# arangesh/TrackMPNN

Hardware: AMD Instinct MI355X
Metric: graph_edges_per_sec_fwd_bwd (higher is better)
Workload: dtype f32; 1 GPU; C2 KITTI Car/RRC-shaped rolling windows: 7 frames, D_t~clip(Poisson(6),1,20), F=8 (2d), H=64, K=0, diff; 1 fwd per frame + 1 bwd per window; 16384 windows/GPU batched block-diagonally (64 distinct seeds tiled); windows_per_gpu=16384, rows_final=6762496, parallelism=sequence-dp1

## Files before the change

### include/tmpnn.h

```cpp
#ifndef TMPNN_H
#define TMPNN_H

#include <stddef.h>
#include <stdint.h>

#ifdef __cplusplus
extern "C" {
#endif

#define TMPNN_ABI_VERSION 4

#define TMPNN_OK 0
#define TMPNN_EINVAL (-1)
#define TMPNN_ELAUNCH (-2)
#define TMPNN_EWORKSPACE (-3)

typedef void* tmpnn_stream;
typedef void* tmpnn_event;

typedef struct tmpnn_seg_plan {
    int32_t T;
    int32_t I;
    int32_t nsplit;
    const int32_t* t_row;
    const int32_t* items;
    const int32_t* rowptr2;
    const int32_t* inc2;
    float* ws;
    size_t ws_floats;
} tmpnn_seg_plan;

typedef struct tmpnn_win_plan {
    int32_t W;
    int32_t nbig;
    const int32_t* wrec;
    const int32_t* erow;
    const uint16_t* recs;
    const int32_t* det;
    const int32_t* drow;
    const int32_t* big_order;
} tmpnn_win_plan;

typedef struct tmpnn_graph {
    int32_t N;
    int32_t E;
    int32_t Dn;
    const int32_t* src;
    const int32_t* dst;
    const int32_t* edge_row;
    const int32_t* det_row;
    const int32_t* rowptr;
    const int32_t* inc;
    const int32_t* det_order;
    const tmpnn_seg_plan* seg_plan;
    const tmpnn_win_plan* win_plan;
} tmpnn_graph;

typedef struct tmpnn_edge_tiles {
    int32_t T;
    int32_t rows_per_tile;
    const int32_t* t_row;
    const int32_t* t_loc;
    const int32_t* t_dptr;
    const int32_t* t_dets;
} tmpnn_edge_tiles;

int tmpnn_abi_version(void);
const char* tmpnn_last_error(void);

int tmpnn_gather_diff_fwd(const tmpnn_graph* g, const float* in, int ld_in, float* out, int ld_out,
                          int H, int accumulate, tmpnn_stream stream);
int tmpnn_gather_concat_fwd(const tmpnn_graph* g, const float* in, int ld_in, float* out, int ld_out,
                            int H, int accumulate, tmpnn_stream stream);
int tmpnn_gather_diff_bwd(const tmpnn_graph* g, const float* d_out, int ld_dout, float* d_in, int ld_din,
                          int H, int accumulate, tmpnn_stream stream);
int tmpnn_gather_concat_bwd(const tmpnn_graph* g, const float* d_out, int ld_dout, float* d_in, int ld_din,
                            int H, int accumulate, tmpnn_stream stream);

int tmpnn_segsum_fwd(const tmpnn_graph* g, const float* in, int ld_in, float* out, int ld_out,
                     int H, int accumulate, int compact_out ,
                     tmpnn_stream stream);
int tmpnn_segsum_fwd_live(const tmpnn_graph* g, const float* in, int ld_in, float* out, int ld_out,
                          int H, int compact_out, int row_limit, tmpnn_stream stream);
int tmpnn_segsum_bwd(const tmpnn_graph* g, const float* d_out, int ld_dout, float* d_in, int ld_din,
                     int H, int accumulate, tmpnn_stream stream);

int tmpnn_att_fwd(const tmpnn_graph* g, const int32_t* erec, const float* h, int ld_h, int H, int K,
                  const float* W_cat, const float* a, const uint8_t* keep, float p_drop,
                  float* ha, float* score, float* stats, float* esk, float* alpha, float* out, int ld_out,
                  tmpnn_stream stream);
size_t tmpnn_att_bwd_ws(int E, int Dn, int H, int K);
int tmpnn_att_index(const tmpnn_graph* g, const int32_t* pos, const int32_t* src_pos, const int32_t* dst_pos,
                    int32_t* erec, int32_t* inc_other, tmpnn_stream stream);
int tmpnn_att_bwd(const tmpnn_graph* g, const int32_t* erec, const int32_t* inc_other,
                  const float* h, int ld_h, int H, int K,
                  const float* W_cat, const float* a, const uint8_t* keep, float p_drop,
                  const float* ha, const float* score, const float* stats, const float* esk,
                  const float* d_out, int ld_dout, float* ws, size_t ws_floats,
                  float* d_h, int ld_dh, float* dW_att, float* da, tmpnn_stream stream);
int tmpnn_att_bwd_heads(const tmpnn_graph* g, const int32_t* erec, const int32_t* inc_other,
                        const float* h, int ld_h, int H, int K,
                        const float* W_cat, const float* a, const uint8_t* keep, float p_drop,
                        const float* ha, const float* score, const float* stats, const float* esk,
                        const float* d_out, int ld_dout, float* ws, size_t ws_floats,
                        float* d_h, int ld_dh, float* const* dW_heads, float* const* da_heads, tmpnn_stream stream);

int tmpnn_gru_fwd_head_parts(int H, int IN, int xmode);
int tmpnn_gru_fwd(const int32_t* rows, int R, int xmode, const int32_t* src, const int32_t* dst,
                  const float* msg, int ld_msg, int msg_compact, int IN, const float* h, int ld_h, int H,
                  const float* wih_t, const float* whh_t, const float* b_ih, const float* b_hh,
                  float* h_out, int ld_out, float* gates, size_t gate_plane,
                  const float* w_head, float* logit_part, size_t part_stride, tmpnn_stream stream);
int tmpnn_gru_bwd_data(const int32_t* rows, int R, int IN, const float* h, int ld_h, int H,
                       const float* w_ih, const float* w_hh,
                       const float* gates, size_t gate_plane, const float* d_hout, int ld_dhout,
                       const float* dy, const float* w_head,
                       float* d_msg, int ld_dmsg, float* d_h, int ld_dh,
                       const int32_t* add_src, const int32_t* add_dst, const float* add_msg, int ld_add,
                       tmpnn_stream stream);
size_t tmpnn_gru_bwd_weights_ws(int R, int IN, int H);
int tmpnn_gru_bwd_weights(const int32_t* rows, int R, int xmode, const int32_t* src, const int32_t* dst,
                          const float* msg, int ld_msg, int msg_compact, int IN,
                          const float* h, int ld_h, int H,
                          const float* gates, size_t gate_plane, const float* d_hout, int ld_dhout,
                          const float* dy, const float* w_head,
                          float* dW_ih, float* dW_hh, float* db_ih, float* db_hh,
                          void* ws, size_t ws_bytes, tmpnn_stream stream);

int tmpnn_gru_bwd_fused_available(int H, int IN, int xmode);
size_t tmpnn_gru_bwd_fused_ws(int R, int IN, int H);
int tmpnn_gru_bwd_fused(const int32_t* rows, int R, int xmode, const int32_t* src, const int32_t* dst,
                        const float* msg, int ld_msg, int msg_compact, int IN,
                        const float* h, int ld_h, int H, const float* w_ih, const float* w_hh,
                        const float* gates, size_t gate_plane, const float* d_hout, int ld_dhout,
                        const float* dy, const float* w_head,
                        float* d_msg, int ld_dmsg, float* d_h, int ld_dh,
                        const int32_t* add_src, const int32_t* add_dst, const float* add_msg, int ld_add,
                        float* dW_ih, float* dW_hh, float* db_ih, float* db_hh,
                        void* ws, size_t ws_bytes, tmpnn_stream stream);
int tmpnn_gru_bwd_fused_zero_state_available(int H, int IN, int xmode);
int tmpnn_gru_bwd_fused_zero_state(const int32_t* rows, int R, const int32_t* src, const int32_t* dst, int IN,
                                   const float* h, int ld_h, int H, const float* w_ih, const float* b_hn,
                                   const float* gates, size_t gate_plane, const float* d_hout, int ld_dhout,
                                   const float* dy, const float* w_head, float* d_msg, int ld_dmsg,
                                   float* dW_ih, float* db_ih, float* db_hh,
                                   void* ws, size_t ws_bytes, tmpnn_stream stream);

int tmpnn_gru_fwd_tiles(const tmpnn_edge_tiles* tiles, int R, const float* proj, int ld_proj, const float* h, int ld_h, int H,
                        const float* whh_t, const float* b_ih, const float* b_hh, float* h_out, int ld_out, float* gates,
                        size_t gate_plane, const float* w_head, float* logit_part, size_t part_stride, tmpnn_stream stream);
int tmpnn_gru_fwd_tiles_zero_state_available(int H, int xmode);
int tmpnn_gru_fwd_tiles_zero_state(const tmpnn_edge_tiles* tiles, int R, const float* proj, int ld_proj, int H,
                                   const float* b_ih, const float* b_hh, float* h_out, int ld_out, float* gates,
                                   size_t gate_plane, int write_hn, const float* w_head, float* logit_part, size_t part_stride,
                                   tmpnn_stream stream);

int tmpnn_rows_linear(const int32_t* rows, int R, const float* in, int ld_in, int H, const float* wt, int NOUT,
                      float* out, int ld_out, tmpnn_stream stream);

int tmpnn_transpose(const float* in, int rows, int cols, float* out, tmpnn_stream stream);

int tmpnn_input_bn_fwd(const float* xdet, int ld_x, int F, int nd, const int32_t* seg_ptr,
                       const int32_t* seg_cnt, const int32_t* seg_of_det ,
                       int S, int H, int training,
                       const float* w1, const float* b1, const float* gamma, const float* beta,
                       float* running_mean, float* running_var,
                       const float* w2, const float* b2,
                       float* y_save, float* mean, float* rstd, float* ws_a ,
                       const int32_t* out_row, float* h_new, int ld_h, tmpnn_stream stream);
size_t tmpnn_input_bn_bwd_ws(int nd, int S, int H, int F);
int tmpnn_input_bn_bwd(const float* xdet, int ld_x, int F, int nd, const int32_t* seg_ptr,
                       const int32_t* seg_cnt, const int32_t* seg_of_det, int S, int H, int training,
                       const float* w1, const float* b1, const float* gamma, const float* beta,
                       const float* w2,
                       const float* y_save, const float* mean, const float* rstd,
                       const int32_t* out_row, const float* d_h, int ld_dh,
                       float* d_xdet, int ld_dx, float* d_xzero,
                       float* dw1, float* db1, float* dgamma, float* dbeta, float* dw2, float* db2,
                       float* ws, size_t ws_floats, tmpnn_stream stream);

int tmpnn_input_tf_supported(int H, int F, int max_seg_rows);
int tmpnn_input_tf_fwd(const float* xdet, const int64_t* x_rows, int ld_x, int F, int nd, const int32_t* seg_ptr, const int32_t* seg_cnt,
                       const int32_t* seg_of_det, int S, int max_seg_rows, int H, int training, const float* w1, const float* b1,
                       const float* gamma, const float* beta, float* running_mean, float* running_var, const float* w2,
                       const float* b2, float* y_save, float* mean, float* rstd, const int32_t* out_row, float* h_new,
                       int ld_h, tmpnn_stream stream);
size_t tmpnn_input_tf_bwd_ws(int nd, int S, int H, int F, int training);
int tmpnn_input_tf_bwd(const float* xdet, const int64_t* x_rows, int ld_x, int F, int nd, const int32_t* seg_ptr, const int32_t* seg_cnt,
                       const int32_t* seg_of_det, int S, int max_seg_rows, int H, int training, const float* w1, const float* b1,
                       const float* gamma, const float* beta, const float* w2, const float* y_save, const float* mean,
                       const float* rstd, const int32_t* out_row, const float* d_h, int ld_dh, float* d_xdet, int ld_dx,
                       float* d_xzero, float* dw1, float* db1, float* dgamma, float* dbeta, float* dw2, float* db2, void* ws,
                       size_t ws_bytes, tmpnn_stream stream);

int tmpnn_heads_fwd(const float* h, int ld_h, int C, int N, const uint8_t* is_edge,
                    const float* w_node, const float* b_node, const float* w_edge, const float* b_edge,
                    float* logits, float* scores, tmpnn_stream stream);
int tmpnn_heads_finish(const float* parts, size_t part_stride, int nparts, int N, const uint8_t* is_edge,
                       const float* b_node, const float* b_edge, float* logits, float* scores, tmpnn_stream stream);
size_t tmpnn_heads_bwd_ws(int N, int C);
int tmpnn_heads_bwd(const float* h, int ld_h, int C, int N, const uint8_t* is_edge,
                    const float* w_node, const float* w_edge, const float* scores,
                    const float* d_logits, const float* d_scores, float* dy_out,
                    float* d_h, int ld_dh, int accumulate,
                    float* dw_node, float* db_node, float* dw_edge, float* db_edge,
                    void* ws, size_t ws_bytes, tmpnn_stream stream);

int tmpnn_targets(const tmpnn_graph* g, const uint8_t* labels, uint8_t* targets, tmpnn_stream stream);
size_t tmpnn_ce_loss_ws(int Dn);
int tmpnn_ce_loss_fwd(const tmpnn_graph* g, const float* logits, const uint8_t* targets, float* stats, float* loss,
                      float* ws, size_t ws_floats, tmpnn_stream stream);
int tmpnn_ce_loss_bwd(const tmpnn_graph* g, const int32_t* src_pos, const int32_t* dst_pos, const float* logits,
                      const float* stats, const float* d_loss, float* d_logits, tmpnn_stream stream);
size_t tmpnn_focal_loss_ws(int R);
int tmpnn_focal_loss_fwd(const int32_t* rows, int R, const float* scores, const uint8_t* targets, float gamma,
                         int use_alpha, float alpha0, float alpha1, float* loss_sum, float* ws, size_t ws_floats,
                         tmpnn_stream stream);
int tmpnn_focal_loss_bwd(const int32_t* rows, int R, const float* scores, const uint8_t* targets, float gamma,
                         int use_alpha, float alpha0, float alpha1, const float* d_loss, float scale, float* d_scores,
                         tmpnn_stream stream);
size_t tmpnn_bce_logits_ws(long n);
int tmpnn_bce_logits_sum_fwd(const float* logits, const float* targets, long n, float* loss_sum, float* ws, size_t ws_floats,
                             tmpnn_stream stream);
int tmpnn_bce_logits_sum_bwd(const float* logits, const float* targets, long n, const float* d_loss, float* d_logits,
                             tmpnn_stream stream);
int tmpnn_train_losses_supported(int E, int Dn);
size_t tmpnn_train_losses_ws(int E, int Dn);
int tmpnn_train_losses_fwd(const tmpnn_graph* g, const float* logits, const float* scores, const uint8_t* labels,
                           int tp_classifier, uint8_t* targets, float* stats, float* out, float* ws, size_t ws_floats,
                           tmpnn_stream stream);
int tmpnn_train_losses_bwd(const tmpnn_graph* g, const int32_t* src_pos, const int32_t* dst_pos, const float* logits,
                           const float* scores, const uint8_t* targets, const float* stats, const float* d_c, const float* d_f,
                           int tp_classifier, float* d_logits, float* d_scores, tmpnn_stream stream);

#define TMPNN_DG_MAX_ROWS 4096
#define TMPNN_DG_BIG_ROWS 65535
#define TMPNN_TRACK_MAX_ROWS 32768
#define TMPNN_DG_META 8
#define TMPNN_DG_BAD_VALUE 1
#define TMPNN_DG_BAD_ROW 2
#define TMPNN_DG_BAD_ENDPOINT 4
#define TMPNN_DG_BAD_ORDER 8
#define TMPNN_DG_BAD_EDGE_DIAG 16
#define TMPNN_DG_BAD_EDGE_ADJ 32

typedef struct tmpnn_dgraph {
    int32_t N;
    int32_t cap;
    int32_t* meta;
    uint8_t* is_edge;
    int32_t* pos;
    int32_t* src;
    int32_t* dst;
    int32_t* src_pos;
    int32_t* dst_pos;
    int32_t* edge_row;
    int32_t* det_row;
    int32_t* rowptr;
    int32_t* inc;
} tmpnn_dgraph;

size_t tmpnn_dgraph_ints(int cap);
int tmpnn_dgraph_bind(void* arena, int cap, int N, tmpnn_dgraph* out);

int tmpnn_graph_from_coo(int N, const int64_t* node_idx, const float* node_val, int64_t nnz_node,
                         const int64_t* edge_idx, const float* edge_val, int64_t nnz_edge,
                         const tmpnn_dgraph* g, tmpnn_stream stream);

int tmpnn_graph_from_coo_arena(int N, const int64_t* node_idx, const float* node_val, int64_t nnz_node,
                               const int64_t* edge_idx, const float* edge_val, int64_t nnz_edge, void* arena, int cap,
                               tmpnn_stream stream);
int tmpnn_graph_from_coo_arena_ws(int N, const int64_t* node_idx, const float* node_val, int64_t nnz_node,
                                  const int64_t* edge_idx, const float* edge_val, int64_t nnz_edge, void* arena, int cap,
                                  void* ws, size_t ws_ints, tmpnn_stream stream);

int tmpnn_graph_from_rows_ws(int N, const uint8_t* is_edge, const int32_t* row_src, const int32_t* row_dst,
                             const tmpnn_dgraph* g, void* ws, size_t ws_ints, tmpnn_stream stream);

typedef struct tmpnn_mp_params {
    int32_t G, H, IN_e , F_total;
    int32_t F[3];
    float* w1[3]; float* b1[3]; float* gamma[3]; float* beta[3]; float* w2[3]; float* b2[3];
    float* run_mean[3]; float* run_var[3];
    int64_t* num_batches_tracked[3];
    float* e_wih[3]; float* e_whh[3]; float* e_bih[3]; float* e_bhh[3];
    float* n_wih[3]; float* n_whh[3]; float* n_bih[3]; float* n_bhh[3];
    float* w_node; float* b_node; float* w_edge; float* b_edge;
} tmpnn_mp_params;

size_t tmpnn_mp_iter_prep_floats(int G, int H, int IN_e);
int tmpnn_mp_iter_prepare(const tmpnn_mp_params* P, float* prep, tmpnn_stream stream);

size_t tmpnn_mp_iter_save_floats(int N, int n_new, int G, int H);
int tmpnn_mp_iter_fwd(const tmpnn_mp_params* P, const float* prep, const tmpnn_dgraph* g, int n_new,
                      const float* x, int ld_x, float* h, int training,
                      float* h_out, float* logits, float* scores, float* save, size_t save_floats,
                      tmpnn_stream stream);
size_t tmpnn_mp_iter_save_es_offset(int N, int n_new, int G, int H);
int tmpnn_mp_iter_fwd_parts(const tmpnn_mp_params* P, const float* prep, const tmpnn_dgraph* g, int n_new,
                            const float* x, int ld_x, float* h, int training,
                            float* h_out, float* logits, float* scores, float* save, size_t save_floats, int parts,
                            tmpnn_stream stream);
size_t tmpnn_mp_iter_bwd_ws(int N, int n_new, int G, int H, int IN_e);
int tmpnn_mp_iter_bwd(const tmpnn_mp_params* P, const float* prep, const tmpnn_dgraph* g, int n_new,
                      const float* x, int ld_x, const float* h, const float* h_out, const float* scores,
                      const float* save, int training,
                      const float* d_scores, int st_dscores, const float* d_logits, int st_dlogits,
                      const float* d_hout, float* d_h, float* d_x, const tmpnn_mp_params* grads,
                      void* ws, size_t ws_bytes, tmpnn_stream stream);
int tmpnn_mp_iter_bwd_parts(const tmpnn_mp_params* P, const float* prep, const tmpnn_dgraph* g, int n_new,
                            const float* x, int ld_x, const float* h, const float* h_out, const float* scores,
                            const float* save, int training,
                            const float* d_scores, int st_dscores, const float* d_logits, int st_dlogits,
                            const float* d_hout, float* d_h, float* d_x, const tmpnn_mp_params* grads,
                            void* ws, size_t ws_bytes, int parts, tmpnn_stream stream);

size_t tmpnn_track_finalize_ws(int max_dets);

typedef struct tmpnn_track_rows {
    int32_t *ts, *det_id, *assoc;
    uint8_t* is_edge;
    int32_t *src, *dst;
    uint8_t* labels;
} tmpnn_track_rows;
int tmpnn_track_load(int N, int ND, const int32_t* packed, const tmpnn_track_rows* rows, const float* X, int ld_x, int F,
                     float* feats, int ld_f, int32_t* y_track, const tmpnn_dgraph* g, void* ws, size_t ws_ints,
                     tmpnn_stream stream);
int tmpnn_track_select(const tmpnn_dgraph* g, const tmpnn_track_rows* rows, const float* score, int mode, int t,
                       int associate, int32_t* active, int32_t* small, tmpnn_stream stream);
int tmpnn_track_select_ws(const tmpnn_dgraph* g, const tmpnn_track_rows* rows, const float* score, int mode, int t,
                          int associate, int32_t* active, int32_t* small, void* ws, size_t ws_bytes, tmpnn_stream stream);
int tmpnn_track_hungarian_max_dets(void);
int tmpnn_track_extend(int N, int A, int D, const int32_t* active, const int32_t* new_ids, int t, const int32_t* track,
                       const tmpnn_track_rows* rows, const float* X, int ld_x, int F, float* feats, int ld_f,
                       const tmpnn_dgraph* g_new, void* ws, size_t ws_ints, tmpnn_stream stream);
int tmpnn_track_extend_tf(int N, int A, int D, const int32_t* active, const int32_t* new_ids, int t, const int32_t* track,
                          const tmpnn_track_rows* rows, const float* X, int ld_x, const tmpnn_mp_params* P, float* h,
                          float* save, size_t save_floats, const tmpnn_dgraph* g_new, const int32_t* counts,
                          const float* gather_src, int ld_gather, const int32_t* gather_keep, tmpnn_stream stream);
int tmpnn_track_retire(const tmpnn_dgraph* g, const tmpnn_track_rows* rows, const float* score, int associate, int t_upto,
                       int ret_win, int32_t* y_track, int ND, int32_t* pos_of_det, void* fin_ws, size_t fin_ws_bytes,
                       int32_t* keep, int32_t* small, const tmpnn_track_rows* rows_out, const float* h, int ld_h, int W,
                       float* h_new, int ld_hn, float* s_new, int next_t, int32_t* active, int32_t* notify,
                       tmpnn_stream stream);


int tmpnn_wide_supported(int H, int IN);
size_t tmpnn_wide_prep_bytes(int H, int IN);
int tmpnn_wide_prepare(const float* w_ih , const float* w_hh , int IN, int H, void* prep,
                       tmpnn_stream stream);
int tmpnn_wide_gru_fwd(const void* prep, const int32_t* det_rows, int Dn, const int32_t* rows, int R,
                       const int32_t* src_pos, const int32_t* dst_pos, const float* h, int ld_h, int H,
                       const float* b_ih, const float* b_hh, float* P, float* h_out, int ld_out, float* gates,
                       size_t gate_plane, tmpnn_stream stream);
int tmpnn_wide_gru_fwd_tiled(const void* prep, const int32_t* det_rows, int Dn, const tmpnn_edge_tiles* tiles, int R,
                             const float* h, int ld_h, int H, const float* b_ih, const float* b_hh, float* P,
                             float* h_out, int ld_out, float* gates, size_t gate_plane, tmpnn_stream stream);


// ... 44 lines not shown
```

### trackmpnn_amd/_lib.py

```python
from __future__ import annotations

import ctypes as C

import torch
import os
import re
from typing import Dict, List, Optional

_HERE = os.path.dirname(os.path.abspath(__file__))
LIB_PATH = os.environ.get('TMPNN_LIB_PATH') or os.path.join(_HERE, 'lib', 'libtmpnn.so')
HEADER_PATH = os.path.join(os.path.dirname(_HERE), 'include', 'tmpnn.h')

ABI_VERSION = 4

c_int = C.c_int
c_void_p = C.c_void_p
c_size_t = C.c_size_t
c_float = C.c_float


class CSegPlan(C.Structure):
    _fields_ = [('T', C.c_int32), ('I', C.c_int32), ('nsplit', C.c_int32), ('t_row', c_void_p), ('items', c_void_p),
                ('rowptr2', c_void_p), ('inc2', c_void_p), ('ws', c_void_p), ('ws_floats', c_size_t)]


class CWinPlan(C.Structure):
    _fields_ = [('W', C.c_int32), ('nbig', C.c_int32), ('wrec', c_void_p), ('erow', c_void_p), ('recs', c_void_p),
                ('det', c_void_p), ('drow', c_void_p), ('big_order', c_void_p)]


class CGraph(C.Structure):
    _fields_ = [('N', C.c_int32), ('E', C.c_int32), ('Dn', C.c_int32),
                ('src', c_void_p), ('dst', c_void_p), ('edge_row', c_void_p), ('det_row', c_void_p),
                ('rowptr', c_void_p), ('inc', c_void_p), ('det_order', c_void_p), ('seg_plan', c_void_p),
                ('win_plan', c_void_p)]


_GP = C.POINTER(CGraph)


class CEdgeTiles(C.Structure):
    _fields_ = [('T', C.c_int32), ('rows_per_tile', C.c_int32), ('t_row', c_void_p), ('t_loc', c_void_p),
                ('t_dptr', c_void_p), ('t_dets', c_void_p)]


_TP = C.POINTER(CEdgeTiles)


class CDGraph(C.Structure):
    _fields_ = [('N', C.c_int32), ('cap', C.c_int32), ('meta', c_void_p), ('is_edge', c_void_p), ('pos', c_void_p),
                ('src', c_void_p), ('dst', c_void_p), ('src_pos', c_void_p), ('dst_pos', c_void_p),
                ('edge_row', c_void_p), ('det_row', c_void_p), ('rowptr', c_void_p), ('inc', c_void_p)]


_P3 = c_void_p * 3


class CMpParams(C.Structure):
    _fields_ = [('G', C.c_int32), ('H', C.c_int32), ('IN_e', C.c_int32), ('F_total', C.c_int32), ('F', C.c_int32 * 3),
                ('w1', _P3), ('b1', _P3), ('gamma', _P3), ('beta', _P3), ('w2', _P3), ('b2', _P3),
                ('run_mean', _P3), ('run_var', _P3), ('num_batches_tracked', _P3),
                ('e_wih', _P3), ('e_whh', _P3), ('e_bih', _P3), ('e_bhh', _P3),
                ('n_wih', _P3), ('n_whh', _P3), ('n_bih', _P3), ('n_bhh', _P3),
                ('w_node', c_void_p), ('b_node', c_void_p), ('w_edge', c_void_p), ('b_edge', c_void_p)]


class CTrackRows(C.Structure):
    _fields_ = [('ts', c_void_p), ('det_id', c_void_p), ('assoc', c_void_p), ('is_edge', c_void_p), ('src', c_void_p),
                ('dst', c_void_p), ('labels', c_void_p)]


_DGP = C.POINTER(CDGraph)
_MPP = C.POINTER(CMpParams)
_TRP = C.POINTER(CTrackRows)

_SIGNATURES = {
    'tmpnn_abi_version': (c_int, []),
    'tmpnn_last_error': (C.c_char_p, []),
    'tmpnn_gather_diff_fwd': (c_int, [_GP, c_void_p, c_int, c_void_p, c_int, c_int, c_int, c_void_p]),
    'tmpnn_gather_concat_fwd': (c_int, [_GP, c_void_p, c_int, c_void_p, c_int, c_int, c_int, c_void_p]),
    'tmpnn_gather_diff_bwd': (c_int, [_GP, c_void_p, c_int, c_void_p, c_int, c_int, c_int, c_void_p]),
    'tmpnn_gather_concat_bwd': (c_int, [_GP, c_void_p, c_int, c_void_p, c_int, c_int, c_int, c_void_p]),
    'tmpnn_segsum_fwd': (c_int, [_GP, c_void_p, c_int, c_void_p, c_int, c_int, c_int, c_int, c_void_p]),
    'tmpnn_segsum_fwd_live': (c_int, [_GP, c_void_p, c_int, c_void_p, c_int, c_int, c_int, c_int, c_void_p]),
    'tmpnn_segsum_bwd': (c_int, [_GP, c_void_p, c_int, c_void_p, c_int, c_int, c_int, c_void_p]),
    'tmpnn_att_fwd': (c_int, [_GP, c_void_p, c_void_p, c_int, c_int, c_int, c_void_p, c_void_p, c_void_p, c_float,
                              c_void_p, c_void_p, c_void_p, c_void_p, c_void_p, c_void_p, c_int, c_void_p]),
    'tmpnn_att_bwd_ws': (c_size_t, [c_int, c_int, c_int, c_int]),
    'tmpnn_att_index': (c_int, [_GP, c_void_p, c_void_p, c_void_p, c_void_p, c_void_p, c_void_p]),
    'tmpnn_att_bwd': (c_int, [_GP, c_void_p, c_void_p, c_void_p, c_int, c_int, c_int, c_void_p, c_void_p, c_void_p,
                              c_float, c_void_p, c_void_p, c_void_p, c_void_p, c_void_p, c_int, c_void_p, c_size_t,
                              c_void_p, c_int, c_void_p, c_void_p, c_void_p]),
    'tmpnn_att_bwd_heads': (c_int, [_GP, c_void_p, c_void_p, c_void_p, c_int, c_int, c_int, c_void_p, c_void_p,
                                    c_void_p, c_float, c_void_p, c_void_p, c_void_p, c_void_p, c_void_p, c_int, c_void_p,
                                    c_size_t, c_void_p, c_int, c_void_p, c_void_p, c_void_p]),
    'tmpnn_gru_fwd': (c_int, [c_void_p, c_int, c_int, c_void_p, c_void_p, c_void_p, c_int, c_int, c_int,
                              c_void_p, c_int, c_int, c_void_p, c_void_p, c_void_p, c_void_p,
                              c_void_p, c_int, c_void_p, c_size_t, c_void_p, c_void_p, c_size_t, c_void_p]),
    'tmpnn_gru_fwd_head_parts': (c_int, [c_int, c_int, c_int]),
    'tmpnn_gru_fwd_tiles': (c_int, [_TP, c_int, c_void_p, c_int, c_void_p, c_int, c_int, c_void_p, c_void_p, c_void_p,
                                    c_void_p, c_int, c_void_p, c_size_t, c_void_p, c_void_p, c_size_t, c_void_p]),
    'tmpnn_gru_fwd_tiles_zero_state_available': (c_int, [c_int, c_int]),
    'tmpnn_gru_fwd_tiles_zero_state': (c_int, [_TP, c_int, c_void_p, c_int, c_int, c_void_p, c_void_p, c_void_p, c_int,
                                               c_void_p, c_size_t, c_int, c_void_p, c_void_p, c_size_t, c_void_p]),
    'tmpnn_heads_finish': (c_int, [c_void_p, c_size_t, c_int, c_int, c_void_p, c_void_p, c_void_p, c_void_p, c_void_p, c_void_p]),
    'tmpnn_gru_bwd_data': (c_int, [c_void_p, c_int, c_int, c_void_p, c_int, c_int, c_void_p, c_void_p,
                                   c_void_p, c_size_t, c_void_p, c_int, c_void_p, c_void_p,
                                   c_void_p, c_int, c_void_p, c_int,
                                   c_void_p, c_void_p, c_void_p, c_int, c_void_p]),
    'tmpnn_gru_bwd_weights_ws': (c_size_t, [c_int, c_int, c_int]),
    'tmpnn_gru_bwd_weights': (c_int, [c_void_p, c_int, c_int, c_void_p, c_void_p, c_void_p, c_int, c_int, c_int,
                                      c_void_p, c_int, c_int, c_void_p, c_size_t, c_void_p, c_int, c_void_p, c_void_p,
                                      c_void_p, c_void_p, c_void_p, c_void_p, c_void_p, c_size_t, c_void_p]),
    'tmpnn_gru_bwd_fused_available': (c_int, [c_int, c_int, c_int]),
    'tmpnn_gru_bwd_fused_ws': (c_size_t, [c_int, c_int, c_int]),
    'tmpnn_gru_bwd_fused': (c_int, [c_void_p, c_int, c_int, c_void_p, c_void_p, c_void_p, c_int, c_int, c_int,
                                    c_void_p, c_int, c_int, c_void_p, c_void_p, c_void_p, c_size_t, c_void_p, c_int,
                                    c_void_p, c_void_p, c_void_p, c_int, c_void_p, c_int,
                                    c_void_p, c_void_p, c_void_p, c_int, c_void_p, c_void_p, c_void_p, c_void_p,
                                    c_void_p, c_size_t, c_void_p]),
    'tmpnn_gru_bwd_fused_zero_state_available': (c_int, [c_int, c_int, c_int]),
    'tmpnn_gru_bwd_fused_zero_state': (c_int, [c_void_p, c_int, c_void_p, c_void_p, c_int, c_void_p, c_int, c_int,
                                               c_void_p, c_void_p, c_void_p, c_size_t, c_void_p, c_int, c_void_p,
                                               c_void_p, c_void_p, c_int, c_void_p, c_void_p, c_void_p, c_void_p,
                                               c_size_t, c_void_p]),
    'tmpnn_rows_linear': (c_int, [c_void_p, c_int, c_void_p, c_int, c_int, c_void_p, c_int, c_void_p, c_int, c_void_p]),
    'tmpnn_transpose': (c_int, [c_void_p, c_int, c_int, c_void_p, c_void_p]),
    'tmpnn_input_bn_fwd': (c_int, [c_void_p, c_int, c_int, c_int, c_void_p, c_void_p, c_void_p, c_int, c_int, c_int,
                                   c_void_p, c_void_p, c_void_p, c_void_p, c_void_p, c_void_p, c_void_p, c_void_p,
                                   c_void_p, c_void_p, c_void_p, c_void_p, c_void_p, c_void_p, c_int, c_void_p]),
    'tmpnn_input_bn_bwd_ws': (c_size_t, [c_int, c_int, c_int, c_int]),
    'tmpnn_input_bn_bwd': (c_int, [c_void_p, c_int, c_int, c_int, c_void_p, c_void_p, c_void_p, c_int, c_int, c_int,
                                   c_void_p, c_void_p, c_void_p, c_void_p, c_void_p,
                                   c_void_p, c_void_p, c_void_p, c_void_p, c_void_p, c_int,
                                   c_void_p, c_int, c_void_p,
                                   c_void_p, c_void_p, c_void_p, c_void_p, c_void_p, c_void_p,
                                   c_void_p, c_size_t, c_void_p]),
    'tmpnn_input_tf_supported': (c_int, [c_int, c_int, c_int]),
    'tmpnn_input_tf_fwd': (c_int, [c_void_p, c_void_p, c_int, c_int, c_int, c_void_p, c_void_p, c_void_p, c_int, c_int, c_int, c_int,
                                   c_void_p, c_void_p, c_void_p, c_void_p, c_void_p, c_void_p, c_void_p, c_void_p,
                                   c_void_p, c_void_p, c_void_p, c_void_p, c_void_p, c_int, c_void_p]),
    'tmpnn_input_tf_bwd_ws': (c_size_t, [c_int, c_int, c_int, c_int, c_int]),
    'tmpnn_input_tf_bwd': (c_int, [c_void_p, c_void_p, c_int, c_int, c_int, c_void_p, c_void_p, c_void_p, c_int, c_int, c_int, c_int,
                                   c_void_p, c_void_p, c_void_p, c_void_p, c_void_p,
                                   c_void_p, c_void_p, c_void_p, c_void_p, c_void_p, c_int,
                                   c_void_p, c_int, c_void_p,
                                   c_void_p, c_void_p, c_void_p, c_void_p, c_void_p, c_void_p,
                                   c_void_p, c_size_t, c_void_p]),
    'tmpnn_heads_fwd': (c_int, [c_void_p, c_int, c_int, c_int, c_void_p, c_void_p, c_void_p, c_void_p, c_void_p,
                                c_void_p, c_void_p, c_void_p]),
    'tmpnn_heads_bwd_ws': (c_size_t, [c_int, c_int]),
    'tmpnn_heads_bwd': (c_int, [c_void_p, c_int, c_int, c_int, c_void_p, c_void_p, c_void_p, c_void_p, c_void_p,
                                c_void_p, c_void_p, c_void_p, c_int, c_int, c_void_p, c_void_p, c_void_p, c_void_p,
                                c_void_p, c_size_t, c_void_p]),
    'tmpnn_targets': (c_int, [_GP, c_void_p, c_void_p, c_void_p]),
    'tmpnn_ce_loss_ws': (c_size_t, [c_int]),
    'tmpnn_ce_loss_fwd': (c_int, [_GP, c_void_p, c_void_p, c_void_p, c_void_p, c_void_p, c_size_t, c_void_p]),
    'tmpnn_ce_loss_bwd': (c_int, [_GP, c_void_p, c_void_p, c_void_p, c_void_p, c_void_p, c_void_p, c_void_p]),
    'tmpnn_focal_loss_ws': (c_size_t, [c_int]),
    'tmpnn_focal_loss_fwd': (c_int, [c_void_p, c_int, c_void_p, c_void_p, c_float, c_int, c_float, c_float, c_void_p,
                                     c_void_p, c_size_t, c_void_p]),
    'tmpnn_focal_loss_bwd': (c_int, [c_void_p, c_int, c_void_p, c_void_p, c_float, c_int, c_float, c_float, c_void_p,
                                     c_float, c_void_p, c_void_p]),
    'tmpnn_bce_logits_ws': (c_size_t, [C.c_long]),
    'tmpnn_bce_logits_sum_fwd': (c_int, [c_void_p, c_void_p, C.c_long, c_void_p, c_void_p, c_size_t, c_void_p]),
    'tmpnn_bce_logits_sum_bwd': (c_int, [c_void_p, c_void_p, C.c_long, c_void_p, c_void_p, c_void_p]),
    'tmpnn_train_losses_supported': (c_int, [c_int, c_int]),
    'tmpnn_train_losses_ws': (c_size_t, [c_int, c_int]),
    'tmpnn_train_losses_fwd': (c_int, [_GP, c_void_p, c_void_p, c_void_p, c_int, c_void_p, c_void_p, c_void_p, c_void_p,
                                       c_size_t, c_void_p]),
    'tmpnn_train_losses_bwd': (c_int, [_GP, c_void_p, c_void_p, c_void_p, c_void_p, c_void_p, c_void_p, c_void_p, c_void_p,
                                       c_int, c_void_p, c_void_p, c_void_p]),
    'tmpnn_dgraph_ints': (c_size_t, [c_int]),
    'tmpnn_dgraph_bind': (c_int, [c_void_p, c_int, c_int, _DGP]),
    'tmpnn_graph_from_coo': (c_int, [c_int, c_void_p, c_void_p, C.c_int64, c_void_p, c_void_p, C.c_int64, _DGP, c_void_p]),
    'tmpnn_graph_from_coo_arena': (c_int, [c_int, c_void_p, c_void_p, C.c_int64, c_void_p, c_void_p, C.c_int64, c_void_p, c_int, c_void_p]),
    'tmpnn_graph_from_coo_arena_ws': (c_int, [c_int, c_void_p, c_void_p, C.c_int64, c_void_p, c_void_p, C.c_int64, c_void_p, c_int,
                                              c_void_p, c_size_t, c_void_p]),
    'tmpnn_graph_from_rows_ws': (c_int, [c_int, c_void_p, c_void_p, c_void_p, _DGP, c_void_p, c_size_t, c_void_p]),
    'tmpnn_track_finalize_ws': (c_size_t, [c_int]),
    'tmpnn_track_load': (c_int, [c_int, c_int, c_void_p, _TRP, c_void_p, c_int, c_int, c_void_p, c_int, c_void_p, _DGP, c_void_p,
                                 c_size_t, c_void_p]),
    'tmpnn_track_select': (c_int, [_DGP, _TRP, c_void_p, c_int, c_int, c_int, c_void_p, c_void_p, c_void_p]),
    'tmpnn_track_select_ws': (c_int, [_DGP, _TRP, c_void_p, c_int, c_int, c_int, c_void_p, c_void_p, c_void_p, c_size_t, c_void_p]),
    'tmpnn_track_hungarian_max_dets': (c_int, []),
    'tmpnn_track_extend': (c_int, [c_int, c_int, c_int, c_void_p, c_void_p, c_int, c_void_p, _TRP, c_void_p, c_int, c_int,
                                   c_void_p, c_int, _DGP, c_void_p, c_size_t, c_void_p]),
    'tmpnn_track_extend_tf': (c_int, [c_int, c_int, c_int, c_void_p, c_void_p, c_int, c_void_p, _TRP, c_void_p, c_int, c_void_p,
                                      c_void_p, c_void_p, c_size_t, _DGP, c_void_p, c_void_p, c_int, c_void_p, c_void_p]),
    'tmpnn_track_retire': (c_int, [_DGP, _TRP, c_void_p, c_int, c_int, c_int, c_void_p, c_int, c_void_p, c_void_p, c_size_t,
                                   c_void_p, c_void_p, _TRP, c_void_p, c_int, c_int, c_void_p, c_int, c_void_p, c_int,
                                   c_void_p, c_void_p, c_void_p]),
    'tmpnn_wide_supported': (c_int, [c_int, c_int]),
    'tmpnn_wide_prep_bytes': (c_size_t, [c_int, c_int]),
    'tmpnn_wide_prepare': (c_int, [c_void_p, c_void_p, c_int, c_int, c_void_p, c_void_p]),
    'tmpnn_wide_gru_fwd': (c_int, [c_void_p, c_void_p, c_int, c_void_p, c_int, c_void_p, c_void_p, c_void_p, c_int, c_int,
                                   c_void_p, c_void_p, c_void_p, c_void_p, c_int, c_void_p, c_size_t, c_void_p]),
    'tmpnn_wide_gru_fwd_tiled': (c_int, [c_void_p, c_void_p, c_int, _TP, c_int, c_void_p, c_int, c_int, c_void_p, c_void_p,
                                         c_void_p, c_void_p, c_int, c_void_p, c_size_t, c_void_p]),
    'tmpnn_wide_gru_bwd_diff_ws': (c_size_t, [c_int, c_int, c_int, c_int]),
    'tmpnn_wide_gru_bwd_diff': (c_int, [c_void_p, _GP, c_void_p, c_int, c_int, c_void_p, c_size_t, c_void_p, c_int,
                                        c_void_p, c_void_p, c_void_p, c_int, c_void_p, c_void_p, c_void_p, c_void_p,
                                        c_void_p, c_size_t, c_void_p]),
    'tmpnn_wide_gru_bwd_diff_fused': (c_int, [c_void_p, _GP, c_void_p, c_int, c_int, c_void_p, c_size_t, c_void_p, c_int,
                                              c_void_p, c_void_p, c_void_p, c_int, c_void_p, c_void_p, c_void_p, c_void_p,
                                              c_void_p, c_size_t, c_void_p, c_int, c_void_p, c_void_p, c_void_p, c_void_p]),
    'tmpnn_mp_iter_prep_floats': (c_size_t, [c_int, c_int, c_int]),
    'tmpnn_mp_iter_prepare': (c_int, [_MPP, c_void_p, c_void_p]),
    'tmpnn_mp_iter_save_floats': (c_size_t, [c_int, c_int, c_int, c_int]),
    'tmpnn_mp_iter_fwd': (c_int, [_MPP, c_void_p, _DGP, c_int, c_void_p, c_int, c_void_p, c_int,
                                  c_void_p, c_void_p, c_void_p, c_void_p, c_size_t, c_void_p]),
    'tmpnn_mp_iter_save_es_offset': (c_size_t, [c_int, c_int, c_int, c_int]),
    'tmpnn_mp_iter_fwd_parts': (c_int, [_MPP, c_void_p, _DGP, c_int, c_void_p, c_int, c_void_p, c_int,
                                        c_void_p, c_void_p, c_void_p, c_void_p, c_size_t, c_int, c_void_p]),
    'tmpnn_mp_iter_bwd_parts': (c_int, [_MPP, c_void_p, _DGP, c_int, c_void_p, c_int, c_void_p, c_void_p, c_void_p, c_void_p,
                                        c_int, c_void_p, c_int, c_void_p, c_int, c_void_p, c_void_p, c_void_p, _MPP, c_void_p,
                                        c_size_t, c_int, c_void_p]),
    'tmpnn_mp_iter_bwd_ws': (c_size_t, [c_int, c_int, c_int, c_int, c_int]),
    'tmpnn_mp_iter_bwd': (c_int, [_MPP, c_void_p, _DGP, c_int, c_void_p, c_int, c_void_p, c_void_p, c_void_p, c_void_p,
                                  c_int, c_void_p, c_int, c_void_p, c_int, c_void_p, c_void_p, c_void_p, _MPP, c_void_p,
                                  c_size_t, c_void_p]),
}

_lib: Optional[C.CDLL] = None


_VARIANT_SIGNATURES = {
    'tmpnn_track_append': (c_int, [c_int, c_int, c_int, c_void_p, c_void_p, c_int, c_void_p, c_void_p, c_void_p, c_void_p,
                                   c_void_p, c_void_p, c_void_p, c_void_p, c_void_p]),
    'tmpnn_gru_bwd_weights_variant': (c_int, [c_void_p, c_int, c_int, c_void_p, c_void_p, c_void_p, c_int, c_int, c_int,
                                              c_void_p, c_int, c_int, c_void_p, c_size_t, c_void_p, c_int, c_void_p, c_void_p,
                                              c_void_p, c_void_p, c_void_p, c_void_p, c_void_p, c_size_t, c_int, c_void_p]),
    'tmpnn_gru_bwd_weights_choice': (c_int, []),
    'tmpnn_wide_gru_bwd_diff_aux': (c_int, [c_void_p, _GP, c_void_p, c_int, c_int, c_void_p, c_size_t, c_void_p, c_int,
                                            c_void_p, c_void_p, c_void_p, c_int, c_void_p, c_void_p, c_void_p, c_void_p,
                                            c_void_p, c_size_t, c_void_p, c_void_p, c_void_p, c_void_p]),
    'tmpnn_wide_gru_bwd_data_ws': (c_size_t, [c_int, c_int]),
    'tmpnn_wide_gru_bwd_data': (c_int, [c_void_p, c_void_p, c_int, c_void_p, c_int, c_int, c_void_p, c_size_t, c_void_p, c_int,
                                        c_void_p, c_void_p, c_void_p, c_int, c_void_p, c_int, c_void_p, c_size_t, c_void_p]),
    'tmpnn_wide_gru_bwd_weights_ws': (c_size_t, [c_int, c_int]),
    'tmpnn_wide_gru_bwd_weights': (c_int, [c_void_p, c_void_p, c_int, c_void_p, c_void_p, c_void_p, c_int, c_int, c_void_p,
                                           c_void_p, c_void_p, c_void_p, c_void_p, c_size_t, c_void_p]),
}


def header_symbols(variants: bool = False) -> List[str]:
    with open(HEADER_PATH) as f:
        txt = f.read()
    if not variants:
        txt = re.sub(r'#ifdef TMPNN_KEEP_VARIANTS.*?#endif', '', txt, flags=re.S)
    txt = re.sub(r'/\*.*?\*/', '', txt, flags=re.S)
    return sorted(set(re.findall(r'\b(tmpnn_[a-z0-9_]+)\s*\(', txt)))


def load() -> C.CDLL:
    global _lib
    if _lib is not None:
        return _lib
    if not os.path.exists(LIB_PATH):
        raise RuntimeError(
            f'{LIB_PATH} is missing: build it with `python -c "import __graft_entry__ as g; g.build()"` '
            '(hipcc --offload-arch=gfx950).  trackmpnn_amd has no CPU or torch fallback.')
    lib = C.CDLL(LIB_PATH)
    for name, (res, args) in _SIGNATURES.items():
        try:
            fn = getattr(lib, name)
        except AttributeError as e:
            raise RuntimeError(f'libtmpnn.so does not export {name}; rebuild it') from e
        fn.restype = res
        fn.argtypes = args
    for name, (res, args) in _VARIANT_SIGNATURES.items():
        fn = getattr(lib, name, None)
        if fn is not None:
            fn.restype = res
            fn.argtypes = args
    v = lib.tmpnn_abi_version()
    if v != ABI_VERSION:
        raise RuntimeError(f'libtmpnn.so ABI version {v} != expected {ABI_VERSION}; rebuild it')
    _lib = lib
    return lib


def last_error() -> str:
    return load().tmpnn_last_error().decode('utf-8', 'replace')


def call(name: str, *args) -> None:
    lib = load()
    rc = getattr(lib, name)(*args)
    if rc != 0:
        raise RuntimeError(f'{name} failed (code {rc}): {last_error()}')


def fn(name: str):
    return getattr(load(), name)


def ptr(t) -> Optional[int]:
    if t is None:
        return None
    return t.data_ptr()


def raw_stream(device=None) -> int:
    idx = torch.cuda.current_device() if device is None or device.index is None else device.index
    return torch._C._cuda_getCurrentRawStream(idx)
```

### trackmpnn_amd/csrc/dense.hip

```cpp
#include "common.h"

namespace tmpnn {

static constexpr float BN_EPS = 1e-5f;
static constexpr float BN_MOMENTUM = 0.1f;

__global__ __launch_bounds__(256) void k_gemm(GemmArgs g, int kper, float* slab) {
    __shared__ float As[16][68];
    __shared__ float Bs[16][68];
    const int tid = threadIdx.x;
    const int tx = tid & 15, ty = tid >> 4;
    const int m0 = blockIdx.y * 64, n0 = blockIdx.x * 64;
    const int kbeg = blockIdx.z * kper;
    const int kend = min(g.K, kbeg + kper);
    float acc[4][4] = {};
    const bool va = (reinterpret_cast<uintptr_t>(g.A) & 15) == 0 && ((g.sak == 1 ? g.sam : g.sak) & 3) == 0;
    const bool vb = (reinterpret_cast<uintptr_t>(g.B) & 15) == 0 && ((g.sbn == 1 ? g.sbk : g.sbn) & 3) == 0;
    for (int k0 = kbeg; k0 < kend; k0 += 16) {
        const bool fullk = k0 + 16 <= kend;
        if (fullk && m0 + 64 <= g.M && !g.a_krows && g.sak == 1 && va) {
            const int m = tid >> 2, kq = (tid & 3) * 4;
            const long ar = g.a_rows ? g.a_rows[m0 + m] : (m0 + m);
            const float4 v = *reinterpret_cast<const float4*>(g.A + ar * g.sam + k0 + kq);
            As[kq][m] = v.x; As[kq + 1][m] = v.y; As[kq + 2][m] = v.z; As[kq + 3][m] = v.w;
// ... 498 lines not shown
    d.w = r.w / cnt * (cnt * d.w - a1.w - yh.w * a2.w);
    *reinterpret_cast<float4*>(dyhat + idx) = d;
}

__global__ void k_bn_bwd_dy0(float* __restrict__ s1, float* __restrict__ s2, const int32_t* __restrict__ seg_ptr,
                             const int32_t* __restrict__ seg_cnt, int S, int H, const float* __restrict__ b1,
                             const float* __restrict__ mean, const float* __restrict__ rstd) {
    const size_t idx = (size_t)blockIdx.x * blockDim.x + threadIdx.x;
    if (idx >= (size_t)S * H) return;
    const int s = (int)(idx / H), j = (int)(idx % H);
    const float cnt = (float)seg_cnt[s];
    const float nz = cnt - (float)(seg_ptr[s + 1] - seg_ptr[s]);
    const float yh0 = (b1[j] - mean[idx]) * rstd[idx];
    const float dy0 = rstd[idx] / cnt * (-s1[idx] - yh0 * s2[idx]);
    s1[idx] = dy0;
    s2[idx] = nz * dy0;
}

__global__ void k_gather_rows(const float* __restrict__ src, long ld, const int32_t* __restrict__ rows, int n, int H,
                              float* __restrict__ dst) {
    const size_t idx = ((size_t)blockIdx.x * blockDim.x + threadIdx.x) * 4;
    if (idx >= (size_t)n * H) return;
    const int i = (int)(idx / H), j = (int)(idx % H);
    *reinterpret_cast<float4*>(dst + idx) = *reinterpret_cast<const float4*>(src + (size_t)rows[i] * ld + j);
}

__global__ __launch_bounds__(256) void k_heads_fwd(const float* __restrict__ h, int ld_h, int C, int N,
                                                   const uint8_t* __restrict__ is_edge,
                                                   const float* __restrict__ w_node, const float* __restrict__ b_node,
                                                   const float* __restrict__ w_edge, const float* __restrict__ b_edge,
                                                   float* __restrict__ logits, float* __restrict__ scores) {
    const int sub = threadIdx.x & 15;
    const long rows_per_pass = (long)gridDim.x * 16;
    for (long i = (long)blockIdx.x * 16 + (threadIdx.x >> 4); i < N; i += rows_per_pass) {
        const bool e = is_edge[i] != 0;
        const float* w = e ? w_edge : w_node;
        const float* hr = h + (size_t)i * ld_h;
        float s = 0.f;
        for (int c4 = sub * 4; c4 < C; c4 += 64) {
            const float4 x = *reinterpret_cast<const float4*>(hr + c4);
            const float4 ww = *reinterpret_cast<const float4*>(w + c4);
            s += x.x * ww.x + x.y * ww.y + x.z * ww.z + x.w * ww.w;
        }
        s += __shfl_xor(s, 8);
        s += __shfl_xor(s, 4);
        s += __shfl_xor(s, 2);
        s += __shfl_xor(s, 1);
        if (sub == 0) {
            const float y = s + (e ? b_edge[0] : b_node[0]);
            logits[i] = y;
            scores[i] = 1.0f / (1.0f + expf(-y));
        }
    }
}

__global__ void k_heads_finish(const float* __restrict__ parts, size_t stride, int nparts, int N,
                               const uint8_t* __restrict__ is_edge, const float* __restrict__ b_node,
                               const float* __restrict__ b_edge, float* __restrict__ logits,
                               float* __restrict__ scores) {
    const int i = blockIdx.x * blockDim.x + threadIdx.x;
    if (i >= N) return;
    float y = is_edge[i] ? b_edge[0] : b_node[0];
    for (int p = 0; p < nparts; ++p) y += parts[(size_t)p * stride + i];
    logits[i] = y;
    scores[i] = 1.0f / (1.0f + expf(-y));
}

__global__ __launch_bounds__(256) void k_heads_bwd(const float* __restrict__ h, int ld_h, int C, int N,
                                                   const uint8_t* __restrict__ is_edge,
                                                   const float* __restrict__ w_node, const float* __restrict__ w_edge,
                                                   const float* __restrict__ scores, const float* __restrict__ d_logits,
                                                   const float* __restrict__ d_scores, float* __restrict__ dy_out,
                                                   float* __restrict__ d_h,
                                                   int ld_dh, int accumulate, int rows_per_block,
                                                   float* __restrict__ part) {
    extern __shared__ float sm[];
    const int cpt = C >> 2;
    const int slots = 256 / cpt;
    const int slot = threadIdx.x / cpt;
    const int c4 = (threadIdx.x % cpt) * 4;
    const bool active = slot < slots;
    float4 an = make_float4(0.f, 0.f, 0.f, 0.f), ae = an;
    float bn = 0.f, be = 0.f;
    const long r0 = (long)blockIdx.x * rows_per_block;
    const long r1 = min((long)N, r0 + rows_per_block);
    if (active) {
        constexpr int UR = 4;
        for (long i0 = r0 + slot; i0 < r1; i0 += (long)slots * UR) {
            float dyv[UR];
            bool ev[UR], live[UR];
            float4 xv[UR];
#pragma unroll
            for (int u = 0; u < UR; ++u) {
                const long i = i0 + (long)u * slots;
                live[u] = i < r1;
                const long ic = live[u] ? i : r1 - 1;
                float dy = d_logits ? d_logits[ic] : 0.f;
                if (d_scores) {
                    const float sc = scores[ic];
                    dy += d_scores[ic] * sc * (1.0f - sc);
                }
                dyv[u] = live[u] ? dy : 0.f;
                ev[u] = is_edge[ic] != 0;
                xv[u] = *reinterpret_cast<const float4*>(h + (size_t)ic * ld_h + c4);
            }
#pragma unroll
            for (int u = 0; u < UR; ++u) {
                if (!live[u]) continue;
                const long i = i0 + (long)u * slots;
                const float dy = dyv[u];
                const bool e = ev[u];
                const float4 x = xv[u];
                if (dy_out && c4 == 0) dy_out[i] = dy;
                if (d_h) {
                    const float4 w = *reinterpret_cast<const float4*>((e ? w_edge : w_node) + c4);
                    float* dp = d_h + (size_t)i * ld_dh + c4;
                    float4 o = make_float4(dy * w.x, dy * w.y, dy * w.z, dy * w.w);
                    if (accumulate) {
                        const float4 p = *reinterpret_cast<const float4*>(dp);
                        o.x += p.x; o.y += p.y; o.z += p.z; o.w += p.w;
                    }
                    *reinterpret_cast<float4*>(dp) = o;
                }
                if (e) { ae.x += dy * x.x; ae.y += dy * x.y; ae.z += dy * x.z; ae.w += dy * x.w; if (c4 == 0) be += dy; }
                else   { an.x += dy * x.x; an.y += dy * x.y; an.z += dy * x.z; an.w += dy * x.w; if (c4 == 0) bn += dy; }
            }
        }
        float* my = sm + (size_t)slot * 2 * C;
        *reinterpret_cast<float4*>(my + c4) = an;
        *reinterpret_cast<float4*>(my + C + c4) = ae;
        if (c4 == 0) {
            sm[(size_t)slots * 2 * C + slot * 2 + 0] = bn;
            sm[(size_t)slots * 2 * C + slot * 2 + 1] = be;
        }
    }
    __syncthreads();
    float* out = part + (size_t)blockIdx.x * (2 * C + 2);
    for (int j = threadIdx.x; j < 2 * C + 2; j += 256) {
        float s = 0.f;
        if (j < 2 * C) for (int k = 0; k < slots; ++k) s += sm[(size_t)k * 2 * C + j];
        else for (int k = 0; k < slots; ++k) s += sm[(size_t)slots * 2 * C + k * 2 + (j - 2 * C)];
        out[j] = s;
    }
}

__global__ void k_heads_bwd_final(const float* __restrict__ red, int C, float* __restrict__ dw_node,
                                  float* __restrict__ db_node, float* __restrict__ dw_edge,
                                  float* __restrict__ db_edge) {
    const int j = blockIdx.x * blockDim.x + threadIdx.x;
    if (j >= 2 * C + 2) return;
    const float s = red[j];
    if (j < C) dw_node[j] += s;
    else if (j < 2 * C) dw_edge[j - C] += s;
    else if (j == 2 * C) db_node[0] += s;
    else db_edge[0] += s;
}

static int heads_rows_per_block(int N) {
    long rpb = ((long)N + 2047) / 2048;
    if (rpb < 64) rpb = 64;
    return (int)rpb;
}

}

using namespace tmpnn;

extern "C" {

int tmpnn_input_bn_fwd(const float* xdet, int ld_x, int F, int nd, const int32_t* seg_ptr, const int32_t* seg_cnt,
                       const int32_t* seg_of_det, int S, int H, int training, const float* w1, const float* b1, const float* gamma,
                       const float* beta, float* running_mean, float* running_var, const float* w2, const float* b2,
                       float* y_save, float* mean, float* rstd, float* ws_a, const int32_t* out_row, float* h_new,
                       int ld_h, tmpnn_stream stream) {
    TM_REQUIRE(supported_H_cell(H), "input_bn_fwd: unsupported H=%d", H);
    TM_REQUIRE(F > 0 && nd >= 0 && S >= 0, "input_bn_fwd: F=%d nd=%d S=%d", F, nd, S);
    TM_REQUIRE(w1 && b1 && gamma && beta && running_mean && running_var && w2 && b2 && mean && rstd,
               "input_bn_fwd: null parameter pointer");
    TM_REQUIRE(!training || (seg_ptr && seg_cnt && S > 0), "input_bn_fwd: training needs segments");
    hipStream_t st = as_stream(stream);
    int rc;
    if (nd > 0) {
        TM_REQUIRE(xdet && y_save && ws_a && out_row && h_new && ld_x >= F && ld_h >= H, "input_bn_fwd: null/short buffers");
        TM_REQUIRE(aligned16(y_save) && aligned16(ws_a) && aligned16(mean) && aligned16(rstd) && aligned16(gamma) && aligned16(beta),
                   "input_bn_fwd: y_save / ws_a / mean / rstd / gamma / beta must be 16-byte aligned");
        GemmArgs g{xdet, ld_x, 1, nullptr, nullptr, w1, 1, F, b1, y_save, H, nullptr, nd, H, F, 0};
        if ((rc = launch_gemm(g, st))) return rc;
    }
    if (training) {
        hipLaunchKernelGGL(k_bn_stats, dim3(S), dim3(H, bn_row_groups(nd, S, H)), 0, st, y_save, seg_ptr, seg_cnt, H, b1, mean, rstd);
        if ((rc = check_launch("bn_stats"))) return rc;
        hipLaunchKernelGGL(k_bn_running, dim3(H), dim3(64), 0, st, mean, rstd, seg_cnt, S, H, running_mean,
                           running_var);
        if ((rc = check_launch("bn_running"))) return rc;
    } else {
        hipLaunchKernelGGL(k_running_to_stats, dim3(ceil_div(H, 64)), dim3(64), 0, st, running_mean, running_var, H,
                           mean, rstd);
        if ((rc = check_launch("running_to_stats"))) return rc;
    }
    if (nd == 0) return TMPNN_OK;
    hipLaunchKernelGGL(k_bn_apply, dim3(ceil_div((long)nd * H / 4, 256)), dim3(256), 0, st, y_save, nd, H,
                       training ? seg_ptr : nullptr, S, seg_of_det, mean, rstd, gamma, beta, (float*)nullptr, ws_a);
    if ((rc = check_launch("bn_apply"))) return rc;
    GemmArgs g2{ws_a, H, 1, nullptr, nullptr, w2, 1, H, b2, h_new, ld_h, out_row, nd, H, H, 0};
    return launch_gemm(g2, st);
}

int tmpnn_input_bn_bwd(const float* xdet, int ld_x, int F, int nd, const int32_t* seg_ptr, const int32_t* seg_cnt,
                       const int32_t* seg_of_det, int S, int H, int training, const float* w1, const float* b1, const float* gamma,
                       const float* beta, const float* w2, const float* y_save, const float* mean, const float* rstd,
                       const int32_t* out_row, const float* d_h, int ld_dh, float* d_xdet, int ld_dx, float* d_xzero,
                       float* dw1, float* db1, float* dgamma, float* dbeta, float* dw2, float* db2, float* ws,
                       size_t ws_floats, tmpnn_stream stream) {
    TM_REQUIRE(supported_H_cell(H), "input_bn_bwd: unsupported H=%d", H);
    TM_REQUIRE(F > 0 && nd >= 0 && S >= 0, "input_bn_bwd: F=%d nd=%d S=%d", F, nd, S);
    TM_REQUIRE(w1 && b1 && gamma && beta && w2 && mean && rstd && dw1 && db1 && dgamma && dbeta && dw2 && db2,
               "input_bn_bwd: null parameter pointer");
    hipStream_t st = as_stream(stream);
    if (nd == 0) {
        if (d_xzero && S > 0) (void)hipMemsetAsync(d_xzero, 0, sizeof(float) * (size_t)S * F, st);
        return TMPNN_OK;
    }
    TM_REQUIRE(xdet && y_save && out_row && d_h && ws, "input_bn_bwd: null buffers");
    const size_t ndH = (size_t)nd * H, SH = (size_t)(S > 0 ? S : 1) * H;
    const size_t need = tmpnn_input_bn_bwd_ws(nd, S, H, F);
    if (ws_floats < need) return set_error(TMPNN_EWORKSPACE, "input_bn_bwd: workspace %zu < %zu floats", ws_floats, need);
    TM_REQUIRE(aligned16(y_save) && aligned16(mean) && aligned16(rstd) && aligned16(gamma) && aligned16(beta) && aligned16(ws) &&
                   aligned16(d_h) && (ld_dh & 3) == 0,
               "input_bn_bwd: y_save / mean / rstd / gamma / beta / ws / d_h must be 16-byte aligned (ld_dh a multiple of 4)");
    float* B0 = ws;
    float* B1 = B0 + ndH;
    float* B2 = B1 + ndH;
    float* s1 = B2 + ndH;
    float* s2 = s1 + SH;
    float* scratch = s2 + SH;
    const size_t scratch_n = ws_floats - (3 * ndH + 2 * SH);
    const int gridE = ceil_div((long)ndH / 4, 256);
    int rc;
    hipLaunchKernelGGL(k_gather_rows, dim3(gridE), dim3(256), 0, st, d_h, (long)ld_dh, out_row, nd, H, B0);
    if ((rc = check_launch("gather_rows"))) return rc;
    hipLaunchKernelGGL(k_bn_apply, dim3(gridE), dim3(256), 0, st, y_save, nd, H, training ? seg_ptr : nullptr, S,
                       seg_of_det, mean, rstd, gamma, beta, B1, B2);
    if ((rc = check_launch("bn_apply"))) return rc;
    {
        GemmArgs g{B0, 1, H, nullptr, nullptr, B2, H, 1, nullptr, dw2, H, nullptr, H, H, nd, 1};
        if ((rc = launch_gemm_splitk(g, scratch, scratch_n, st))) return rc;
        if ((rc = launch_colsum(B0, H, nullptr, 0, nd, H, db2, 1, scratch, scratch_n, st))) return rc;
    }
    {
        GemmArgs g{B0, H, 1, nullptr, nullptr, w2, H, 1, nullptr, B2, H, nullptr, nd, H, H, 0};
        if ((rc = launch_gemm(g, st))) return rc;
    }
    hipLaunchKernelGGL(k_bn_bwd_act, dim3(gridE), dim3(256), 0, st, B2, B1, nd, H, gamma, beta, B0);
    if ((rc = check_launch("bn_bwd_act"))) return rc;
    if ((rc = launch_colsum(B0, H, B1, H, nd, H, dgamma, 1, scratch, scratch_n, st))) return rc;
    if ((rc = launch_colsum(B0, H, nullptr, 0, nd, H, dbeta, 1, scratch, scratch_n, st))) return rc;
    if (training) {
        hipLaunchKernelGGL(k_bn_bwd_seg, dim3(S), dim3(H, bn_row_groups(nd, S, H)), 0, st, B2, B1, seg_ptr, seg_cnt, H, b1, mean, rstd, s1, s2);
        if ((rc = check_launch("bn_bwd_seg"))) return rc;
    }
    hipLaunchKernelGGL(k_bn_bwd_dy, dim3(gridE), dim3(256), 0, st, B2, B1, nd, H, seg_ptr, seg_cnt, S, seg_of_det, rstd,
                       s1, s2, training);
    if ((rc = check_launch("bn_bwd_dy"))) return rc;
    {
        GemmArgs g{B2, 1, H, nullptr, nullptr, xdet, ld_x, 1, nullptr, dw1, F, nullptr, H, F, nd, 1};
        if ((rc = launch_gemm_splitk(g, scratch, scratch_n, st))) return rc;
        if ((rc = launch_colsum(B2, H, nullptr, 0, nd, H, db1, 1, scratch, scratch_n, st))) return rc;
        if (d_xdet) {
            GemmArgs gx{B2, H, 1, nullptr, nullptr, w1, F, 1, nullptr, d_xdet, ld_dx, nullptr, nd, F, H, 0};
            if ((rc = launch_gemm(gx, st))) return rc;
        }
    }
    if (training) {
        hipLaunchKernelGGL(k_bn_bwd_dy0, dim3(ceil_div((long)S * H, 256)), dim3(256), 0, st, s1, s2, seg_ptr, seg_cnt,
                           S, H, b1, mean, rstd);
        if ((rc = check_launch("bn_bwd_dy0"))) return rc;
        const size_t cs2 = colsum_ws_floats(S, H);
        if (scratch_n < cs2) return set_error(TMPNN_EWORKSPACE, "input_bn_bwd: workspace too small for segments");
        if ((rc = launch_colsum(s2, H, nullptr, 0, S, H, db1, 1, scratch, scratch_n, st))) return rc;
        if (d_xzero) {
            GemmArgs gz{s1, H, 1, nullptr, nullptr, w1, F, 1, nullptr, d_xzero, F, nullptr, S, F, H, 0};
            if ((rc = launch_gemm(gz, st))) return rc;
        }
    } else if (d_xzero && S > 0) {
        (void)hipMemsetAsync(d_xzero, 0, sizeof(float) * (size_t)S * F, st);
    }
    return TMPNN_OK;
}

size_t tmpnn_input_bn_bwd_ws(int nd, int S, int H, int F) {
    if (nd <= 0) return 0;
    const size_t ndH = (size_t)nd * H, SH = (size_t)(S > 0 ? S : 1) * H;
    size_t x = colsum_ws_floats(nd, H);
    const size_t a = gemm_splitk_ws_floats(H, H, nd), b = gemm_splitk_ws_floats(H, F, nd),
                 c = colsum_ws_floats(S > 0 ? S : 1, H);
    if (a > x) x = a;
    if (b > x) x = b;
    if (c > x) x = c;
    return 3 * ndH + 2 * SH + x;
}

int tmpnn_heads_fwd(const float* h, int ld_h, int C, int N, const uint8_t* is_edge, const float* w_node,
                    const float* b_node, const float* w_edge, const float* b_edge, float* logits, float* scores,
                    tmpnn_stream stream) {
    TM_REQUIRE(C > 0 && (C & 3) == 0 && N >= 0, "heads_fwd: C=%d N=%d", C, N);
    if (N == 0) return TMPNN_OK;
    TM_REQUIRE(h && is_edge && w_node && b_node && w_edge && b_edge && logits && scores, "heads_fwd: null pointer");
    TM_REQUIRE(ld_h >= C && (ld_h & 3) == 0 && aligned16(h) && aligned16(w_node) && aligned16(w_edge),
               "heads_fwd: rows must be 16-byte aligned");
    long b = ((long)N + 15) / 16;
    if (b > 4096) b = 4096;
    hipLaunchKernelGGL(k_heads_fwd, dim3((int)b), dim3(256), 0, as_stream(stream), h, ld_h, C, N, is_edge, w_node,
                       b_node, w_edge, b_edge, logits, scores);
    return check_launch("heads_fwd");
}

int tmpnn_heads_finish(const float* parts, size_t part_stride, int nparts, int N, const uint8_t* is_edge,
                       const float* b_node, const float* b_edge, float* logits, float* scores, tmpnn_stream stream) {
    TM_REQUIRE(nparts > 0 && N >= 0, "heads_finish: nparts=%d N=%d", nparts, N);
    if (N == 0) return TMPNN_OK;
    TM_REQUIRE(parts && is_edge && b_node && b_edge && logits && scores && part_stride >= (size_t)N, "heads_finish: null pointer");
    hipLaunchKernelGGL(k_heads_finish, dim3(ceil_div(N, 256)), dim3(256), 0, as_stream(stream), parts, part_stride, nparts, N,
                       is_edge, b_node, b_edge, logits, scores);
    return check_launch("heads_finish");
}

size_t tmpnn_heads_bwd_ws(int N, int C) {
    if (N <= 0) return 0;
    const int rpb = heads_rows_per_block(N);
    const int nblk = ceil_div(N, rpb);
    const size_t n = 2 * (size_t)C + 2;
    return ((size_t)nblk * n + n + reduce_slabs_ws_floats(nblk, n)) * sizeof(float);
}

int tmpnn_heads_bwd(const float* h, int ld_h, int C, int N, const uint8_t* is_edge, const float* w_node,
                    const float* w_edge, const float* scores, const float* d_logits, const float* d_scores,
                    float* dy_out, float* d_h, int ld_dh, int accumulate, float* dw_node, float* db_node,
                    float* dw_edge, float* db_edge, void* ws, size_t ws_bytes, tmpnn_stream stream) {
    TM_REQUIRE(C > 0 && (C & 3) == 0 && C <= 1024 && N >= 0, "heads_bwd: C=%d N=%d", C, N);
    if (N == 0) return TMPNN_OK;
    TM_REQUIRE(h && is_edge && w_node && w_edge && dw_node && db_node && dw_edge && db_edge, "heads_bwd: null pointer");
    TM_REQUIRE(d_scores == nullptr || scores != nullptr, "heads_bwd: d_scores needs scores");
    TM_REQUIRE((ld_h & 3) == 0 && aligned16(h) && aligned16(w_node) && aligned16(w_edge) &&
                   (d_h == nullptr || ((ld_dh & 3) == 0 && aligned16(d_h))),
               "heads_bwd: rows must be 16-byte aligned");
    const size_t need = tmpnn_heads_bwd_ws(N, C);
    if (!ws || ws_bytes < need) return set_error(TMPNN_EWORKSPACE, "heads_bwd: workspace %zu < %zu", ws_bytes, need);
    const int rpb = heads_rows_per_block(N);
    const int nblk = ceil_div(N, rpb);
    const int cpt = C >> 2;
    TM_REQUIRE(cpt <= 256, "heads_bwd: C too wide");
    const int slots = 256 / cpt;
    const size_t shm = ((size_t)slots * 2 * C + (size_t)slots * 2) * sizeof(float);
    hipStream_t st = as_stream(stream);
    hipLaunchKernelGGL(k_heads_bwd, dim3(nblk), dim3(256), shm, st, h, ld_h, C, N, is_edge, w_node, w_edge, scores,
                       d_logits, d_scores, dy_out, d_h, ld_dh, accumulate, rpb, reinterpret_cast<float*>(ws));
    int rc = check_launch("heads_bwd");
    if (rc) return rc;
    const size_t nred = 2 * (size_t)C + 2;
    float* part = reinterpret_cast<float*>(ws);
    float* red = part + (size_t)nblk * nred;
    if ((rc = launch_reduce_slabs(part, nred, nblk, red, nred, 0, st, red + nred))) return rc;
    hipLaunchKernelGGL(k_heads_bwd_final, dim3(ceil_div(2 * C + 2, 256)), dim3(256), 0, st, red, C, dw_node, db_node,
                       dw_edge, db_edge);
    return check_launch("heads_bwd_final");
}

}
```

### trackmpnn_amd/csrc/gru_bwd.hip

```cpp
#include "gru_common.h"

namespace tmpnn {



template <int NT>
__global__ __launch_bounds__(256) void k_gru_bwd_data(GruBwdDataArgs a) {
    const int wave = threadIdx.x >> 6, lane = threadIdx.x & 63;
    const int c = lane & 31, half = lane >> 5;
    const int r0 = (blockIdx.x * 4 + wave) * 32;
    if (r0 >= a.R) return;
    const int H = a.H;
    const int vcol0 = blockIdx.y * (32 * NT);
    const bool is_dx = vcol0 < a.IN;
    const int n0 = is_dx ? vcol0 : vcol0 - a.IN;
    const float* __restrict__ W = is_dx ? a.w_ih : a.w_hh;
    const int ldw = is_dx ? a.IN : H;
    const int li = min(r0 + c, a.R - 1);
    const int row = a.rows[li];
    const size_t gp = a.gate_plane;

    f32x16 acc[NT];
#pragma unroll
    for (int t = 0; t < NT; ++t)
// ... 1290 lines not shown
        const uint16_t* p0_ = (base0);                                                                       \
        const uint16_t* p1_ = (base1);                                                                       \
        const uint2 u0_ = lds_read_tr(p0_), u1_ = lds_read_tr(p1_);                                          \
        const uint2 v0_ = lds_read_tr(p0_ + (pstride)), v1_ = lds_read_tr(p1_ + (pstride));                 \
        const uint2 w0_ = lds_read_tr(p0_ + 2 * (pstride)), w1_ = lds_read_tr(p1_ + 2 * (pstride));         \
        (q1) = make_uint4(u0_.x, u0_.y, u1_.x, u1_.y);                                                       \
        (q2) = make_uint4(v0_.x, v0_.y, v1_.x, v1_.y);                                                       \
        (q3) = make_uint4(w0_.x, w0_.y, w1_.x, w1_.y);                                                       \
    } while (0)
#define ONE_LD_BT(kb)                                                                                        \
    do {                                                                                                     \
        ONE_LD_TR(cur + (kb) * 2048 + offB[0][0], cur + (kb) * 2048 + offB[0][1], PB, bt[0].p1, bt[0].p2, bt[0].p3); \
        ONE_LD_TR(cur + (kb) * 2048 + offB[1][0], cur + (kb) * 2048 + offB[1][1], PB, bt[1].p1, bt[1].p2, bt[1].p3); \
    } while (0)
#define ONE_LD_A(g)                                                                                          \
    ONE_LD_TR(cur + ((g) / 3) * 2048 + offA[(g) % 3][0], cur + ((g) / 3) * 2048 + offA[(g) % 3][1], PA,      \
              aW[0][0], aW[0][1], aW[0][2])
        ONE_LD_D(0);
        ONE_LD_BT(0);
        ONE_LD_A(0);
        const int erow_n = a.rows[min((tile + G) * 32 + c, a.R - 1)];
        const bool elive_n = (it + 1 < nmine) && ((tile + G) * 32 + c < a.R);

        f32x16 accd;
#pragma unroll
        for (int i = 0; i < 16; ++i) accd[i] = 0.f;
        float d0[4], tt[4];
#pragma unroll
        for (int hs = 0; hs < 12; ++hs) {
            const int g = hs >> 1, kk = hs & 1, j = g % 3;
            if (hs + 1 < 12) ONE_LD_D(hs + 1);
            if (kk == 0) {
                acc[j][0] = mfma_c<0>(aW[0], bt[0], acc[j][0]);  accd = mfma_c<0>(wq[hs], bD[hs & 1], accd);
                acc[j][1] = mfma_c<0>(aW[0], bt[1], acc[j][1]);  accd = mfma_c<1>(wq[hs], bD[hs & 1], accd);
                acc[j][0] = mfma_c<1>(aW[0], bt[0], acc[j][0]);  accd = mfma_c<2>(wq[hs], bD[hs & 1], accd);
                acc[j][1] = mfma_c<1>(aW[0], bt[1], acc[j][1]);  accd = mfma_c<3>(wq[hs], bD[hs & 1], accd);
                acc[j][0] = mfma_c<2>(aW[0], bt[0], acc[j][0]);  accd = mfma_c<4>(wq[hs], bD[hs & 1], accd);
                acc[j][1] = mfma_c<2>(aW[0], bt[1], acc[j][1]);  accd = mfma_c<5>(wq[hs], bD[hs & 1], accd);
#pragma unroll
                for (int pc = 0; pc < 3; ++pc) {
                    const uint4 q = aW[0][pc];
                    bsum[j] = dot2_ones(q.x, bsum[j]); bsum[j] = dot2_ones(q.y, bsum[j]);
                    bsum[j] = dot2_ones(q.z, bsum[j]); bsum[j] = dot2_ones(q.w, bsum[j]);
                }
            } else {
                accd = mfma_c<0>(wq[hs], bD[hs & 1], accd);  acc[j][0] = mfma_c<3>(aW[0], bt[0], acc[j][0]);
                accd = mfma_c<1>(wq[hs], bD[hs & 1], accd);  acc[j][1] = mfma_c<3>(aW[0], bt[1], acc[j][1]);
                accd = mfma_c<2>(wq[hs], bD[hs & 1], accd);  acc[j][0] = mfma_c<4>(aW[0], bt[0], acc[j][0]);
                accd = mfma_c<3>(wq[hs], bD[hs & 1], accd);  acc[j][1] = mfma_c<4>(aW[0], bt[1], acc[j][1]);
                accd = mfma_c<4>(wq[hs], bD[hs & 1], accd);  acc[j][0] = mfma_c<5>(aW[0], bt[0], acc[j][0]);
                accd = mfma_c<5>(wq[hs], bD[hs & 1], accd);  acc[j][1] = mfma_c<5>(aW[0], bt[1], acc[j][1]);
            }
            if (kk == 1 && g + 1 < 6) ONE_LD_A(g + 1);
            if (hs == 5) ONE_LD_BT(1);
            if (hs < 6)
                half_slice<XMODE, UP, FUSE>(hs % 6, rawA, validA, head4, d0, tt, nxt, stA0, stA1, seA, SUB, PA, PB, OFF_B, OFF_E);
            else
                half_slice<XMODE, UP, FUSE>(hs % 6, rawB, validB, head4, d0, tt, nxt, stA0 + stB, stA1 + stB, seA + seB, SUB,
                                                    PA, PB, OFF_B, OFF_E);
            __builtin_amdgcn_sched_barrier(0);
            if (hs == 5) {
                half_issue_main<UP>(a, idA, f4, rawA);
                half_issue_gather<XMODE, FUSE>(a, idB, f4, rawB);
                __builtin_amdgcn_sched_barrier(0);
                validB = idB.valid;
                idB = half_ids<XMODE, FUSE>(a, tile + 2 * G, it + 2 < nmine, 16 + hr);
            }
            if (hs == 11) {
                half_issue_main<UP>(a, idB, f4, rawB);
                half_issue_gather<XMODE, FUSE>(a, idA, f4, rawA);
                __builtin_amdgcn_sched_barrier(0);
                validA = idA.valid;
                idA = half_ids<XMODE, FUSE>(a, tile + 3 * G, it + 3 < nmine, hr);
            }
        }
#undef ONE_LD_A
#undef ONE_LD_BT
#undef ONE_LD_TR
#undef ONE_LD_D
        if (is_dx) {
            if (elive) {
#pragma unroll
                for (int q = 0; q < 4; ++q)
                    *reinterpret_cast<float4*>(a.d_msg + (size_t)erow * a.ld_dmsg + n0 + 8 * q + 4 * half) =
                        make_float4(accd[4 * q], accd[4 * q + 1], accd[4 * q + 2], accd[4 * q + 3]);
            }
        } else {
            const float* e = reinterpret_cast<const float*>(cur + OFF_E) + eoff;
            float4 ex4[4];
#pragma unroll
            for (int q = 0; q < 4; ++q) ex4[q] = *reinterpret_cast<const float4*>(e + ((((n0 + 8 * q + 4 * half) >> 2) ^ (c & 15)) << 2));
            if (elive) {
#pragma unroll
                for (int q = 0; q < 4; ++q)
                    *reinterpret_cast<float4*>(a.d_h + (size_t)erow * a.ld_dh + n0 + 8 * q + 4 * half) =
                        make_float4(accd[4 * q] + ex4[q].x, accd[4 * q + 1] + ex4[q].y, accd[4 * q + 2] + ex4[q].z,
                                    accd[4 * q + 3] + ex4[q].w);
            }
        }
        erow = erow_n; elive = elive_n;
        __syncthreads();
    }
#undef ONE_STAGE
    float* sw = a.slab_w + (size_t)blockIdx.x * (3 * H) * (2 * H);
#pragma unroll
    for (int j = 0; j < 3; ++j)
#pragma unroll
        for (int t = 0; t < 2; ++t)
#pragma unroll
            for (int reg = 0; reg < 16; ++reg) {
                const int jj = (jt0 + j) * 32 + acc_row(reg, half);
                sw[(size_t)jj * (2 * H) + which * H + t * 32 + c] = acc[j][t][reg];
            }
    float* sb = a.slab_b + (size_t)blockIdx.x * 6 * H;
#pragma unroll
    for (int j = 0; j < 3; ++j) {
        const float tot = bsum[j] + __shfl_xor(bsum[j], 32);
        const int col = (jt0 + j) * 32 + c;
        if (half == 0) {
            if (which == 0) {
                sb[col] = tot;
                if (col < 2 * H) sb[3 * H + col] = tot;
            } else if (col >= 2 * H) {
                sb[3 * H + col] = tot;
            }
        }
    }
}
#endif

__device__ __forceinline__ f32x4 mfma16_bf16(const uint4& a, const uint4& b, f32x4 c) {
    return __builtin_amdgcn_mfma_f32_16x16x32_bf16(__builtin_bit_cast(bf16x8, a), __builtin_bit_cast(bf16x8, b), c, 0, 0, 0);
}
template <int C>
__device__ __forceinline__ f32x4 mfma16_c(const uint4 (&a)[3], const uint4 (&b)[3], f32x4 acc) {
    if (C == 0) return mfma16_bf16(a[2], b[0], acc);
    if (C == 1) return mfma16_bf16(a[0], b[2], acc);
    if (C == 2) return mfma16_bf16(a[1], b[1], acc);
    if (C == 3) return mfma16_bf16(a[1], b[0], acc);
    if (C == 4) return mfma16_bf16(a[0], b[1], acc);
    return mfma16_bf16(a[0], b[0], acc);
}
template <int C>
__device__ __forceinline__ f32x16 mfma32_c(const uint4 (&a)[3], const uint4 (&b)[3], f32x16 acc) {
    if (C == 0) return mfma_bf16(a[2], b[0], acc);
    if (C == 1) return mfma_bf16(a[0], b[2], acc);
    if (C == 2) return mfma_bf16(a[1], b[1], acc);
    if (C == 3) return mfma_bf16(a[1], b[0], acc);
    if (C == 4) return mfma_bf16(a[0], b[1], acc);
    return mfma_bf16(a[0], b[0], acc);
}

#define TWO_MARK(i) do { } while (0)
struct TwoRaw { float4 dh, r, z, n, hn, hp, xa, xb, ea, eb; float dy; };
#define TWO_LD4(p) (*reinterpret_cast<const float4*>(p))

#ifndef TWO_SCHED
#define TWO_SCHED 1
#endif
#ifndef TWO_EXP
#define TWO_EXP 0
#endif
template <int XMODE, int UP, bool FUSE, bool HHS = true>
__global__ __launch_bounds__(512) void k_gru_bwd_two(GruBwdFusedArgs a, int ntiles) {
    constexpr int exp_ = TWO_EXP;
    constexpr int H = 64;
    constexpr int SUB = 32 * 128;
    constexpr int PA = 2 * SUB, PB = SUB;
    constexpr int OFF_B = 3 * PA, OFF_E = OFF_B + 3 * PB;
    constexpr int BUF = OFF_E + 32 * 64 * 2;
    extern __shared__ float lds[];
    uint16_t* const lds16 = reinterpret_cast<uint16_t*>(lds);
    const int tid = threadIdx.x;
    const int wave = __builtin_amdgcn_readfirstlane(tid >> 6), lane = tid & 63;
    const int role = wave >> 2, q = wave & 3;
    const int lrole = role;
    const int j16 = lane & 15, kq = lane >> 4;
    const int srow = 4 * wave + kq, f4 = 4 * j16;
    const int n0 = 16 * q;
    uint4 wq[6][3];
    {
        const float* W = role == 0 ? a.w_ih : a.w_hh;
        const int ldw = role == 0 ? a.ld_wih : H;
#pragma unroll
        for (int s6 = 0; s6 < 6; ++s6) {
            const int ch = s6 < 4 ? 4 * kq + s6 : 16 + 4 * (s6 - 4) + kq;
            float v[8];
#pragma unroll
            for (int i = 0; i < 8; ++i) v[i] = W[(size_t)(8 * ch + i) * ldw + n0 + j16];
            const Split8 sp = split8_arr(v);
            wq[s6][0] = sp.p1; wq[s6][1] = sp.p2; wq[s6][2] = sp.p3;
        }
    }
    const float headl = (UP & 2) ? a.up.w_head[lane] : 0.f;
    const int st0 = dui_off(srow, f4);
    const int se0 = srow * 64 + (((f4 >> 2) ^ (srow & 15)) << 2);
    const int swzj = dui_swz(j16), rowj = j16 * 128;
    const int hix = lrole == 0 ? 0 : 64;
    const int half = lane >> 5, c32 = lane & 31;
    const int jt0 = (q >> 1) * 3, tt = q & 1;
    const int i16 = lane & 15, tq = i16 >> 2, tp = i16 & 3, tg = (lane >> 4) & 1;
    const int trow = (8 * half + tq) * 128, tsw0 = (tq << 2) | (2 * half);
    int offA[3], offB;
#pragma unroll
    for (int j = 0; j < 3; ++j) {
        const int jj0 = (jt0 + j) * 32;
        const int col = (lrole == 1 && jj0 >= 2 * H) ? jj0 + H : jj0;
        const int ch = ((col & 127) >> 3) + 2 * tg + (tp >> 1);
        offA[j] = (col >> 7) * SUB + trow + ((ch ^ tsw0) << 3) + 4 * (tp & 1);
    }
    {
        const int ch = ((lrole * H + tt * 32) >> 3) + 2 * tg + (tp >> 1);
        offB = OFF_B + trow + ((ch ^ tsw0) << 3) + 4 * (tp & 1);
    }
    f32x16 acc[3];
#pragma unroll
    for (int j = 0; j < 3; ++j)
#pragma unroll
        for (int i = 0; i < 16; ++i) acc[j][i] = 0.f;
    float bsum[3] = {0.f, 0.f, 0.f};

    const int G = gridDim.x;
    const int nmine = (ntiles - (int)blockIdx.x + G - 1) / G;
    TwoRaw raw;
    float d0[4], tv[4];
    auto row_of = [&](int tile, bool tvld, bool& vld) -> int {
        const int lr = tile * 32 + srow;
        vld = tvld && lr < a.R;
        return vld ? lr : a.R - 1;
    };
#define TWO_SLICE(SL, img, vld)                                                                              \
    do {                                                                                                     \
        float o_[4];                                                                                         \
        if ((SL) == 0) {                                                                                     \
            const float dh_[4] = {raw.dh.x, raw.dh.y, raw.dh.z, raw.dh.w}, r_[4] = {raw.r.x, raw.r.y, raw.r.z, raw.r.w}; \
            const float z_[4] = {raw.z.x, raw.z.y, raw.z.z, raw.z.w}, n_[4] = {raw.n.x, raw.n.y, raw.n.z, raw.n.w}; \
            const float hn_[4] = {raw.hn.x, raw.hn.y, raw.hn.z, raw.hn.w};                                   \
            float q_[4];                                                                                     \
            _Pragma("unroll") for (int i = 0; i < 4; ++i) {                                                  \
                float d_ = (UP & 1) ? dh_[i] : 0.f;                                                          \
                if (UP & 2) d_ += raw.dy * __shfl(headl, f4 + i);                                                        \
                d0[i] = (vld) ? d_ : 0.f;                                                                    \
                tv[i] = d0[i] * (1.0f - z_[i]) * (1.0f - n_[i] * n_[i]);                                     \
                q_[i] = tv[i] * r_[i];                                                                       \
                o_[i] = q_[i] * hn_[i] * (1.0f - r_[i]);                                                     \
            }                                                                                                \
            half_put((img), st0, PA, o_);                                                                    \
            half_put((img), SUB + (st0 ^ 64), PA, q_);                                                       \
        } else if ((SL) == 1) {                                                                              \
            const float z_[4] = {raw.z.x, raw.z.y, raw.z.z, raw.z.w}, n_[4] = {raw.n.x, raw.n.y, raw.n.z, raw.n.w}; \
            const float hp_[4] = {raw.hp.x, raw.hp.y, raw.hp.z, raw.hp.w};                                   \
            float e_[4];                                                                                     \
            _Pragma("unroll") for (int i = 0; i < 4; ++i) {                                                  \
                o_[i] = d0[i] * (hp_[i] - n_[i]) * z_[i] * (1.0f - z_[i]);                                   \
                e_[i] = d0[i] * z_[i];                                                                       \
            }                                                                                                \
            half_put((img), st0 ^ 64, PA, o_);                                                               \
            *reinterpret_cast<float4*>(reinterpret_cast<float*>((img) + OFF_E) + se0) = make_float4(e_[0], e_[1], e_[2], e_[3]); \
        } else if ((SL) == 2) {                                                                              \
            const float hp_[4] = {raw.hp.x, raw.hp.y, raw.hp.z, raw.hp.w};                                   \
            half_put((img) + OFF_B, st0 ^ 64, PB, hp_);                                                      \
        } else if ((SL) == 3) {                                                                              \
            half_put((img), SUB + st0, PA, tv);                                                              \
        } else if ((SL) == 5) {                                                                              \
            const float xa_[4] = {raw.xa.x, raw.xa.y, raw.xa.z, raw.xa.w}, xb_[4] = {raw.xb.x, raw.xb.y, raw.xb.z, raw.xb.w}; \
            _Pragma("unroll") for (int i = 0; i < 4; ++i) o_[i] = XMODE == 1 ? xa_[i] - xb_[i] : xa_[i];     \
            half_put((img) + OFF_B, st0, PB, o_);                                                            \
            if (FUSE) {                                                                                      \
                float4* ep_ = reinterpret_cast<float4*>(reinterpret_cast<float*>((img) + OFF_E) + se0);      \
                float4 e4_ = *ep_;                                                                           \
                e4_.x += raw.ea.x - raw.eb.x; e4_.y += raw.ea.y - raw.eb.y;                                  \
                e4_.z += raw.ea.z - raw.eb.z; e4_.w += raw.ea.w - raw.eb.w;                                  \
                *ep_ = e4_;                                                                                  \
            }                                                                                                \
        }                                                                                                    \
    } while (0)
#define TWO_ISSUE_MAIN(SL, orow_)                                                                            \
    do {                                                                                                     \
        const size_t gp_ = a.gate_plane;                                                                     \
        const float* g0_ = a.gates + (size_t)(orow_) * H + f4;                                               \
        if ((SL) == 0) {                                                                                     \
            if (UP & 1) raw.dh = *reinterpret_cast<const float4*>(a.up.d_hout + (size_t)(orow_) * a.up.ld_dhout + f4); \
            if (UP & 2) raw.dy = a.up.dy[(orow_)];                                                           \
            raw.hn = TWO_LD4(g0_ + 3 * gp_);                                                                 \
            raw.r = TWO_LD4(g0_);                                                                            \
        } else if ((SL) == 1) {                                                                              \
            raw.n = TWO_LD4(g0_ + 2 * gp_);                                                                  \
            raw.z = TWO_LD4(g0_ + gp_);                                                                      \
        } else if ((SL) == 2) {                                                                              \
            raw.hp = *reinterpret_cast<const float4*>(a.h + (size_t)(orow_) * a.ld_h + f4);                  \
        }                                                                                                    \
    } while (0)
#define TWO_ISSUE_GATHER(gs_, gd_)                                                                           \
    do {                                                                                                     \
        if (XMODE == 0) raw.xa = *reinterpret_cast<const float4*>(a.msg + (size_t)(gs_) * a.ld_msg + f4);    \
        if (XMODE != 0) {                                                                                    \
            raw.xa = *reinterpret_cast<const float4*>(a.h + (size_t)(gs_) * a.ld_h + f4);                    \
            if (XMODE == 1) raw.xb = *reinterpret_cast<const float4*>(a.h + (size_t)(gd_) * a.ld_h + f4);    \
            if (FUSE) {                                                                                      \
                raw.ea = *reinterpret_cast<const float4*>(a.add_msg + (size_t)(gs_) * a.ld_add + f4);        \
                raw.eb = *reinterpret_cast<const float4*>(a.add_msg + (size_t)(gd_) * a.ld_add + f4);        \
            }                                                                                                \
        }                                                                                                    \
    } while (0)
#define TWO_GATHER_IDS(lp_, gs_, gd_)                                                                        \
    do {                                                                                                     \
        if (XMODE == 0) { (gs_) = a.msg_compact ? (lp_) : a.rows[(lp_)]; (gd_) = 0; }                        \
        else { (gs_) = a.src[(lp_)]; (gd_) = a.dst[(lp_)]; }                                                 \
    } while (0)

    bool valid_cur, valid_n;
    int gs_cur, gd_cur;
    int orow_n;
    {
        bool v0, v1;
        const int lp0 = row_of(blockIdx.x, true, v0);
        const int o0 = a.rows[lp0];
        TWO_GATHER_IDS(lp0, gs_cur, gd_cur);
        TWO_ISSUE_MAIN(0, o0); TWO_ISSUE_MAIN(1, o0); TWO_ISSUE_MAIN(2, o0); TWO_ISSUE_GATHER(gs_cur, gd_cur);
        const int lp1 = row_of(blockIdx.x + G, 1 < nmine, v1);
        const int o1 = a.rows[lp1];
        TWO_SLICE(0, lds16, v0); TWO_ISSUE_MAIN(0, o1);
        TWO_SLICE(1, lds16, v0); TWO_ISSUE_MAIN(1, o1);
        TWO_SLICE(2, lds16, v0); TWO_ISSUE_MAIN(2, o1);
        TWO_SLICE(3, lds16, v0);
        TWO_SLICE(5, lds16, v0);
        valid_cur = v1;
        TWO_GATHER_IDS(lp1, gs_cur, gd_cur);
        const int lp2 = row_of(blockIdx.x + 2 * G, 2 < nmine, valid_n);
        orow_n = a.rows[lp2];
    }
    __syncthreads();

#define TWO_STAGE(ROLE_)                                                                                     \
    do {                                                                                                     \
        if (!(exp_ & 2)) TWO_SLICE(s6, nxt, valid_cur);                                                      \
        if (!(exp_ & 1)) {                                                                                   \
            TWO_ISSUE_MAIN(s6, orow_n);                                                                      \
             \
             \
            if (s6 == 3) TWO_ISSUE_GATHER(gs_cur, gd_cur);                                                   \
        }                                                                                                    \
        if (TWO_SCHED == 0) __builtin_amdgcn_sched_barrier(0);                                               \
    } while (0)
    for (int it = 0; it < nmine; ++it) {
        const int tile = blockIdx.x + it * G;
        uint16_t* const cur = lds16 + (it & 1) * BUF;
        uint16_t* const nxt = lds16 + ((it & 1) ^ 1) * BUF;
        const int er0 = a.rows[min(tile * 32 + j16, a.R - 1)], er1 = a.rows[min(tile * 32 + 16 + j16, a.R - 1)];
        const bool el0 = tile * 32 + j16 < a.R, el1 = tile * 32 + 16 + j16 < a.R;
        f32x4 accd[2];
#pragma unroll
        for (int i = 0; i < 4; ++i) { accd[0][i] = 0.f; accd[1][i] = 0.f; }
#pragma unroll
        for (int s6 = 0; s6 < 6; ++s6) {
            const int kb = s6 / 3, j = s6 % 3;
            uint4 bd[3], aw[3], bt[3];
            const uint16_t* pd;
            {
                const int chunk = s6 < 4 ? 4 * kq + s6 : 4 * (s6 - 4) + kq;
                int inrow = (chunk ^ swzj) << 3;
                if (s6 >= 4) inrow ^= hix;
                pd = cur + (s6 >= 4 ? SUB : 0) + rowj + inrow;
            }
            {
                const uint16_t* p0 = cur + kb * 2048 + offB;
                const uint16_t* p1 = cur + kb * 2048 + (offB ^ 8) + 4 * 128;
#pragma unroll
                for (int pc = 0; pc < 3; ++pc) {
                    const uint2 u0 = lds_read_tr(p0 + pc * PB), u1 = lds_read_tr(p1 + pc * PB);
                    bt[pc] = make_uint4(u0.x, u0.y, u1.x, u1.y);
                }
            }
            {
                const uint16_t* p0 = cur + kb * 2048 + offA[j];
                const uint16_t* p1 = cur + kb * 2048 + (offA[j] ^ 8) + 4 * 128;
#pragma unroll
                for (int pc = 0; pc < 3; ++pc) {
                    const uint2 u0 = lds_read_tr(p0 + pc * PA), u1 = lds_read_tr(p1 + pc * PA);
                    aw[pc] = make_uint4(u0.x, u0.y, u1.x, u1.y);
                }
            }
            TWO_MARK(0);
            if (TWO_SCHED >= 1) TWO_STAGE(0);
            TWO_MARK(1);
            if (!(exp_ & 4)) {
            acc[j] = mfma32_c<0>(aw, bt, acc[j]); acc[j] = mfma32_c<1>(aw, bt, acc[j]);
            acc[j] = mfma32_c<2>(aw, bt, acc[j]); acc[j] = mfma32_c<3>(aw, bt, acc[j]);
            acc[j] = mfma32_c<4>(aw, bt, acc[j]); acc[j] = mfma32_c<5>(aw, bt, acc[j]);
            } else { acc[j][0] += __uint_as_float(aw[0].x ^ bt[0].x ^ aw[1].y ^ bt[1].y ^ aw[2].z ^ bt[2].z); }
            if (HHS && kb == tt && !(exp_ & 8)) {
#pragma unroll
                for (int pc = 0; pc < 3; ++pc) {
                    const uint4 v = aw[pc];
                    bsum[j] = dot2_ones(v.x, bsum[j]); bsum[j] = dot2_ones(v.y, bsum[j]);
                    bsum[j] = dot2_ones(v.z, bsum[j]); bsum[j] = dot2_ones(v.w, bsum[j]);
                }
            }
            if (TWO_SCHED == 0) __builtin_amdgcn_sched_barrier(0);
            TWO_MARK(2);
#pragma unroll
            for (int pc = 0; pc < 3; ++pc) bd[pc] = *reinterpret_cast<const uint4*>(pd + pc * PA);
            if (!(exp_ & 4)) {
            accd[0] = mfma16_c<0>(wq[s6], bd, accd[0]); accd[0] = mfma16_c<1>(wq[s6], bd, accd[0]);
            accd[0] = mfma16_c<2>(wq[s6], bd, accd[0]); accd[0] = mfma16_c<3>(wq[s6], bd, accd[0]);
            accd[0] = mfma16_c<4>(wq[s6], bd, accd[0]); accd[0] = mfma16_c<5>(wq[s6], bd, accd[0]);
            } else { accd[0][0] += __uint_as_float(bd[0].x ^ bd[1].y ^ bd[2].z); }
            if (TWO_SCHED == 0) __builtin_amdgcn_sched_barrier(0);
#pragma unroll
            for (int pc = 0; pc < 3; ++pc) bd[pc] = *reinterpret_cast<const uint4*>(pd + pc * PA + 16 * 128);
            if (!(exp_ & 4)) {
            accd[1] = mfma16_c<0>(wq[s6], bd, accd[1]); accd[1] = mfma16_c<1>(wq[s6], bd, accd[1]);
            accd[1] = mfma16_c<2>(wq[s6], bd, accd[1]); accd[1] = mfma16_c<3>(wq[s6], bd, accd[1]);
            accd[1] = mfma16_c<4>(wq[s6], bd, accd[1]); accd[1] = mfma16_c<5>(wq[s6], bd, accd[1]);
            } else { accd[1][0] += __uint_as_float(bd[0].x ^ bd[1].y ^ bd[2].z); }
            if (TWO_SCHED == 0) __builtin_amdgcn_sched_barrier(0);
            if (TWO_SCHED == 0) TWO_STAGE(0);
            __builtin_amdgcn_sched_barrier(0);
            TWO_MARK(3);
        }
        {
            bool vnn;
            const int lp2 = row_of(tile + 2 * G, it + 2 < nmine, vnn);
            TWO_GATHER_IDS(lp2, gs_cur, gd_cur);
            valid_cur = valid_n;
            const int lp3 = row_of(tile + 3 * G, it + 3 < nmine, valid_n);
            orow_n = a.rows[lp3];
            (void)vnn;
        }
        int cofs = n0 + 4 * kq;
        asm volatile("" : "+v"(cofs));
        if (exp_ & 16) {
            if (accd[0][0] + accd[1][1] + (float)er0 + (float)er1 == 123.456f) a.d_msg[cofs] = 1.f;
        } else if (role == 0) {
            if (el0) *reinterpret_cast<float4*>(a.d_msg + ((size_t)er0 * a.ld_dmsg + cofs)) =
                         make_float4(accd[0][0], accd[0][1], accd[0][2], accd[0][3]);
            if (el1) *reinterpret_cast<float4*>(a.d_msg + ((size_t)er1 * a.ld_dmsg + cofs)) =
                         make_float4(accd[1][0], accd[1][1], accd[1][2], accd[1][3]);
        } else if (HHS) {
            const float* e = reinterpret_cast<const float*>(cur + OFF_E);
            const int cq = cofs >> 2;
            const float4 x0 = *reinterpret_cast<const float4*>(e + j16 * 64 + ((cq ^ j16) << 2));
            const float4 x1 = *reinterpret_cast<const float4*>(e + (16 + j16) * 64 + ((cq ^ j16) << 2));
            if (el0) *reinterpret_cast<float4*>(a.d_h + ((size_t)er0 * a.ld_dh + cofs)) =
                         make_float4(accd[0][0] + x0.x, accd[0][1] + x0.y, accd[0][2] + x0.z, accd[0][3] + x0.w);
            if (el1) *reinterpret_cast<float4*>(a.d_h + ((size_t)er1 * a.ld_dh + cofs)) =
                         make_float4(accd[1][0] + x1.x, accd[1][1] + x1.y, accd[1][2] + x1.z, accd[1][3] + x1.w);
        }
        TWO_MARK(4);
        __syncthreads();
        TWO_MARK(5);
    }
#undef TWO_STAGE
#undef TWO_GATHER_IDS
#undef TWO_ISSUE_GATHER
#undef TWO_ISSUE_MAIN
#undef TWO_SLICE
    float* sw = a.slab_w + (size_t)blockIdx.x * (3 * H) * (2 * H);
    if (HHS || role == 0) {
#pragma unroll
        for (int j = 0; j < 3; ++j)
#pragma unroll
            for (int reg = 0; reg < 16; ++reg) {
                const int jj = (jt0 + j) * 32 + acc_row(reg, half);
                sw[(size_t)jj * (2 * H) + role * H + tt * 32 + c32] = acc[j][reg];
            }
    }
    {
        float* red = lds;
#pragma unroll
        for (int j = 0; j < 3; ++j) {
            const float tot = bsum[j] + __shfl_xor(bsum[j], 32);
            if (half == 0) red[wave * 96 + j * 32 + c32] = tot;
        }
        __syncthreads();
        if (HHS && tt == 0 && half == 0) {
            float* sb = a.slab_b + (size_t)blockIdx.x * 6 * H;
#pragma unroll
            for (int j = 0; j < 3; ++j)
                sb[role * 3 * H + (jt0 + j) * 32 + c32] = red[wave * 96 + j * 32 + c32] + red[(wave + 1) * 96 + j * 32 + c32];
        }
    }
}

template <int UP>
__global__ __launch_bounds__(512) void k_gru_bwd_zs(GruBwdFusedArgs a, const float* __restrict__ b_hn, int ntiles) {
    constexpr int H = 64;
    constexpr int SUB = 32 * 128;
    constexpr int PA = 2 * SUB, PB = SUB;
    constexpr int OFF_B = 3 * PA;
    constexpr int BUF = OFF_B + 3 * PB;
    extern __shared__ float lds[];
    uint16_t* const lds16 = reinterpret_cast<uint16_t*>(lds);
    const int tid = threadIdx.x;
    const int wave = __builtin_amdgcn_readfirstlane(tid >> 6), lane = tid & 63;
    const int role = wave >> 2, q = wave & 3;
    const int j16 = lane & 15, kq = lane >> 4;
    const int srow = 4 * wave + kq, f4 = 4 * j16;
    const int n0 = 16 * q;
    uint4 wq[6][3];
#pragma unroll
    for (int s6 = 0; s6 < 6; ++s6) {
        const int ch = s6 < 4 ? 4 * kq + s6 : 16 + 4 * (s6 - 4) + kq;
        float v[8];
#pragma unroll
        for (int i = 0; i < 8; ++i) v[i] = a.w_ih[(size_t)(8 * ch + i) * a.ld_wih + n0 + j16];
        const Split8 sp = split8_arr(v);
        wq[s6][0] = sp.p1; wq[s6][1] = sp.p2; wq[s6][2] = sp.p3;
    }
    const float headl = (UP & 2) ? a.up.w_head[lane] : 0.f;
    const float4 bhn = *reinterpret_cast<const float4*>(b_hn + f4);
    const int st0 = dui_off(srow, f4);
    const int swzj = dui_swz(j16), rowj = (16 * role + j16) * 128;
    const int half = lane >> 5, c32 = lane & 31;
    const int jt0 = (q >> 1) * 3, tt = q & 1;
    const int i16 = lane & 15, tq = i16 >> 2, tp = i16 & 3, tg = (lane >> 4) & 1;
    const int trow = (8 * half + tq) * 128, tsw0 = (tq << 2) | (2 * half);
    const int kofs = role * 2048;
    int offA[3], offB;
#pragma unroll
    for (int j = 0; j < 3; ++j) {
        const int col = (jt0 + j) * 32;
        const int ch = ((col & 127) >> 3) + 2 * tg + (tp >> 1);
        offA[j] = kofs + (col >> 7) * SUB + trow + ((ch ^ tsw0) << 3) + 4 * (tp & 1);
    }
    {
        const int ch = ((tt * 32) >> 3) + 2 * tg + (tp >> 1);
        offB = kofs + OFF_B + trow + ((ch ^ tsw0) << 3) + 4 * (tp & 1);
    }
    f32x16 acc[3];
#pragma unroll
    for (int j = 0; j < 3; ++j)
#pragma unroll
        for (int i = 0; i < 16; ++i) acc[j][i] = 0.f;
    float bs_r[4] = {0.f, 0.f, 0.f, 0.f}, bs_z[4] = {0.f, 0.f, 0.f, 0.f};
    float bs_n[4] = {0.f, 0.f, 0.f, 0.f}, bs_nr[4] = {0.f, 0.f, 0.f, 0.f};

    const int G = gridDim.x;
    const int nmine = (ntiles - (int)blockIdx.x + G - 1) / G;
    struct { float4 dh, r, z, n, xa, xb; float dy; } raw;
    float d0[4], tv[4];
    auto row_of = [&](int tile, bool tvld, bool& vld) -> int {
        const int lr = tile * 32 + srow;
        vld = tvld && lr < a.R;
        return vld ? lr : a.R - 1;
    };
#define ZS_SLICE(SL, img, vld)                                                                               \
    do {                                                                                                     \
        float o_[4];                                                                                         \
        if ((SL) == 0) {                                                                                     \
            const float dh_[4] = {raw.dh.x, raw.dh.y, raw.dh.z, raw.dh.w}, r_[4] = {raw.r.x, raw.r.y, raw.r.z, raw.r.w}; \
            const float z_[4] = {raw.z.x, raw.z.y, raw.z.z, raw.z.w}, n_[4] = {raw.n.x, raw.n.y, raw.n.z, raw.n.w}; \
            const float hn_[4] = {bhn.x, bhn.y, bhn.z, bhn.w};                                               \
            _Pragma("unroll") for (int i = 0; i < 4; ++i) {                                                  \
                float d_ = (UP & 1) ? dh_[i] : 0.f;                                                          \
                if (UP & 2) d_ += raw.dy * __shfl(headl, f4 + i);                                            \
                d0[i] = (vld) ? d_ : 0.f;                                                                    \
                tv[i] = d0[i] * (1.0f - z_[i]) * (1.0f - n_[i] * n_[i]);                                     \
                const float q_ = tv[i] * r_[i];                                                              \
                o_[i] = q_ * hn_[i] * (1.0f - r_[i]);                                                        \
                bs_r[i] += o_[i]; bs_n[i] += tv[i]; bs_nr[i] += q_;                                          \
            }                                                                                                \
            half_put((img), st0, PA, o_);                                                                    \
        } else if ((SL) == 1) {                                                                              \
            const float z_[4] = {raw.z.x, raw.z.y, raw.z.z, raw.z.w}, n_[4] = {raw.n.x, raw.n.y, raw.n.z, raw.n.w}; \
            _Pragma("unroll") for (int i = 0; i < 4; ++i) {                                                  \
                o_[i] = d0[i] * (0.0f - n_[i]) * z_[i] * (1.0f - z_[i]);                                     \
                bs_z[i] += o_[i];                                                                            \
            }                                                                                                \
            half_put((img), st0 ^ 64, PA, o_);                                                               \
        } else if ((SL) == 3) {                                                                              \
            half_put((img), SUB + st0, PA, tv);                                                              \
        } else if ((SL) == 5) {                                                                              \
            const float xa_[4] = {raw.xa.x, raw.xa.y, raw.xa.z, raw.xa.w}, xb_[4] = {raw.xb.x, raw.xb.y, raw.xb.z, raw.xb.w}; \
            _Pragma("unroll") for (int i = 0; i < 4; ++i) o_[i] = xa_[i] - xb_[i];                           \
            half_put((img) + OFF_B, st0, PB, o_);                                                            \
        }                                                                                                    \
    } while (0)
#define ZS_ISSUE_MAIN(SL, orow_)                                                                             \
    do {                                                                                                     \
        const size_t gp_ = a.gate_plane;                                                                     \
        const float* g0_ = a.gates + (size_t)(orow_) * H + f4;                                               \
        if ((SL) == 0) {                                                                                     \
            if (UP & 1) raw.dh = *reinterpret_cast<const float4*>(a.up.d_hout + (size_t)(orow_) * a.up.ld_dhout + f4); \
            if (UP & 2) raw.dy = a.up.dy[(orow_)];                                                           \
            raw.r = TWO_LD4(g0_);                                                                            \
        } else if ((SL) == 1) {                                                                              \
            raw.n = TWO_LD4(g0_ + 2 * gp_);                                                                  \
            raw.z = TWO_LD4(g0_ + gp_);                                                                      \
        }                                                                                                    \
    } while (0)
#define ZS_ISSUE_GATHER(gs_, gd_)                                                                            \
    do {                                                                                                     \
        raw.xa = *reinterpret_cast<const float4*>(a.h + (size_t)(gs_) * a.ld_h + f4);                        \
        raw.xb = *reinterpret_cast<const float4*>(a.h + (size_t)(gd_) * a.ld_h + f4);                        \
    } while (0)

    bool valid_cur, valid_n;
    int gs_cur, gd_cur;
    int orow_n;
    {
        bool v0, v1;
        const int lp0 = row_of(blockIdx.x, true, v0);
        const int o0 = a.rows[lp0];
        gs_cur = a.src[lp0]; gd_cur = a.dst[lp0];
        ZS_ISSUE_MAIN(0, o0); ZS_ISSUE_MAIN(1, o0); ZS_ISSUE_GATHER(gs_cur, gd_cur);
        const int lp1 = row_of(blockIdx.x + G, 1 < nmine, v1);
        const int o1 = a.rows[lp1];
        ZS_SLICE(0, lds16, v0); ZS_ISSUE_MAIN(0, o1);
        ZS_SLICE(1, lds16, v0); ZS_ISSUE_MAIN(1, o1);
        ZS_SLICE(3, lds16, v0);
        ZS_SLICE(5, lds16, v0);
        valid_cur = v1;
        gs_cur = a.src[lp1]; gd_cur = a.dst[lp1];
        const int lp2 = row_of(blockIdx.x + 2 * G, 2 < nmine, valid_n);
        orow_n = a.rows[lp2];
    }
    __syncthreads();

    for (int it = 0; it < nmine; ++it) {
        const int tile = blockIdx.x + it * G;
        uint16_t* const cur = lds16 + (it & 1) * BUF;
        uint16_t* const nxt = lds16 + ((it & 1) ^ 1) * BUF;
        const int er = a.rows[min(tile * 32 + 16 * role + j16, a.R - 1)];
        const bool el = tile * 32 + 16 * role + j16 < a.R;
        f32x4 accd;
#pragma unroll
        for (int i = 0; i < 4; ++i) accd[i] = 0.f;
// ... 6 lines not shown
                pd = cur + (s6 >= 4 ? SUB : 0) + rowj + ((chunk ^ swzj) << 3);
            }
            if (s6 < 3) {
                uint4 aw[3], bt[3];
                {
                    const uint16_t* p0 = cur + offB;
                    const uint16_t* p1 = cur + (offB ^ 8) + 4 * 128;
#pragma unroll
                    for (int pc = 0; pc < 3; ++pc) {
                        const uint2 u0 = lds_read_tr(p0 + pc * PB), u1 = lds_read_tr(p1 + pc * PB);
                        bt[pc] = make_uint4(u0.x, u0.y, u1.x, u1.y);
                    }
                }
                const uint16_t* p0 = cur + offA[s6];
                const uint16_t* p1 = cur + (offA[s6] ^ 8) + 4 * 128;
#pragma unroll
                for (int pc = 0; pc < 3; ++pc) {
                    const uint2 u0 = lds_read_tr(p0 + pc * PA), u1 = lds_read_tr(p1 + pc * PA);
                    aw[pc] = make_uint4(u0.x, u0.y, u1.x, u1.y);
                }
                ZS_SLICE(s6, nxt, valid_cur);
                ZS_ISSUE_MAIN(s6, orow_n);
                acc[s6] = mfma32_c<0>(aw, bt, acc[s6]); acc[s6] = mfma32_c<1>(aw, bt, acc[s6]);
                acc[s6] = mfma32_c<2>(aw, bt, acc[s6]); acc[s6] = mfma32_c<3>(aw, bt, acc[s6]);
                acc[s6] = mfma32_c<4>(aw, bt, acc[s6]); acc[s6] = mfma32_c<5>(aw, bt, acc[s6]);
            } else {
                ZS_SLICE(s6, nxt, valid_cur);
                if (s6 == 3) ZS_ISSUE_GATHER(gs_cur, gd_cur);
            }
#pragma unroll
            for (int pc = 0; pc < 3; ++pc) bd[pc] = *reinterpret_cast<const uint4*>(pd + pc * PA);
            accd = mfma16_c<0>(wq[s6], bd, accd); accd = mfma16_c<1>(wq[s6], bd, accd);
            accd = mfma16_c<2>(wq[s6], bd, accd); accd = mfma16_c<3>(wq[s6], bd, accd);
            accd = mfma16_c<4>(wq[s6], bd, accd); accd = mfma16_c<5>(wq[s6], bd, accd);
            __builtin_amdgcn_sched_barrier(0);
        }
        {
            bool vnn;
            const int lp2 = row_of(tile + 2 * G, it + 2 < nmine, vnn);
            gs_cur = a.src[lp2]; gd_cur = a.dst[lp2];
            valid_cur = valid_n;
            const int lp3 = row_of(tile + 3 * G, it + 3 < nmine, valid_n);
            orow_n = a.rows[lp3];
            (void)vnn;
        }
        int cofs = n0 + 4 * kq;
        asm volatile("" : "+v"(cofs));
        if (el) *reinterpret_cast<float4*>(a.d_msg + ((size_t)er * a.ld_dmsg + cofs)) =
                    make_float4(accd[0], accd[1], accd[2], accd[3]);
        __syncthreads();
    }
#undef ZS_ISSUE_GATHER
#undef ZS_ISSUE_MAIN
#undef ZS_SLICE
    float* sw = a.slab_w + (size_t)blockIdx.x * (3 * H) * (2 * H);
#pragma unroll
    for (int j = 0; j < 3; ++j)
#pragma unroll
        for (int reg = 0; reg < 16; ++reg) {
            const int jj = (jt0 + j) * 32 + acc_row(reg, half);
            sw[(size_t)jj * (2 * H) + role * H + tt * 32 + c32] = acc[j][reg];
        }
    {
        float* red = lds;
        *reinterpret_cast<float4*>(red + srow * 256 + 0 * 64 + f4) = make_float4(bs_r[0], bs_r[1], bs_r[2], bs_r[3]);
        *reinterpret_cast<float4*>(red + srow * 256 + 1 * 64 + f4) = make_float4(bs_z[0], bs_z[1], bs_z[2], bs_z[3]);
        *reinterpret_cast<float4*>(red + srow * 256 + 2 * 64 + f4) = make_float4(bs_n[0], bs_n[1], bs_n[2], bs_n[3]);
        *reinterpret_cast<float4*>(red + srow * 256 + 3 * 64 + f4) = make_float4(bs_nr[0], bs_nr[1], bs_nr[2], bs_nr[3]);
        __syncthreads();
        if (tid < 256) {
            float s = 0.f;
            for (int r = 0; r < 32; ++r) s += red[r * 256 + tid];
            float* sb = a.slab_b + (size_t)blockIdx.x * 6 * H;
            const int g = tid >> 6, c = tid & 63;
            if (g < 3) sb[g * H + c] = s;
            if (g != 2) sb[3 * H + (g == 3 ? 2 : g) * H + c] = s;
        }
    }
}


__global__ void k_gru_reduce_w(const float* __restrict__ slab_w, const float* __restrict__ slab_b, int n_rs,
                               int IN, int H, float* __restrict__ dW_ih, float* __restrict__ dW_hh,
                               float* __restrict__ db_ih, float* __restrict__ db_hh) {
    const int XH = IN + H;
    const size_t nW = (size_t)3 * H * XH;
    const size_t i = (size_t)blockIdx.x * blockDim.x + threadIdx.x;
    if (i < nW) {
        float s = 0.f;
        for (int k = 0; k < n_rs; ++k) s += slab_w[(size_t)k * nW + i];
        const int j = (int)(i / XH), col = (int)(i % XH);
        if (col < IN) dW_ih[(size_t)j * IN + col] += s;
        else dW_hh[(size_t)j * H + (col - IN)] += s;
    } else if (i < nW + (size_t)6 * H) {
        const int b = (int)(i - nW);
        float s = 0.f;
        for (int k = 0; k < n_rs; ++k) s += slab_b[(size_t)k * 6 * H + b];
        if (b < 3 * H) db_ih[b] += s;
        else db_hh[b - 3 * H] += s;
    }
}

__global__ void k_gru_reduce_w_half(const float* __restrict__ slab_w, const float* __restrict__ slab_b, int n_rs, int H,
                                    float* __restrict__ dW_ih, int ld_dwih, float* __restrict__ dW_hh,
                                    float* __restrict__ db_ih, float* __restrict__ db_hh, int full) {
    const int XH = 2 * H;
    const size_t nW = (size_t)3 * H * XH;
    const size_t i = (size_t)blockIdx.x * blockDim.x + threadIdx.x;
    if (i < nW) {
        const int j = (int)(i / XH), col = (int)(i % XH);
        if (col >= H && !full) return;
        float s = 0.f;
        for (int k = 0; k < n_rs; ++k) s += slab_w[(size_t)k * nW + i];
        if (col < H) dW_ih[(size_t)j * ld_dwih + col] += s;
        else dW_hh[(size_t)j * H + (col - H)] += s;
    } else if (full && i < nW + (size_t)6 * H) {
        const int b = (int)(i - nW);
        float s = 0.f;
        for (int k = 0; k < n_rs; ++k) s += slab_b[(size_t)k * 6 * H + b];
        if (b < 3 * H) db_ih[b] += s;
        else db_hh[b - 3 * H] += s;
    }
}

__global__ void k_fold_slabs_gru(const float* __restrict__ slabs, size_t stride, int nslab, float* __restrict__ out,
                                 size_t n) {
    const size_t i = (size_t)blockIdx.x * blockDim.x + threadIdx.x;
    if (i >= n) return;
    const int k0 = blockIdx.y * 32, k1 = min(nslab, k0 + 32);
    float s = 0.f;
#pragma unroll 8
    for (int k = k0; k < k1; ++k) s += slabs[(size_t)k * stride + i];
    out[(size_t)blockIdx.y * n + i] = s;
}

__global__ void k_gru_reduce_w_zs(const float* __restrict__ slab_w, const float* __restrict__ slab_b, int n_rs, int H,
                                  float* __restrict__ dW_ih, float* __restrict__ db_ih, float* __restrict__ db_hh) {
    const size_t nI = (size_t)3 * H * H, nW = 2 * nI;
    const size_t i = (size_t)blockIdx.x * blockDim.x + threadIdx.x;
    if (i < nI) {
        const size_t o = (i / H) * (2 * H) + (i % H);
        float s = 0.f;
        for (int k = 0; k < n_rs; ++k) s += slab_w[(size_t)k * nW + o] + slab_w[(size_t)k * nW + o + H];
        dW_ih[i] += s;
    } else if (i < nI + (size_t)6 * H) {
        const int b = (int)(i - nI);
        float s = 0.f;
        for (int k = 0; k < n_rs; ++k) s += slab_b[(size_t)k * 6 * H + b];
        if (b < 3 * H) db_ih[b] += s;
        else db_hh[b - 3 * H] += s;
    }
}


static int weights_variant_default() {
    static const int v = [] {
        if (!split_enabled()) return 0;
        const char* e = getenv("TMPNN_SPLIT_WEIGHTS");
        return (e && e[0] == '0') ? 0 : 1;
    }();
    return v;
}
static void plan_weights(int R, int IN, int H, int* n_rs, int* RS, int* NQ, int* NCH) {
    *NQ = 3 * H / 32;
    *NCH = (IN + H + 127) / 128;
    long per = (long)(*NQ) * (*NCH);
    long want = 4096 / per;
    if (want < 1) want = 1;
    long by_rows = (R + 63) / 64;
    long n = by_rows < want ? by_rows : want;
    if (n < 1) n = 1;
    long rs = (R + n - 1) / n;
    rs = (rs + 1) & ~1L;
    if (rs < 2) rs = 2;
    n = (R + rs - 1) / rs;
    if (n < 1) n = 1;
    *n_rs = (int)n;
    *RS = (int)rs;
}

}

using namespace tmpnn;

extern "C" {

int tmpnn_gru_bwd_data(const int32_t* rows, int R, int IN, const float* h, int ld_h, int H, const float* w_ih,
                       const float* w_hh, const float* gates, size_t gate_plane, const float* d_hout, int ld_dhout,
                       const float* dy, const float* w_head, float* d_msg, int ld_dmsg, float* d_h, int ld_dh,
                       const int32_t* add_src, const int32_t* add_dst, const float* add_msg, int ld_add,
                       tmpnn_stream stream) {
    TM_REQUIRE(supported_H_cell(H), "gru_bwd_data: unsupported H=%d", H);
    if (R == 0) return TMPNN_OK;
    TM_REQUIRE(R > 0 && IN > 0 && IN % 32 == 0 && (H % 64 != 0 || IN % 64 == 0), "gru_bwd_data: R=%d IN=%d", R, IN);
    TM_REQUIRE(rows && h && w_ih && w_hh && gates && d_msg && d_h, "gru_bwd_data: null pointer");
    TM_REQUIRE(d_hout != nullptr || dy != nullptr, "gru_bwd_data: no upstream gradient (d_hout and dy both null)");
    TM_REQUIRE(dy == nullptr || (w_head != nullptr && aligned16(w_head)), "gru_bwd_data: dy needs a 16-byte aligned w_head");
    TM_REQUIRE((ld_h & 3) == 0 && aligned16(h) && aligned16(gates) && (gate_plane & 3) == 0 &&
                   (d_hout == nullptr || ((ld_dhout & 3) == 0 && aligned16(d_hout) && ld_dhout >= H)),
               "gru_bwd_data: rows must be 16-byte aligned");
    TM_REQUIRE(ld_dmsg >= IN && ld_dh >= H && ld_h >= H, "gru_bwd_data: leading dimension too small");
    TM_REQUIRE(add_msg == nullptr || (add_src && add_dst && ld_add >= H), "gru_bwd_data: fused aggregation adjoint args");
    GruBwdDataArgs a{rows, R, IN, h, ld_h, H, w_ih, w_hh, gates, gate_plane, DhSrc{d_hout, ld_dhout, dy, w_head},
                     d_msg, ld_dmsg, d_h, ld_dh, add_src, add_dst, add_msg, ld_add};
    hipStream_t st = as_stream(stream);
    if (H <= 64 && (IN == H || IN == 2 * H) && aligned16(w_ih) && aligned16(w_hh) && aligned16(d_msg) &&
        (ld_dmsg & 3) == 0 && aligned16(d_h) && (ld_dh & 3) == 0 &&
        (add_msg == nullptr || (aligned16(add_msg) && (ld_add & 3) == 0))) {
        const int ntiles = ceil_div(R, 256);
        dim3 pgrid(ntiles < 256 ? ntiles : 256), pblock(512);
        const size_t shm = sizeof(float) * ((size_t)(IN + H) * 3 * H + 4);
        const int up = (d_hout ? 1 : 0) | (dy ? 2 : 0);
        const bool fuse = add_msg != nullptr;
        if (split_enabled() && IN == H) {
            const size_t shm2 = (size_t)3 * (IN + H) * (3 * H + 8) * 2 + 16 + sizeof(float) * H;
#define S3(HH, UU, FF)                                                                                       \
    do {                                                                                                     \
        TM_SHM_ONCE((k_gru_bwd_data_split<HH, UU, FF>), shm2);                    \
        hipLaunchKernelGGL((k_gru_bwd_data_split<HH, UU, FF>), pgrid, pblock, shm2, st, a, ntiles);          \
    } while (0)
#define SL(HH)                                                                                               \
    do {                                                                                                     \
        if (fuse) { if (up == 1) S3(HH, 1, true); else if (up == 2) S3(HH, 2, true); else S3(HH, 3, true); }      \
        else      { if (up == 1) S3(HH, 1, false); else if (up == 2) S3(HH, 2, false); else S3(HH, 3, false); }   \
    } while (0)
            if (H == 64) SL(64); else SL(32);
#undef SL
#undef S3
            return check_launch("gru_bwd_data_split");
        }
#define L3(HH, II, UU, FF)                                                                                   \
    do {                                                                                                     \
        TM_SHM_ONCE((k_gru_bwd_data_lds<HH, II, UU, FF>), shm);                     \
        hipLaunchKernelGGL((k_gru_bwd_data_lds<HH, II, UU, FF>), pgrid, pblock, shm, st, a, ntiles);         \
    } while (0)
#define LL(HH, II)                                                                                           \
    do {                                                                                                     \
        if (fuse) { if (up == 1) L3(HH, II, 1, true); else if (up == 2) L3(HH, II, 2, true); else L3(HH, II, 3, true); }      \
        else      { if (up == 1) L3(HH, II, 1, false); else if (up == 2) L3(HH, II, 2, false); else L3(HH, II, 3, false); }   \
    } while (0)
        if (H == 64) { if (IN == 64) LL(64, 64); else LL(64, 128); }
        else         { if (IN == 32) LL(32, 32); else LL(32, 64); }
#undef LL
#undef L3
        return check_launch("gru_bwd_data_lds");
    }
    int NT = (H % 128 == 0 && IN % 128 == 0) ? 4 : (H % 64 == 0) ? 2 : 1;
    if (NT > 1 && (long)ceil_div(R, 128) * ((IN + H) / (32 * NT)) < 128) NT = 1;
    dim3 grid(ceil_div(R, 128), (IN + H) / (32 * NT)), block(256);
    if (NT == 4) hipLaunchKernelGGL((k_gru_bwd_data<4>), grid, block, 0, st, a);
    else if (NT == 2) hipLaunchKernelGGL((k_gru_bwd_data<2>), grid, block, 0, st, a);
    else hipLaunchKernelGGL((k_gru_bwd_data<1>), grid, block, 0, st, a);
    return check_launch("gru_bwd_data");
}

static bool weights_use_lds(int IN, int H) { return H == 64 && IN == H; }
static int weights_lds_blocks(int R) {
    const int ntiles = ceil_div(R, 32);
    return ntiles < 512 ? ntiles : 512;
}

static bool weights_use_chunk(int IN, int H) { return H % 64 == 0 && IN % 64 == 0 && !weights_use_lds(IN, H); }
static int weights_chunk_slabs(int R, int IN, int H) {
    const int ntiles = ceil_div(R, 32);
    const int per = (H / 64) * ceil_div(IN + H, 128);
    int want = 1024 / per;
    if (want < 1) want = 1;
    return ntiles < want ? ntiles : want;
}


#ifdef TMPNN_KEEP_VARIANTS
static bool fused_two_waves() {
    static const bool v = [] { const char* e = getenv("TMPNN_BWD_TWO"); return e == nullptr || e[0] != '0'; }();
    return v;
}
#endif

static int fused_blocks(int R) {
    const int ntiles = ceil_div(R, 32);
    return ntiles < 256 ? ntiles : 256;
}

static bool device_gives_160k() {
    static std::atomic<int> cache[16];
    int dev = 0;
    (void)hipGetDevice(&dev);
    int v = cache[dev & 15].load(std::memory_order_relaxed);
    if (v == 0) {
        int bytes = 0;
        if (hipDeviceGetAttribute(&bytes, hipDeviceAttributeMaxSharedMemoryPerBlock, dev) != hipSuccess) bytes = 0;
        v = bytes >= 163840 ? 1 : 2;
        cache[dev & 15].store(v, std::memory_order_relaxed);
    }
    return v == 1;
}

int tmpnn_gru_bwd_fused_available(int H, int IN, int xmode) {
#ifdef TMPNN_KEEP_VARIANTS
    if (xmode == 2 && !fused_two_waves()) return 0;
#endif
    return (H == 64 && ((IN == 64 && (xmode == 0 || xmode == 1)) || (IN == 128 && xmode == 2)) && device_gives_160k()) ? 1 : 0;
}

size_t tmpnn_gru_bwd_fused_ws(int R, int IN, int H) {
    if (R <= 0) return 0;
    const int n = fused_blocks(R);
    const size_t per = (size_t)3 * H * (IN + H) + (size_t)6 * H;
    return ((size_t)n * per + reduce_slabs_ws_floats(n, per)) * sizeof(float);
}

static int gru_bwd_fused_concat(GruBwdFusedArgs a, int R, int H, const int32_t* src, const int32_t* dst, const float* w_ih,
                                float* d_msg, float* dW_ih, float* dW_hh, float* db_ih, float* db_hh, float* fold, int up,
                                bool fuse, hipStream_t st) {
    const int n_rs = fused_blocks(R);
    const int ntiles = ceil_div(R, 32);
    const size_t shm = 163840;
    const size_t nW = (size_t)3 * H * 2 * H, nB = (size_t)6 * H;
    int rc;
    for (int half = 0; half < 2; ++half) {
        a.src = half == 0 ? src : dst;
        a.dst = half == 0 ? dst : src;
        a.w_ih = w_ih + (size_t)half * H;
        a.ld_wih = 2 * H;
        a.d_msg = d_msg + (size_t)half * H;
#define LC(U, F, S)                                                                                          \
    do {                                                                                                     \
        TM_SHM_ONCE((k_gru_bwd_two<2, U, F, S>), shm);                                                       \
        hipLaunchKernelGGL((k_gru_bwd_two<2, U, F, S>), dim3(n_rs), dim3(512), shm, st, a, ntiles);          \
    } while (0)
#define LCU(F, S) do { if (up == 1) LC(1, F, S); else if (up == 2) LC(2, F, S); else LC(3, F, S); } while (0)
        if (half == 0) { if (fuse) LCU(true, true); else LCU(false, true); }
        else LCU(false, false);
#undef LCU
#undef LC
        if ((rc = check_launch("gru_bwd_fused_concat"))) return rc;
        const float* rw = a.slab_w;
        const float* rb = a.slab_b;
        int nred = n_rs;
        if (n_rs > 64) {
            const int ng = ceil_div(n_rs, 32);
            float* fw = fold;
            float* fb = fold + (size_t)ng * nW;
            hipLaunchKernelGGL(k_fold_slabs_gru, dim3(ceil_div((long)nW, 256), ng), dim3(256), 0, st, a.slab_w, nW, n_rs, fw, nW);
            if (half == 0)
                hipLaunchKernelGGL(k_fold_slabs_gru, dim3(ceil_div((long)nB, 256), ng), dim3(256), 0, st, a.slab_b, nB, n_rs, fb, nB);
            if ((rc = check_launch("gru_fold"))) return rc;
            rw = fw; rb = fb; nred = ng;
        }
        hipLaunchKernelGGL(k_gru_reduce_w_half, dim3(ceil_div((long)(nW + nB), 256)), dim3(256), 0, st, rw, rb, nred, H,
                           dW_ih + (size_t)half * H, 2 * H, dW_hh, db_ih, db_hh, half == 0 ? 1 : 0);
        if ((rc = check_launch("gru_reduce_w_half"))) return rc;
    }
    return TMPNN_OK;
}

int tmpnn_gru_bwd_fused(const int32_t* rows, int R, int xmode, const int32_t* src, const int32_t* dst, const float* msg,
                        int ld_msg, int msg_compact, int IN, const float* h, int ld_h, int H, const float* w_ih,
                        const float* w_hh, const float* gates, size_t gate_plane, const float* d_hout, int ld_dhout,
                        const float* dy, const float* w_head, float* d_msg, int ld_dmsg, float* d_h, int ld_dh,
                        const int32_t* add_src, const int32_t* add_dst, const float* add_msg, int ld_add, float* dW_ih,
                        float* dW_hh, float* db_ih, float* db_hh, void* ws, size_t ws_bytes, tmpnn_stream stream) {
    TM_REQUIRE(tmpnn_gru_bwd_fused_available(H, IN, xmode), "gru_bwd_fused: H=%d IN=%d xmode=%d not supported", H, IN, xmode);
    if (R == 0) return TMPNN_OK;
    TM_REQUIRE(R > 0 && rows && h && w_ih && w_hh && gates && d_msg && d_h && dW_ih && dW_hh && db_ih && db_hh,
               "gru_bwd_fused: null pointer");
    TM_REQUIRE(d_hout != nullptr || dy != nullptr, "gru_bwd_fused: no upstream gradient");
    TM_REQUIRE(dy == nullptr || (w_head != nullptr && aligned16(w_head)), "gru_bwd_fused: dy needs a 16-byte aligned w_head");
    TM_REQUIRE(xmode == 0 ? (msg != nullptr && (ld_msg & 3) == 0 && aligned16(msg) && ld_msg >= IN) : (src && dst),
               "gru_bwd_fused: message source");
    TM_REQUIRE((ld_h & 3) == 0 && aligned16(h) && aligned16(gates) && (gate_plane & 3) == 0 && aligned16(w_ih) &&
                   aligned16(w_hh) && (d_hout == nullptr || ((ld_dhout & 3) == 0 && aligned16(d_hout))) &&
                   (ld_dmsg & 3) == 0 && aligned16(d_msg) && (ld_dh & 3) == 0 && aligned16(d_h) &&
                   (add_msg == nullptr || ((ld_add & 3) == 0 && aligned16(add_msg) && add_src && add_dst)),
               "gru_bwd_fused: rows must be 16-byte aligned");
    TM_REQUIRE(xmode == 0 || add_msg == nullptr || (add_src == src && add_dst == dst),
               "gru_bwd_fused: with xmode != 0 the fused adjoint gathers through src / dst (pass the same arrays)");
    const size_t need = tmpnn_gru_bwd_fused_ws(R, IN, H);
    if (ws == nullptr || ws_bytes < need)
        return set_error(TMPNN_EWORKSPACE, "gru_bwd_fused: workspace %zu < %zu bytes", ws_bytes, need);
    const int n_rs = fused_blocks(R);
    const size_t nW = (size_t)3 * H * (IN + H), nB = (size_t)6 * H;
    float* slab_w = reinterpret_cast<float*>(ws);
    float* slab_b = slab_w + (size_t)n_rs * nW;
    float* fold = slab_b + (size_t)n_rs * nB;
    GruBwdFusedArgs a{rows, R, src, dst, msg, ld_msg, msg_compact, h, ld_h, w_ih, w_hh, gates, gate_plane,
                      DhSrc{d_hout, ld_dhout, dy, w_head}, d_msg, ld_dmsg, d_h, ld_dh, add_src, add_dst, add_msg, ld_add,
                      slab_w, slab_b, IN};
    const int ntiles = ceil_div(R, 32);
    const size_t shm = 163840;
    hipStream_t st = as_stream(stream);
    const int up = (d_hout ? 1 : 0) | (dy ? 2 : 0);
    const bool fuse = add_msg != nullptr;
    if (xmode == 2) {
        TM_REQUIRE(ld_dmsg >= 2 * H, "gru_bwd_fused: the concat cell writes d_msg [.., 2H]");
        float* sb = slab_w + (size_t)n_rs * 3 * H * 2 * H;
        a.slab_b = sb;
        return gru_bwd_fused_concat(a, R, H, src, dst, w_ih, d_msg, dW_ih, dW_hh, db_ih, db_hh, sb + (size_t)n_rs * nB, up,
                                    fuse, st);
    }
#ifdef TMPNN_KEEP_VARIANTS
#define LF(X, U, F)                                                                                          \
    do {                                                                                                     \
        if (fused_two_waves() && !((X) == 0 && (F))) {      \
            TM_SHM_ONCE((k_gru_bwd_two<X, U, F>), shm);                                                      \
            hipLaunchKernelGGL((k_gru_bwd_two<X, U, F>), dim3(n_rs), dim3(512), shm, st, a, ntiles);         \
        } else {                                                                                             \
            TM_SHM_ONCE((k_gru_bwd_one<X, U, F>), shm);                                                      \
            hipLaunchKernelGGL((k_gru_bwd_one<X, U, F>), dim3(n_rs), dim3(256), shm, st, a, ntiles);         \
        }                                                                                                    \
    } while (0)
#else
    TM_REQUIRE(!(xmode == 0 && fuse), "gru_bwd_fused: xmode 0 with a fused adjoint needs a TMPNN_KEEP_VARIANTS build");
#define LF(X, U, F)                                                                                          \
    do {                                                                                                     \
        if (!((X) == 0 && (F))) {                                                                            \
            TM_SHM_ONCE((k_gru_bwd_two<X, U, F>), shm);                                                      \
            hipLaunchKernelGGL((k_gru_bwd_two<X, U, F>), dim3(n_rs), dim3(512), shm, st, a, ntiles);         \
        }                                                                                                    \
    } while (0)
#endif
#define LU(X, F) do { if (up == 1) LF(X, 1, F); else if (up == 2) LF(X, 2, F); else LF(X, 3, F); } while (0)
    if (xmode == 0) { if (fuse) LU(0, true); else LU(0, false); }
    else            { if (fuse) LU(1, true); else LU(1, false); }
#undef LU
#undef LF
    int rc = check_launch("gru_bwd_fused");
    if (rc) return rc;
    const float* rw = slab_w;
    const float* rb = slab_b;
    int nred = n_rs;
    if (n_rs > 64) {
        const int ng = ceil_div(n_rs, 32);
        float* fw = fold;
        float* fb = fold + (size_t)ng * nW;
        hipLaunchKernelGGL(k_fold_slabs_gru, dim3(ceil_div((long)nW, 256), ng), dim3(256), 0, st, slab_w, nW, n_rs, fw, nW);
        hipLaunchKernelGGL(k_fold_slabs_gru, dim3(ceil_div((long)nB, 256), ng), dim3(256), 0, st, slab_b, nB, n_rs, fb, nB);
        if ((rc = check_launch("gru_fold"))) return rc;
        rw = fw; rb = fb; nred = ng;
    }
    hipLaunchKernelGGL(k_gru_reduce_w, dim3(ceil_div((long)(nW + nB), 256)), dim3(256), 0, st, rw, rb, nred, IN, H,
                       dW_ih, dW_hh, db_ih, db_hh);
    return check_launch("gru_reduce_w");
}

int tmpnn_gru_bwd_fused_zero_state_available(int H, int IN, int xmode) {
    return (H == 64 && IN == 64 && xmode == 1 && device_gives_160k()) ? 1 : 0;
}

int tmpnn_gru_bwd_fused_zero_state(const int32_t* rows, int R, const int32_t* src, const int32_t* dst, int IN,
                                   const float* h, int ld_h, int H, const float* w_ih, const float* b_hn,
                                   const float* gates, size_t gate_plane, const float* d_hout, int ld_dhout,
                                   const float* dy, const float* w_head, float* d_msg, int ld_dmsg, float* dW_ih,
                                   float* db_ih, float* db_hh, void* ws, size_t ws_bytes, tmpnn_stream stream) {
    TM_REQUIRE(tmpnn_gru_bwd_fused_zero_state_available(H, IN, 1), "gru_bwd_fused_zero_state: H=%d IN=%d not supported", H, IN);
    if (R == 0) return TMPNN_OK;
    TM_REQUIRE(R > 0 && rows && src && dst && h && w_ih && b_hn && gates && d_msg && dW_ih && db_ih && db_hh,
               "gru_bwd_fused_zero_state: null pointer");
    TM_REQUIRE(d_hout != nullptr || dy != nullptr, "gru_bwd_fused_zero_state: no upstream gradient");
    TM_REQUIRE(dy == nullptr || (w_head != nullptr && aligned16(w_head)),
               "gru_bwd_fused_zero_state: dy needs a 16-byte aligned w_head");
    TM_REQUIRE((ld_h & 3) == 0 && aligned16(h) && aligned16(gates) && (gate_plane & 3) == 0 && aligned16(w_ih) &&
                   aligned16(b_hn) && (d_hout == nullptr || ((ld_dhout & 3) == 0 && aligned16(d_hout))) &&
                   (ld_dmsg & 3) == 0 && aligned16(d_msg) && ld_dmsg >= IN && ld_h >= H,
               "gru_bwd_fused_zero_state: rows must be 16-byte aligned");
    const size_t need = tmpnn_gru_bwd_fused_ws(R, IN, H);
    if (ws == nullptr || ws_bytes < need)
        return set_error(TMPNN_EWORKSPACE, "gru_bwd_fused_zero_state: workspace %zu < %zu bytes", ws_bytes, need);
    const int n_rs = fused_blocks(R);
    const size_t nW = (size_t)3 * H * (IN + H), nB = (size_t)6 * H;
    float* slab_w = reinterpret_cast<float*>(ws);
    float* slab_b = slab_w + (size_t)n_rs * nW;
    float* fold = slab_b + (size_t)n_rs * nB;
    GruBwdFusedArgs a{rows, R, src, dst, nullptr, 0, 0, h, ld_h, w_ih, nullptr, gates, gate_plane,
                      DhSrc{d_hout, ld_dhout, dy, w_head}, d_msg, ld_dmsg, nullptr, 0, nullptr, nullptr, nullptr, 0,
                      slab_w, slab_b, IN};
    const int ntiles = ceil_div(R, 32);
    const size_t shm = 147456;
    hipStream_t st = as_stream(stream);
    const int up = (d_hout ? 1 : 0) | (dy ? 2 : 0);
#define LZ(U)                                                                                                \
    do {                                                                                                     \
        TM_SHM_ONCE((k_gru_bwd_zs<U>), shm);                                                                 \
        hipLaunchKernelGGL((k_gru_bwd_zs<U>), dim3(n_rs), dim3(512), shm, st, a, b_hn, ntiles);              \
    } while (0)
    if (up == 1) LZ(1); else if (up == 2) LZ(2); else LZ(3);
#undef LZ
    int rc = check_launch("gru_bwd_fused_zero_state");
    if (rc) return rc;
    const float* rw = slab_w;
    const float* rb = slab_b;
    int nred = n_rs;
    if (n_rs > 64) {
        const int ng = ceil_div(n_rs, 32);
        float* fw = fold;
        float* fb = fold + (size_t)ng * nW;
        hipLaunchKernelGGL(k_fold_slabs_gru, dim3(ceil_div((long)nW, 256), ng), dim3(256), 0, st, slab_w, nW, n_rs, fw, nW);
        hipLaunchKernelGGL(k_fold_slabs_gru, dim3(ceil_div((long)nB, 256), ng), dim3(256), 0, st, slab_b, nB, n_rs, fb, nB);
        if ((rc = check_launch("gru_fold"))) return rc;
        rw = fw; rb = fb; nred = ng;
    }
    hipLaunchKernelGGL(k_gru_reduce_w_zs, dim3(ceil_div((long)(3 * H * H + nB), 256)), dim3(256), 0, st, rw, rb, nred, H,
                       dW_ih, db_ih, db_hh);
    return check_launch("gru_reduce_w_zs");
}

#ifdef TMPNN_KEEP_VARIANTS
int tmpnn_gru_bwd_weights_choice(void) { return weights_variant_default(); }
#endif

size_t tmpnn_gru_bwd_weights_ws(int R, int IN, int H) {
    if (R <= 0) return 0;
    int n_rs, RS, NQ, NCH;
    plan_weights(R, IN, H, &n_rs, &RS, &NQ, &NCH);
    if (weights_use_lds(IN, H)) n_rs = std::max(n_rs, weights_lds_blocks(R));
    if (weights_use_chunk(IN, H)) n_rs = std::max(n_rs, weights_chunk_slabs(R, IN, H));
    const size_t per = (size_t)3 * H * (IN + H) + (size_t)6 * H;
    return ((size_t)n_rs * per + reduce_slabs_ws_floats(n_rs, per)) * sizeof(float);
}

int tmpnn_gru_bwd_weights(const int32_t* rows, int R, int xmode, const int32_t* src, const int32_t* dst,
                          const float* msg, int ld_msg, int msg_compact, int IN, const float* h, int ld_h, int H,
                          const float* gates,
                          size_t gate_plane, const float* d_hout, int ld_dhout, const float* dy, const float* w_head,
                          float* dW_ih, float* dW_hh,
                          float* db_ih, float* db_hh, void* ws, size_t ws_bytes, tmpnn_stream stream) {
    return tmpnn_gru_bwd_weights_variant(rows, R, xmode, src, dst, msg, ld_msg, msg_compact, IN, h, ld_h, H, gates,
                                         gate_plane, d_hout, ld_dhout, dy, w_head, dW_ih, dW_hh, db_ih, db_hh, ws,
                                         ws_bytes, -1, stream);
}

int tmpnn_gru_bwd_weights_variant(const int32_t* rows, int R, int xmode, const int32_t* src, const int32_t* dst,
                                  const float* msg, int ld_msg, int msg_compact, int IN, const float* h, int ld_h, int H,
                                  const float* gates,
                                  size_t gate_plane, const float* d_hout, int ld_dhout, const float* dy,
                                  const float* w_head, float* dW_ih, float* dW_hh,
                                  float* db_ih, float* db_hh, void* ws, size_t ws_bytes, int variant,
                                  tmpnn_stream stream) {
    TM_REQUIRE(variant >= -1 && variant <= 1, "gru_bwd_weights: variant %d (need -1, 0 or 1)", variant);
    TM_REQUIRE(supported_H_cell(H), "gru_bwd_weights: unsupported H=%d", H);
    if (R == 0) return TMPNN_OK;
    TM_REQUIRE(R > 0 && xmode >= 0 && xmode <= 2 && IN % 32 == 0 && IN > 0, "gru_bwd_weights: R=%d xmode=%d IN=%d", R,
               xmode, IN);
    TM_REQUIRE(IN == (xmode == 2 ? 2 * H : (xmode == 1 ? H : IN)), "gru_bwd_weights: IN=%d vs xmode=%d", IN, xmode);
    TM_REQUIRE(rows && h && gates && dW_ih && dW_hh && db_ih && db_hh, "gru_bwd_weights: null pointer");
    TM_REQUIRE(d_hout != nullptr || dy != nullptr, "gru_bwd_weights: no upstream gradient");
    TM_REQUIRE(dy == nullptr || (w_head != nullptr && aligned16(w_head)), "gru_bwd_weights: dy needs a 16-byte aligned w_head");
    TM_REQUIRE(xmode == 0 ? msg != nullptr : (src != nullptr && dst != nullptr), "gru_bwd_weights: message source");
    const size_t need = tmpnn_gru_bwd_weights_ws(R, IN, H);
    if (ws == nullptr || ws_bytes < need)
        return set_error(TMPNN_EWORKSPACE, "gru_bwd_weights: workspace %zu < %zu bytes", ws_bytes, need);
    int n_rs, RS, NQ, NCH;
    plan_weights(R, IN, H, &n_rs, &RS, &NQ, &NCH);
    const bool vec_ok = (ld_h & 3) == 0 && (d_hout == nullptr || ((ld_dhout & 3) == 0 && aligned16(d_hout))) &&
                        aligned16(h) && aligned16(gates) && (gate_plane & 3) == 0 &&
                        (xmode != 0 || ((ld_msg & 3) == 0 && aligned16(msg)));
    const bool use_lds = weights_use_lds(IN, H) && xmode != 2 && vec_ok;
    const bool use_chunk = weights_use_chunk(IN, H) && vec_ok;
    if (use_lds) n_rs = weights_lds_blocks(R);
    if (use_chunk) n_rs = weights_chunk_slabs(R, IN, H);
    const size_t nW = (size_t)3 * H * (IN + H), nB = (size_t)6 * H;
    float* slab_w = reinterpret_cast<float*>(ws);
    float* slab_b = slab_w + (size_t)n_rs * nW;
    float* fold = slab_b + (size_t)n_rs * nB;
    GruBwdWArgs a{rows, R, src, dst, msg, ld_msg, IN, msg_compact, h, ld_h, H, gates, gate_plane,
                  DhSrc{d_hout, ld_dhout, dy, w_head}, slab_w, slab_b,
                  n_rs, RS, NQ, NCH};
    hipStream_t st = as_stream(stream);
    int rc;
    if (use_lds) {
        const int ntiles = ceil_div(R, 32);
        dim3 grid(n_rs), block(256);
        const size_t shm = (size_t)3 * 32 * (256 + 128) * 2 + sizeof(float) * 64;
        const int up = (d_hout ? 1 : 0) | (dy ? 2 : 0);
        auto launch_split = [&]() {
#define SW(X, U)                                                                                             \
    do {                                                                                                     \
        TM_SHM_ONCE((k_gru_bwd_weights_split<X, U>), shm);                     \
        hipLaunchKernelGGL((k_gru_bwd_weights_split<X, U>), grid, block, shm, st, a, ntiles);                \
    } while (0)
            if (xmode == 0) { if (up == 1) SW(0, 1); else if (up == 2) SW(0, 2); else SW(0, 3); }
            else            { if (up == 1) SW(1, 1); else if (up == 2) SW(1, 2); else SW(1, 3); }
#undef SW
        };
        auto launch_f32 = [&]() {
#define LW(X, U) hipLaunchKernelGGL((k_gru_bwd_weights_lds<64, X, U>), grid, block, 0, st, a, ntiles)
            if (xmode == 0) { if (up == 1) LW(0, 1); else if (up == 2) LW(0, 2); else LW(0, 3); }
            else            { if (up == 1) LW(1, 1); else if (up == 2) LW(1, 2); else LW(1, 3); }
#undef LW
        };
        const int choice = (H == 64 && split_enabled()) ? (variant < 0 ? weights_variant_default() : variant) : 0;
        if (choice != 0) {
            launch_split();
            rc = check_launch("gru_bwd_weights_split");
        } else {
            launch_f32();
// ... 41 lines not shown
```

### trackmpnn_amd/functional.py

```python
from __future__ import annotations

import contextlib
import ctypes
import os
from dataclasses import dataclass
from typing import Dict, List, Optional, Sequence, Tuple

import torch

from . import _lib
from .graph import CallPlan, dense_seg_plan, edge_tiles, win_plan

ATT_DROPOUT_P = 0.5
INPLACE_GRADS = os.environ.get('TMPNN_INPLACE_GRADS', '0') == '1'
FUSED_BWD = os.environ.get('TMPNN_FUSED_BWD', '1') == '1'
ZERO_STATE_BWD = os.environ.get('TMPNN_BWD_ZERO_STATE', '1') != '0'
ZERO_STATE_FWD = os.environ.get('TMPNN_FWD_ZERO_STATE', '1') != '0'
WIDE_OVERLAP = os.environ.get('TMPNN_WIDE_OVERLAP', '0') == '1' and os.environ.get('TMPNN_KEEP_VARIANTS', '0') == '1'
ATT_KMAX = 8
_SPLIT = os.environ.get('TMPNN_SPLIT', '1')[:1] != '0'

_VARIANTS = os.environ.get('TMPNN_KEEP_VARIANTS', '0') == '1'


def _variant(name: str, default: str) -> str:
    return os.environ.get(name, default) if _VARIANTS else default


WIDE_DW = _variant('TMPNN_WIDE_DW', '1') == '1'
WIDE_DET = _variant('TMPNN_WIDE_DET', '1') == '1'
WIDE = _variant('TMPNN_WIDE', '1') != '0' and _SPLIT
WIDE_TILED = _variant('TMPNN_WIDE_TILED', '1') != '0'
FWD_TILED = _variant('TMPNN_FWD_TILED', '1') != '0' and _SPLIT
FWD_TILE_ROWS = 16 if _variant('TMPNN_FWD_TILE_ROWS', '32') == '16' else 32
INPUT_TF = _variant('TMPNN_INPUT_TF', '1') != '0'
RECOMPUTE_GATES = _variant('TMPNN_RECOMPUTE_GATES', '0') == '1'
CONCAT_PROJ = _variant('TMPNN_CONCAT_PROJ', '1') != '0'
WIN_SEGSUM = _variant('TMPNN_SEGSUM_WIN', '0') == '1'
WIDE_FUSED_ADJOINT = _variant('TMPNN_WIDE_FUSED_ADJOINT', '1') != '0'
_aux_streams: Dict[torch.device, 'torch.cuda.Stream'] = {}


def _aux_stream(dev) -> Optional[int]:
    if not WIDE_OVERLAP or torch.cuda.is_current_stream_capturing():
        return None
    key = torch.device(dev)
    s = _aux_streams.get(key)
    if s is None:
        s = torch.cuda.Stream(key)
        _aux_streams[key] = s
    if s.cuda_stream == torch.cuda.current_stream(key).cuda_stream:
        return None
    return s.cuda_stream


def _seg_plan_guard(g, dev, on_aux: bool) -> None:
    plan = g.__dict__.get('_seg_plan')
    if plan is None or torch.cuda.is_current_stream_capturing():
        return
    cur = _aux_streams[torch.device(dev)] if on_aux else torch.cuda.current_stream(dev)
    last = plan.__dict__.get('_last_stream')
    if last is not None and last.cuda_stream != cur.cuda_stream:
        ev = torch.cuda.Event()
        ev.record(last)
        cur.wait_event(ev)
    plan._last_stream = cur


_aux_events: Dict[torch.device, tuple] = {}


def _aux_event_pair(dev):
    key = torch.device(dev)
    ev = _aux_events.get(key)
    if ev is None:
        with torch.cuda.device(key):
            ev = (torch.cuda.Event(enable_timing=False), torch.cuda.Event(enable_timing=False))
            for e in ev:
                e.record(torch.cuda.current_stream(key))
        _aux_events[key] = ev
    return ev


_wide_ws: Dict[torch.device, torch.Tensor] = {}


def _wide_workspace(nbytes: int, dev, slot: int = 0) -> torch.Tensor:
    key = (torch.device(dev), slot)
    ws = _wide_ws.get(key)
    if ws is None or ws.numel() * 4 < nbytes + 16:
        _wide_ws.pop(key, None)
        ws = torch.empty((nbytes // 4 + 4,), dtype=torch.float32, device=dev)
        _wide_ws[key] = ws
    return ws


def _input_tf(plan: CallPlan, H: int, F: int) -> bool:
    return (INPUT_TF and plan.max_seg_nd >= 0 and plan.seg_of_det is not None
            and bool(_lib.load().tmpnn_input_tf_supported(H, F, plan.max_seg_nd)))


_weight_images = None


@contextlib.contextmanager
def weight_cache():
    global _weight_images
    prev = _weight_images
    _weight_images = {}
    try:
        yield
    finally:
        _weight_images = prev


def _cached(key, sources, build):
    if _weight_images is None:
        return build()
    hit = _weight_images.get(key)
    if hit is None:
        hit = _weight_images[key] = (sources, build())
    return hit[1]


def _wide_prep(w_ih: torch.Tensor, w_hh: torch.Tensor, H: int) -> torch.Tensor:
    def build():
        nb = int(_lib.load().tmpnn_wide_prep_bytes(H, H))
        prep = torch.empty((nb // 4 + 4,), dtype=torch.float32, device=w_ih.device)
        _lib.call('tmpnn_wide_prepare', w_ih.data_ptr(), w_hh.data_ptr(), H, H, prep.data_ptr(), _stream())
        return prep
    return _cached(('wide', w_ih.data_ptr(), w_hh.data_ptr(), H), (w_ih, w_hh), build)


@dataclass(frozen=True)
class ModelSpec:
    groups: Tuple[Tuple[str, int], ...]
    H: int
    K: int
    msg_type: str

    @property
    def G(self) -> int:
        return len(self.groups)

    @property
    def IN_e(self) -> int:
        return 2 * self.H if self.msg_type == 'concat' else self.H

    @property
    def F_total(self) -> int:
        return sum(f for _, f in self.groups)

    def param_names(self) -> List[str]:
        names = []
        for g in range(self.G):
            t = f'input_transforms.{g}.'
            names += [t + '0.weight', t + '0.bias', t + '1.weight', t + '1.bias', t + '3.weight', t + '3.bias']
        for g in range(self.G):
            f = f'factor_grus.{g}.'
            names += [f + 'edge_gru.weight_ih', f + 'edge_gru.weight_hh', f + 'edge_gru.bias_ih', f + 'edge_gru.bias_hh']
            for k in range(self.K):
                names += [f + f'gat.{k}.W_att', f + f'gat.{k}.a']
            names += [f + 'node_gru.weight_ih', f + 'node_gru.weight_hh', f + 'node_gru.bias_ih', f + 'node_gru.bias_hh']
        names += ['output_transform_node.weight', 'output_transform_node.bias',
                  'output_transform_edge.weight', 'output_transform_edge.bias']
        return names


def _stream() -> int:
    return _lib.raw_stream()
# ... 167 lines not shown
        wn_g = (w_node.data_ptr() + 4 * gi * H) if cw > 0 else None
        e_wih_t, e_whh_t = _transpose(P[f + 'edge_gru.weight_ih']), _transpose(P[f + 'edge_gru.weight_hh'])
        n_wih_t, n_whh_t = _transpose(P[f + 'node_gru.weight_ih']), _transpose(P[f + 'node_gru.weight_hh'])
        st_det, aux_obj = st, None
        if use_wide and K == 0:
            aux = _aux_stream(dev)
            if aux is not None:
                aux_obj = _aux_streams[torch.device(dev)]
                fork, _ = _aux_event_pair(dev)
                fork.record(torch.cuda.current_stream(dev))
                aux_obj.wait_event(fork)
                st_det = aux
        if use_wide:
            prep = _wide_prep(P[f + 'edge_gru.weight_ih'], P[f + 'edge_gru.weight_hh'], H)
            wide_preps.append(prep)
            proj = torch.empty((Dn, 3 * H), **opts)
            if WIDE_TILED:
                _lib.call('tmpnn_wide_gru_fwd_tiled', prep.data_ptr(), g.det_row.data_ptr(), Dn, edge_tiles(g, 128).cref(), E,
                          hg, GH, H, P[f + 'edge_gru.bias_ih'].data_ptr(), P[f + 'edge_gru.bias_hh'].data_ptr(),
                          proj.data_ptr(), og, GH, gp, plane, st)
            else:
                _lib.call('tmpnn_wide_gru_fwd', prep.data_ptr(), g.det_row.data_ptr(), Dn, g.edge_row.data_ptr(), E,
                          g.src_pos.data_ptr(), g.dst_pos.data_ptr(), hg, GH, H,
                          P[f + 'edge_gru.bias_ih'].data_ptr(), P[f + 'edge_gru.bias_hh'].data_ptr(),
                          proj.data_ptr(), og, GH, gp, plane, st)
        elif use_proj_cat:
            proj = torch.empty((2 * Dn, 3 * H), **opts)
            _lib.call('tmpnn_rows_linear', g.det_row.data_ptr(), Dn, hg, GH, H, e_wih_t.data_ptr(), 3 * H,
                      proj.data_ptr(), 3 * H, st)
            w2n = _cached(('negt', e_wih_t.data_ptr(), H), (e_wih_t,), lambda: e_wih_t[H:].neg().contiguous())
            _lib.call('tmpnn_rows_linear', g.det_row.data_ptr(), Dn, hg, GH, H, w2n.data_ptr(), 3 * H,
                      proj.data_ptr() + 4 * Dn * 3 * H, 3 * H, st)
            _lib.call('tmpnn_gru_fwd_tiles', edge_tiles(g, FWD_TILE_ROWS, dst_offset=Dn).cref(), E, proj.data_ptr(), 3 * H, hg, GH,
                      H, e_whh_t.data_ptr(), P[f + 'edge_gru.bias_ih'].data_ptr(), P[f + 'edge_gru.bias_hh'].data_ptr(),
                      og, GH, gp, plane, we_g, part_g, N, st)
        elif use_proj:
            proj = torch.empty((Dn, 3 * H), **opts)
            _lib.call('tmpnn_rows_linear', g.det_row.data_ptr(), Dn, hg, GH, H, e_wih_t.data_ptr(), 3 * H,
                      proj.data_ptr(), 3 * H, st)
            if FWD_TILED and E > 0:
                recompute = RECOMPUTE_GATES and save
                E_full = E_old if zs_fwd else E
                if E_full > 0:
                    tiles = edge_tiles(g, FWD_TILE_ROWS, e1=E_full)
                    _lib.call('tmpnn_gru_fwd_tiles', tiles.cref(), E_full, proj.data_ptr(), 3 * H, hg, GH, H,
                              e_whh_t.data_ptr(), P[f + 'edge_gru.bias_ih'].data_ptr(), P[f + 'edge_gru.bias_hh'].data_ptr(),
                              og, GH, None if recompute else gp, plane, we_g, part_g, N, st)
                if zs_fwd:
                    _lib.call('tmpnn_gru_fwd_tiles_zero_state', edge_tiles(g, FWD_TILE_ROWS, e0=E_old).cref(), E - E_old,
                              proj.data_ptr(), 3 * H, H, P[f + 'edge_gru.bias_ih'].data_ptr(),
                              P[f + 'edge_gru.bias_hh'].data_ptr(), og, GH, gp, plane, int(save and not zs_bwd), we_g,
                              part_g, N, st)
                if recompute:
                    saved.setdefault('proj', {})[gi] = (proj, e_whh_t)
            else:
                _lib.call('tmpnn_gru_fwd', g.edge_row.data_ptr(), E, 3, g.src_pos.data_ptr(), g.dst_pos.data_ptr(),
                          proj.data_ptr(), 3 * H, 0, H, hg, GH, H, None, e_whh_t.data_ptr(),
                          P[f + 'edge_gru.bias_ih'].data_ptr(), P[f + 'edge_gru.bias_hh'].data_ptr(),
                          og, GH, gp, plane, we_g, part_g, N, st)
        else:
            _lib.call('tmpnn_gru_fwd', g.edge_row.data_ptr(), E, xmode, g.src.data_ptr(), g.dst.data_ptr(),
                      None, 0, 0, spec.IN_e, hg, GH, H,
                      e_wih_t.data_ptr(), e_whh_t.data_ptr(),
                      P[f + 'edge_gru.bias_ih'].data_ptr(), P[f + 'edge_gru.bias_hh'].data_ptr(),
                      og, GH, gp, plane, we_g, part_g, N, st)
        es = es_all[gi]
        if K == 0:
            _seg_plan_guard(g, dev, aux_obj is not None)
            _lib.call('tmpnn_segsum_fwd_live', g.cref(), hg, GH, es.data_ptr(), H, H, 1, zero_from, st_det)
            alphas.append(None)
        else:
            erec, inc_other = g.att_index() if E > 0 else (None, None)
            groups, al = [], []
            for k0 in range(0, K, ATT_KMAX):
                Kg = min(ATT_KMAX, K - k0)
                Ws = [P[f + f'gat.{k}.W_att'] for k in range(k0, k0 + Kg)]
                As = [P[f + f'gat.{k}.a'] for k in range(k0, k0 + Kg)]
                W = _cached(('attW', tuple(t.data_ptr() for t in Ws)), tuple(Ws), lambda: torch.cat(Ws, 1).contiguous())
                a = _cached(('atta', tuple(t.data_ptr() for t in As)), tuple(As),
                            lambda: torch.stack([t.reshape(-1) for t in As]).contiguous())
                ws_ha = torch.empty((max(Dn, 1), Kg * H), **opts)
                score = torch.empty((max(2 * E, 1), Kg), **opts)
                stats = torch.empty((max(Dn, 1), Kg, 2), **opts)
                esk = torch.empty((Kg, max(Dn, 1), H), **opts)
                alpha = torch.empty((Kg, max(2 * E, 1)), **opts)
                kp = None
                if training:
                    kp = _keep_bits(None if keep is None else keep[gi][k0:k0 + Kg], Kg, 2 * E, dev)
                out_g = es if Kg == K else torch.empty_like(es)
                _lib.call('tmpnn_att_fwd', g.cref(), _lib.ptr(erec), hg, GH, H, Kg, W.data_ptr(),
                          a.data_ptr(), _lib.ptr(kp), ATT_DROPOUT_P, ws_ha.data_ptr(), score.data_ptr(), stats.data_ptr(),
                          esk.data_ptr(), alpha.data_ptr(), out_g.data_ptr(), H, st)
                if Kg != K:
                    if k0 == 0:
                        torch.mul(out_g, Kg / K, out=es)
                    else:
                        es.add_(out_g, alpha=Kg / K)
                al += [alpha[k, :2 * E] for k in range(Kg)]
                groups.append((k0, Kg, W, a, kp, ws_ha, score, stats, esk))
            alphas.append(al)
            att_saved.append(groups)
        _lib.call('tmpnn_gru_fwd', g.det_row.data_ptr(), Dn, 0, None, None,
                  es.data_ptr(), H, 1, H, hg, GH, H,
                  n_wih_t.data_ptr(), n_whh_t.data_ptr(),
                  P[f + 'node_gru.bias_ih'].data_ptr(), P[f + 'node_gru.bias_hh'].data_ptr(),
                  og, GH, gp, plane, wn_g, part_g, N, st_det)
        if aux_obj is not None:
            _, join = _aux_event_pair(dev)
            join.record(aux_obj)
            torch.cuda.current_stream(dev).wait_event(join)
    logits = torch.empty((N, 1), **opts)
    scores = torch.empty((N, 1), **opts)
    if cw > 0:
        _lib.call('tmpnn_heads_finish', parts.data_ptr(), N, G * cw, N, g.is_edge.data_ptr(),
                  P['output_transform_node.bias'].data_ptr(), P['output_transform_edge.bias'].data_ptr(),
                  logits.data_ptr(), scores.data_ptr(), st)
    else:
        _lib.call('tmpnn_heads_fwd', h_out.data_ptr(), GH, GH, N, g.is_edge.data_ptr(),
                  P['output_transform_node.weight'].data_ptr(), P['output_transform_node.bias'].data_ptr(),
                  P['output_transform_edge.weight'].data_ptr(), P['output_transform_edge.bias'].data_ptr(),
                  logits.data_ptr(), scores.data_ptr(), st)
    if save:
        saved.update(h_cat=h_cat, gates=gates, es=es_all, att=att_saved, h_out=h_out, scores=scores,
                     wide=wide_preps if use_wide else None)
    return scores, logits, h_out, alphas, saved


def mp_backward(spec: ModelSpec, plan: CallPlan, saved: dict, P: Dict[str, torch.Tensor], training: bool,
                d_scores: Optional[torch.Tensor], d_logits: Optional[torch.Tensor], d_hout: Optional[torch.Tensor],
                need_x: bool, need_h: bool, grad_out=None):
    g = plan.graph
    H, G, K = spec.H, spec.G, spec.K
    GH = G * H
    N, E, Dn = g.N, g.E, g.Dn
    n = saved['n']
    N_old = N - n
    h_cat, gates, es_all, h_out = saved['h_cat'], saved['gates'], saved['es'], saved['h_out']
    dev = h_cat.device
    st = _stream()
    opts = dict(dtype=torch.float32, device=dev)
    names = spec.param_names()
    sizes = [P[nm].numel() for nm in names]
    offs = [0]
    for sz in sizes:
        offs.append(offs[-1] + ((sz + 63) // 64) * 64)
    if grad_out is not None:
        grads = dict(grad_out)
    else:
        flat = torch.zeros((offs[-1],), **opts)
        grads = {nm: flat[o:o + sz].view(P[nm].shape) for nm, o, sz in zip(names, offs, sizes)}

    lib = _lib.load()
    dh_up = _f32c(d_hout) if d_hout is not None else None
    dy = None
    if d_scores is not None or d_logits is not None:
        dy = torch.empty((N,), **opts)
        dl = _f32c(d_logits) if d_logits is not None else None
        ds = _f32c(d_scores) if d_scores is not None else None
        for c0 in range(0, GH, 1024):
            cw_ = min(1024, GH - c0)
            ws_b = lib.tmpnn_heads_bwd_ws(N, cw_)
            ws = torch.empty((max(ws_b // 4, 1),), **opts)
            db_n = grads['output_transform_node.bias'] if c0 == 0 else torch.zeros((1,), **opts)
            db_e = grads['output_transform_edge.bias'] if c0 == 0 else torch.zeros((1,), **opts)
            _lib.call('tmpnn_heads_bwd', h_out.data_ptr() + 4 * c0, GH, cw_, N, g.is_edge.data_ptr(),
                      P['output_transform_node.weight'].data_ptr() + 4 * c0, P['output_transform_edge.weight'].data_ptr() + 4 * c0,
                      saved['scores'].data_ptr(), _lib.ptr(dl), _lib.ptr(ds), dy.data_ptr(), None, 0, 0,
                      grads['output_transform_node.weight'].data_ptr() + 4 * c0, db_n.data_ptr(),
                      grads['output_transform_edge.weight'].data_ptr() + 4 * c0, db_e.data_ptr(),
                      ws.data_ptr(), ws_b, st)
    elif dh_up is None:
        dh_up = torch.zeros((N, GH), **opts)

    d_hcat = torch.empty((N, GH), **opts)
    IN_e = spec.IN_e
    dmsg = torch.empty((N, IN_e), **opts)
    xmode = 2 if spec.msg_type == 'concat' else 1
    plane = N * H
    ws_e = lib.tmpnn_gru_bwd_weights_ws(E, IN_e, H)
    ws_n = lib.tmpnn_gru_bwd_weights_ws(Dn, H, H)
    use_fused_bwd = (FUSED_BWD and lib.tmpnn_gru_bwd_fused_available(H, H, 0)
                     and lib.tmpnn_gru_bwd_fused_available(H, IN_e, xmode))
    ws_f = max(lib.tmpnn_gru_bwd_fused_ws(E, IN_e, H), lib.tmpnn_gru_bwd_fused_ws(Dn, H, H)) if use_fused_bwd else 0
    ws_w = torch.empty((max(ws_e, ws_n, ws_f) // 4 + 1,), **opts)
    w_node, w_edge = P['output_transform_node.weight'], P['output_transform_edge.weight']
    for gi in range(G):
        f = f'factor_grus.{gi}.'
        hg = h_cat.data_ptr() + 4 * gi * H
        dog = (dh_up.data_ptr() + 4 * gi * H) if dh_up is not None else None
        dhg = d_hcat.data_ptr() + 4 * gi * H
        gp = gates[gi].data_ptr()
        es = es_all[gi]
        dyp = _lib.ptr(dy)
        wn = (w_node.data_ptr() + 4 * gi * H) if dy is not None else None
        we = (w_edge.data_ptr() + 4 * gi * H) if dy is not None else None
        fuse = K == 0
        if use_fused_bwd:
            _lib.call('tmpnn_gru_bwd_fused', g.det_row.data_ptr(), Dn, 0, None, None, es.data_ptr(), H, 1, H,
                      hg, GH, H, P[f + 'node_gru.weight_ih'].data_ptr(), P[f + 'node_gru.weight_hh'].data_ptr(),
                      gp, plane, dog, GH, dyp, wn, dmsg.data_ptr(), IN_e, dhg, GH, None, None, None, 0,
                      grads[f + 'node_gru.weight_ih'].data_ptr(), grads[f + 'node_gru.weight_hh'].data_ptr(),
                      grads[f + 'node_gru.bias_ih'].data_ptr(), grads[f + 'node_gru.bias_hh'].data_ptr(),
                      ws_w.data_ptr(), ws_w.numel() * 4, st)
            if saved.get('proj') and gi in saved['proj']:
                proj_s, whh_t_s = saved['proj'][gi]
                h_scr = _wide_workspace(4 * N * GH, dev, slot=2)
                _lib.call('tmpnn_gru_fwd_tiles', edge_tiles(g, FWD_TILE_ROWS).cref(), E, proj_s.data_ptr(), 3 * H, hg, GH, H,
                          whh_t_s.data_ptr(), P[f + 'edge_gru.bias_ih'].data_ptr(), P[f + 'edge_gru.bias_hh'].data_ptr(),
                          h_scr.data_ptr() + 4 * gi * H, GH, gp, plane, None, None, 0, st)
            b_hn = P[f + 'edge_gru.bias_hh'].data_ptr() + 4 * 2 * H
            E_old = E - (n - int(plan.new_det_row.numel())) if n > 0 else E
            if 'zs_bwd' in saved:
                zs = saved['zs_bwd']
            else:
                zs = (ZERO_STATE_BWD and n > 0 and K == 0 and xmode == 1 and 0 <= E_old < E and b_hn % 16 == 0
                      and not (saved.get('proj') and gi in saved['proj'])
                      and lib.tmpnn_gru_bwd_fused_zero_state_available(H, IN_e, xmode))
            E_full = E_old if zs else E
            if E_full > 0:
                _lib.call('tmpnn_gru_bwd_fused', g.edge_row.data_ptr(), E_full, xmode, g.src.data_ptr(), g.dst.data_ptr(),
                          None, 0, 0, IN_e, hg, GH, H,
                          P[f + 'edge_gru.weight_ih'].data_ptr(), P[f + 'edge_gru.weight_hh'].data_ptr(),
                          gp, plane, dog, GH, dyp, we, dmsg.data_ptr(), IN_e, dhg, GH,
                          g.src.data_ptr() if fuse else None, g.dst.data_ptr() if fuse else None,
                          dmsg.data_ptr() if fuse else None, IN_e,
                          grads[f + 'edge_gru.weight_ih'].data_ptr(), grads[f + 'edge_gru.weight_hh'].data_ptr(),
                          grads[f + 'edge_gru.bias_ih'].data_ptr(), grads[f + 'edge_gru.bias_hh'].data_ptr(),
                          ws_w.data_ptr(), ws_w.numel() * 4, st)
            if zs:
                _lib.call('tmpnn_gru_bwd_fused_zero_state', g.edge_row.data_ptr() + 4 * E_old, E - E_old,
                          g.src.data_ptr() + 4 * E_old, g.dst.data_ptr() + 4 * E_old, IN_e, hg, GH, H,
                          P[f + 'edge_gru.weight_ih'].data_ptr(), b_hn, gp, plane, dog, GH, dyp, we,
                          dmsg.data_ptr(), IN_e, grads[f + 'edge_gru.weight_ih'].data_ptr(),
                          grads[f + 'edge_gru.bias_ih'].data_ptr(), grads[f + 'edge_gru.bias_hh'].data_ptr(),
                          ws_w.data_ptr(), ws_w.numel() * 4, st)
        else:
            _lib.call('tmpnn_gru_bwd_data', g.det_row.data_ptr(), Dn, H, hg, GH, H,
                      P[f + 'node_gru.weight_ih'].data_ptr(), P[f + 'node_gru.weight_hh'].data_ptr(),
                      gp, plane, dog, GH, dyp, wn, dmsg.data_ptr(), IN_e, dhg, GH, None, None, None, 0, st)
            _lib.call('tmpnn_gru_bwd_weights', g.det_row.data_ptr(), Dn, 0, None, None, es.data_ptr(), H, 1, H,
                      hg, GH, H, gp, plane, dog, GH, dyp, wn,
                      grads[f + 'node_gru.weight_ih'].data_ptr(), grads[f + 'node_gru.weight_hh'].data_ptr(),
                      grads[f + 'node_gru.bias_ih'].data_ptr(), grads[f + 'node_gru.bias_hh'].data_ptr(),
                      ws_w.data_ptr(), ws_w.numel() * 4, st)
            wide_det = bool(saved.get('wide')) and WIDE_DET
            if wide_det:
                wsb = int(lib.tmpnn_wide_gru_bwd_diff_ws(N, E, Dn, H))
                ws_wide = _wide_workspace(wsb, dev)
                aux = _aux_stream(dev)
                args = (saved['wide'][gi].data_ptr(), g.cref(), hg, GH, H, gp, plane, dog, GH, dyp, we, dhg, GH,
                        grads[f + 'edge_gru.weight_ih'].data_ptr(), grads[f + 'edge_gru.weight_hh'].data_ptr(),
                        grads[f + 'edge_gru.bias_ih'].data_ptr(), grads[f + 'edge_gru.bias_hh'].data_ptr(),
                        ws_wide.data_ptr(), wsb, st)
                evf = evj = None
                if aux is not None:
                    ef, ej = _aux_event_pair(dev)
                    evf, evj = ef.cuda_event, ej.cuda_event
                    if not evf or not evj:
                        aux = evf = evj = None
                _seg_plan_guard(g, dev, aux is not None)
                if fuse and WIDE_FUSED_ADJOINT:
                    _lib.call('tmpnn_wide_gru_bwd_diff_fused', *args[:-1], dmsg.data_ptr(), IN_e, st, aux, evf, evj)
                else:
                    if aux is not None:
                        _lib.call('tmpnn_wide_gru_bwd_diff_aux', *args, aux, evf, evj)
                    else:
                        _lib.call('tmpnn_wide_gru_bwd_diff', *args)
                    if fuse:
                        _lib.call('tmpnn_gather_diff_fwd', g.cref(), dmsg.data_ptr(), IN_e, dhg, GH, H, 1, st)
            elif saved.get('wide'):
                wsb = int(lib.tmpnn_wide_gru_bwd_data_ws(E, H))
                ws_wide = _wide_workspace(wsb, dev)
                _lib.call('tmpnn_wide_gru_bwd_data', saved['wide'][gi].data_ptr(), g.edge_row.data_ptr(), E, hg, GH, H,
                          gp, plane, dog, GH, dyp, we, dmsg.data_ptr(), IN_e, dhg, GH, ws_wide.data_ptr(), wsb, st)
                if fuse:
                    _lib.call('tmpnn_gather_diff_fwd', g.cref(), dmsg.data_ptr(), IN_e, dhg, GH, H, 1, st)
            else:
              _lib.call('tmpnn_gru_bwd_data', g.edge_row.data_ptr(), E, IN_e, hg, GH, H,
                      P[f + 'edge_gru.weight_ih'].data_ptr(), P[f + 'edge_gru.weight_hh'].data_ptr(),
                      gp, plane, dog, GH, dyp, we, dmsg.data_ptr(), IN_e, dhg, GH,
                      g.src.data_ptr() if fuse else None, g.dst.data_ptr() if fuse else None,
                      dmsg.data_ptr() if fuse else None, IN_e, st)
            if wide_det:
                pass
            elif saved.get('wide') and WIDE_DW:
                ws2b = int(lib.tmpnn_wide_gru_bwd_weights_ws(E, H))
                ws2 = _wide_workspace(ws2b, dev, slot=1)
                _lib.call('tmpnn_wide_gru_bwd_weights', ws_wide.data_ptr(), g.edge_row.data_ptr(), E, g.src.data_ptr(),
                          g.dst.data_ptr(), hg, GH, H,
                          grads[f + 'edge_gru.weight_ih'].data_ptr(), grads[f + 'edge_gru.weight_hh'].data_ptr(),
                          grads[f + 'edge_gru.bias_ih'].data_ptr(), grads[f + 'edge_gru.bias_hh'].data_ptr(),
                          ws2.data_ptr(), ws2b, st)
            else:
                _lib.call('tmpnn_gru_bwd_weights', g.edge_row.data_ptr(), E, xmode, g.src.data_ptr(), g.dst.data_ptr(),
                          None, 0, 0, IN_e, hg, GH, H, gp, plane, dog, GH, dyp, we,
                          grads[f + 'edge_gru.weight_ih'].data_ptr(), grads[f + 'edge_gru.weight_hh'].data_ptr(),
                          grads[f + 'edge_gru.bias_ih'].data_ptr(), grads[f + 'edge_gru.bias_hh'].data_ptr(),
                          ws_w.data_ptr(), ws_w.numel() * 4, st)
        if K > 0:
            erec, inc_other = g.att_index() if E > 0 else (None, None)
            for k0, Kg, W, a, kp, ws_ha, score, stats, esk in saved['att'][gi]:
                ws_n_att = lib.tmpnn_att_bwd_ws(E, Dn, H, Kg)
                ws_att = torch.empty((max(ws_n_att, 1),), **opts)
                if Kg == K:
                    d_out, ld_dout = dmsg.data_ptr(), IN_e
                else:
                    d_es_g = torch.zeros((N, H), **opts)
                    d_es_g[g.det_row.long()] = dmsg[g.det_row.long(), :H] * (Kg / K)
                    d_out, ld_dout = d_es_g.data_ptr(), H
                gW = [grads.get(f + f'gat.{k}.W_att') for k in range(k0, k0 + Kg)] if grad_out is not None else []
                ga = [grads.get(f + f'gat.{k}.a') for k in range(k0, k0 + Kg)] if grad_out is not None else []
                args = (g.cref(), _lib.ptr(erec), _lib.ptr(inc_other), hg, GH, H, Kg, W.data_ptr(),
                        a.data_ptr(), _lib.ptr(kp), ATT_DROPOUT_P, ws_ha.data_ptr(), score.data_ptr(), stats.data_ptr(),
                        esk.data_ptr(), d_out, ld_dout, ws_att.data_ptr(), ws_att.numel(), dhg, GH)
                if grad_out is not None and all(t is not None and t.is_contiguous() for t in gW + ga):
                    pW = (ctypes.c_void_p * Kg)(*[t.data_ptr() for t in gW])
                    pa = (ctypes.c_void_p * Kg)(*[t.data_ptr() for t in ga])
                    _lib.call('tmpnn_att_bwd_heads', *args, ctypes.cast(pW, ctypes.c_void_p), ctypes.cast(pa, ctypes.c_void_p), st)
                else:
                    dW = torch.zeros((Kg, H, H), **opts)
                    da = torch.zeros_like(a)
                    _lib.call('tmpnn_att_bwd', *args, dW.data_ptr(), da.data_ptr(), st)
                    for k in range(Kg):
                        if grad_out is not None:
                            grads[f + f'gat.{k0 + k}.W_att'].add_(dW[k])
                            grads[f + f'gat.{k0 + k}.a'].add_(da[k].reshape(-1, 1))
                        else:
                            grads[f + f'gat.{k0 + k}.W_att'] = dW[k]
                            grads[f + f'gat.{k0 + k}.a'] = da[k].reshape(-1, 1)
        name = 'tmpnn_gather_concat_bwd' if spec.msg_type == 'concat' else 'tmpnn_gather_diff_bwd'
        if not (not use_fused_bwd and saved.get('wide') and WIDE_DET):
            _lib.call(name, g.cref(), dmsg.data_ptr(), IN_e, dhg, GH, H, 1, st)

    d_x = None
    if n > 0:
        nd = int(plan.new_det_row.numel())
        S = plan.S
        xdet = saved['xdet']
        Ft = spec.F_total
        d_xdet = torch.empty((max(nd, 1), Ft), **opts) if need_x else None
        d_xzero = torch.empty((max(S, 1), Ft), **opts) if need_x else None
        f0 = 0
        for gi, (_, F) in enumerate(spec.groups):
            t = f'input_transforms.{gi}.'
            dz_g = torch.empty((max(S, 1), F), **opts) if need_x else None
            if _input_tf(plan, H, F):
                wsb = int(lib.tmpnn_input_tf_bwd_ws(nd, S, H, F, int(training)))
                ws = torch.empty((wsb // 4 + 1,), **opts)
                _lib.call('tmpnn_input_tf_bwd', xdet.data_ptr() + 4 * f0, _lib.ptr(saved.get('xrows')), Ft, F, nd,
                          plan.seg_ptr.data_ptr(), plan.seg_cnt.data_ptr(), _lib.ptr(plan.seg_of_det), S, plan.max_seg_nd, H,
                          int(training), P[t + '0.weight'].data_ptr(), P[t + '0.bias'].data_ptr(),
                          P[t + '1.weight'].data_ptr(), P[t + '1.bias'].data_ptr(), P[t + '3.weight'].data_ptr(),
                          saved['y_save'][gi].data_ptr(), saved['mean'][gi].data_ptr(), saved['rstd'][gi].data_ptr(),
                          plan.new_det_row.data_ptr(), d_hcat.data_ptr() + 4 * gi * H, GH,
                          (d_xdet.data_ptr() + 4 * f0) if need_x else None, Ft, _lib.ptr(dz_g),
                          grads[t + '0.weight'].data_ptr(), grads[t + '0.bias'].data_ptr(),
                          grads[t + '1.weight'].data_ptr(), grads[t + '1.bias'].data_ptr(),
                          grads[t + '3.weight'].data_ptr(), grads[t + '3.bias'].data_ptr(),
                          ws.data_ptr(), wsb, st)
                if need_x:
                    d_xzero[:, f0:f0 + F] = dz_g
                f0 += F
                continue
            wsn = lib.tmpnn_input_bn_bwd_ws(nd, S, H, F)
            ws = torch.empty((max(wsn, 1),), **opts)
            _lib.call('tmpnn_input_bn_bwd', xdet.data_ptr() + 4 * f0, Ft, F, nd,
                      plan.seg_ptr.data_ptr(), plan.seg_cnt.data_ptr(), _lib.ptr(plan.seg_of_det), S, H, int(training),
                      P[t + '0.weight'].data_ptr(), P[t + '0.bias'].data_ptr(),
                      P[t + '1.weight'].data_ptr(), P[t + '1.bias'].data_ptr(), P[t + '3.weight'].data_ptr(),
                      saved['y_save'][gi].data_ptr(), saved['mean'][gi].data_ptr(), saved['rstd'][gi].data_ptr(),
                      plan.new_det_row.data_ptr(), d_hcat.data_ptr() + 4 * gi * H, GH,
                      (d_xdet.data_ptr() + 4 * f0) if need_x else None, Ft, _lib.ptr(dz_g),
                      grads[t + '0.weight'].data_ptr(), grads[t + '0.bias'].data_ptr(),
                      grads[t + '1.weight'].data_ptr(), grads[t + '1.bias'].data_ptr(),
                      grads[t + '3.weight'].data_ptr(), grads[t + '3.bias'].data_ptr(),
                      ws.data_ptr(), ws.numel(), st)
            if need_x:
                d_xzero[:, f0:f0 + F] = dz_g
            f0 += F
        if need_x:
# ... 51 lines not shown
```

Before: 727.2 million graph-edges/s.

## Fold output-head weight gradients into fused GRU backward kernel

Computes the output-head weight gradient (dy times recomputed h_out) inside the fused GRU backward kernel, using cross-lane permlane folds and per-block slabs summed by a small reduction kernel. A new heads_dy kernel then only produces dy and the bias gradients, plus the edge weight gradient for zero-state rows. This avoids a separate pass that re-reads the full h_out matrix to form head weight gradients. In exchange the main backward kernel does extra arithmetic, LDS writes and a slab store per block, and there is one more small reduction launch.

```diff
diff --git a/include/tmpnn.h b/include/tmpnn.h
--- a/include/tmpnn.h
+++ b/include/tmpnn.h
@@ -138,6 +138,15 @@
                         const int32_t* add_src, const int32_t* add_dst, const float* add_msg, int ld_add,
                         float* dW_ih, float* dW_hh, float* db_ih, float* db_hh,
                         void* ws, size_t ws_bytes, tmpnn_stream stream);
+int tmpnn_gru_bwd_fused_heads(const int32_t* rows, int R, int xmode, const int32_t* src, const int32_t* dst,
+                              const float* msg, int ld_msg, int msg_compact, int IN,
+                              const float* h, int ld_h, int H, const float* w_ih, const float* w_hh,
+                              const float* gates, size_t gate_plane, const float* d_hout, int ld_dhout,
+                              const float* dy, const float* w_head,
+                              float* d_msg, int ld_dmsg, float* d_h, int ld_dh,
+                              const int32_t* add_src, const int32_t* add_dst, const float* add_msg, int ld_add,
+                              float* dW_ih, float* dW_hh, float* db_ih, float* db_hh, float* dW_head,
+                              void* ws, size_t ws_bytes, tmpnn_stream stream);
 int tmpnn_gru_bwd_fused_zero_state_available(int H, int IN, int xmode);
 int tmpnn_gru_bwd_fused_zero_state(const int32_t* rows, int R, const int32_t* src, const int32_t* dst, int IN,
                                    const float* h, int ld_h, int H, const float* w_ih, const float* b_hn,
@@ -205,6 +214,10 @@
                     float* d_h, int ld_dh, int accumulate,
                     float* dw_node, float* db_node, float* dw_edge, float* db_edge,
                     void* ws, size_t ws_bytes, tmpnn_stream stream);
+int tmpnn_heads_dy(const float* h, int ld_h, int C, int N, const uint8_t* is_edge, const float* scores,
+                   const float* d_logits, const float* d_scores, float* dy_out, int r0, int r1,
+                   float* dw_node, float* db_node, float* dw_edge, float* db_edge,
+                   void* ws, size_t ws_bytes, tmpnn_stream stream);
 
 int tmpnn_targets(const tmpnn_graph* g, const uint8_t* labels, uint8_t* targets, tmpnn_stream stream);
 size_t tmpnn_ce_loss_ws(int Dn);
diff --git a/trackmpnn_amd/_lib.py b/trackmpnn_amd/_lib.py
--- a/trackmpnn_amd/_lib.py
+++ b/trackmpnn_amd/_lib.py
@@ -119,6 +119,11 @@
                                     c_void_p, c_void_p, c_void_p, c_int, c_void_p, c_int,
                                     c_void_p, c_void_p, c_void_p, c_int, c_void_p, c_void_p, c_void_p, c_void_p,
                                     c_void_p, c_size_t, c_void_p]),
+    'tmpnn_gru_bwd_fused_heads': (c_int, [c_void_p, c_int, c_int, c_void_p, c_void_p, c_void_p, c_int, c_int, c_int,
+                                          c_void_p, c_int, c_int, c_void_p, c_void_p, c_void_p, c_size_t, c_void_p, c_int,
+                                          c_void_p, c_void_p, c_void_p, c_int, c_void_p, c_int,
+                                          c_void_p, c_void_p, c_void_p, c_int, c_void_p, c_void_p, c_void_p, c_void_p,
+                                          c_void_p, c_void_p, c_size_t, c_void_p]),
     'tmpnn_gru_bwd_fused_zero_state_available': (c_int, [c_int, c_int, c_int]),
     'tmpnn_gru_bwd_fused_zero_state': (c_int, [c_void_p, c_int, c_void_p, c_void_p, c_int, c_void_p, c_int, c_int,
                                                c_void_p, c_void_p, c_void_p, c_size_t, c_void_p, c_int, c_void_p,
@@ -153,6 +158,8 @@
     'tmpnn_heads_bwd': (c_int, [c_void_p, c_int, c_int, c_int, c_void_p, c_void_p, c_void_p, c_void_p, c_void_p,
                                 c_void_p, c_void_p, c_void_p, c_int, c_int, c_void_p, c_void_p, c_void_p, c_void_p,
                                 c_void_p, c_size_t, c_void_p]),
+    'tmpnn_heads_dy': (c_int, [c_void_p, c_int, c_int, c_int, c_void_p, c_void_p, c_void_p, c_void_p, c_void_p, c_int,
+                               c_int, c_void_p, c_void_p, c_void_p, c_void_p, c_void_p, c_size_t, c_void_p]),
     'tmpnn_targets': (c_int, [_GP, c_void_p, c_void_p, c_void_p]),
     'tmpnn_ce_loss_ws': (c_size_t, [c_int]),
     'tmpnn_ce_loss_fwd': (c_int, [_GP, c_void_p, c_void_p, c_void_p, c_void_p, c_void_p, c_size_t, c_void_p]),
diff --git a/trackmpnn_amd/csrc/dense.hip b/trackmpnn_amd/csrc/dense.hip
--- a/trackmpnn_amd/csrc/dense.hip
+++ b/trackmpnn_amd/csrc/dense.hip
@@ -674,6 +674,89 @@
     const float s = red[j];
     if (j < C) dw_node[j] += s;
     else if (j < 2 * C) dw_edge[j - C] += s;
+    else if (j == 2 * C) db_node[0] += s;
+    else db_edge[0] += s;
+}
+
+__device__ __forceinline__ float head_dy(long i, const float* __restrict__ scores, const float* __restrict__ d_logits,
+                                         const float* __restrict__ d_scores) {
+    float dy = d_logits ? d_logits[i] : 0.f;
+    if (d_scores) {
+        const float sc = scores[i];
+        dy += d_scores[i] * sc * (1.0f - sc);
+    }
+    return dy;
+}
+
+__global__ __launch_bounds__(256) void k_heads_dy(const float* __restrict__ h, int ld_h, int C, int N,
+                                                  const uint8_t* __restrict__ is_edge, const float* __restrict__ scores,
+                                                  const float* __restrict__ d_logits, const float* __restrict__ d_scores,
+                                                  float* __restrict__ dy_out, long r0, long r1, int want,
+                                                  int rows_per_block, float* __restrict__ part) {
+    extern __shared__ float sm[];
+    const int tid = threadIdx.x;
+    const long b0 = (long)blockIdx.x * rows_per_block;
+    const long b1 = min((long)N, b0 + rows_per_block);
+    float bn = 0.f, be = 0.f;
+    for (long i = b0 + tid; i < b1; i += 256) {
+        const float dy = head_dy(i, scores, d_logits, d_scores);
+        dy_out[i] = dy;
+        if (is_edge[i]) be += dy; else bn += dy;
+    }
+    const int cpt = C >> 2;
+    const int slots = 256 / cpt;
+    float* bsm = sm + (size_t)slots * 2 * C;
+    bsm[2 * tid] = bn;
+    bsm[2 * tid + 1] = be;
+    const int slot = tid / cpt;
+    const int c4 = (tid % cpt) * 4;
+    float4 an = make_float4(0.f, 0.f, 0.f, 0.f), ae = an;
+    const long span = (r1 - r0 + gridDim.x - 1) / gridDim.x;
+    const long q0 = r0 + (long)blockIdx.x * span, q1 = min(r1, q0 + span);
+    if (slot < slots) {
+        constexpr int UR = 4;
+        for (long i0 = q0 + slot; i0 < q1; i0 += (long)slots * UR) {
+            float dyv[UR];
+            bool ev[UR];
+            float4 xv[UR];
+#pragma unroll
+            for (int u = 0; u < UR; ++u) {
+                const long i = i0 + (long)u * slots;
+                const long ic = i < q1 ? i : q1 - 1;
+                ev[u] = is_edge[ic] != 0;
+                const bool take = i < q1 && (want & (ev[u] ? 2 : 1));
+                dyv[u] = take ? head_dy(ic, scores, d_logits, d_scores) : 0.f;
+                xv[u] = take ? *reinterpret_cast<const float4*>(h + (size_t)ic * ld_h + c4) : make_float4(0.f, 0.f, 0.f, 0.f);
+            }
+#pragma unroll
+            for (int u = 0; u < UR; ++u) {
+                const float dy = dyv[u];
+                const float4 x = xv[u];
+                if (ev[u]) { ae.x += dy * x.x; ae.y += dy * x.y; ae.z += dy * x.z; ae.w += dy * x.w; }
+                else       { an.x += dy * x.x; an.y += dy * x.y; an.z += dy * x.z; an.w += dy * x.w; }
+            }
+        }
+        float* my = sm + (size_t)slot * 2 * C;
+        *reinterpret_cast<float4*>(my + c4) = an;
+        *reinterpret_cast<float4*>(my + C + c4) = ae;
+    }
+    __syncthreads();
+    float* out = part + (size_t)blockIdx.x * (2 * C + 2);
+    for (int j = tid; j < 2 * C + 2; j += 256) {
+        float s = 0.f;
+        if (j < 2 * C) for (int k = 0; k < slots; ++k) s += sm[(size_t)k * 2 * C + j];
+        else for (int k = 0; k < 256; ++k) s += bsm[2 * k + (j - 2 * C)];
+        out[j] = s;
+    }
+}
+
+__global__ void k_heads_dy_final(const float* __restrict__ red, int C, float* __restrict__ dw_node,
+                                 float* __restrict__ db_node, float* __restrict__ dw_edge, float* __restrict__ db_edge) {
+    const int j = blockIdx.x * blockDim.x + threadIdx.x;
+    if (j >= 2 * C + 2) return;
+    const float s = red[j];
+    if (j < C) { if (dw_node) dw_node[j] += s; }
+    else if (j < 2 * C) { if (dw_edge) dw_edge[j - C] += s; }
     else if (j == 2 * C) db_node[0] += s;
     else db_edge[0] += s;
 }
@@ -888,4 +971,35 @@
     return check_launch("heads_bwd_final");
 }
 
-}
+int tmpnn_heads_dy(const float* h, int ld_h, int C, int N, const uint8_t* is_edge, const float* scores,
+                   const float* d_logits, const float* d_scores, float* dy_out, int r0, int r1, float* dw_node,
+                   float* db_node, float* dw_edge, float* db_edge, void* ws, size_t ws_bytes, tmpnn_stream stream) {
+    TM_REQUIRE(C > 0 && (C & 3) == 0 && C <= 1024 && N >= 0, "heads_dy: C=%d N=%d", C, N);
+    if (N == 0) return TMPNN_OK;
+    TM_REQUIRE(is_edge && dy_out && db_node && db_edge, "heads_dy: null pointer");
+    TM_REQUIRE(d_scores == nullptr || scores != nullptr, "heads_dy: d_scores needs scores");
+    if (r0 < 0) r0 = 0;
+    if (r1 > N) r1 = N;
+    const int want = r0 < r1 ? ((dw_node ? 1 : 0) | (dw_edge ? 2 : 0)) : 0;
+    TM_REQUIRE(want == 0 || (h && (ld_h & 3) == 0 && ld_h >= C && aligned16(h)), "heads_dy: h rows must be 16-byte aligned");
+    const size_t need = tmpnn_heads_bwd_ws(N, C);
+    if (!ws || ws_bytes < need) return set_error(TMPNN_EWORKSPACE, "heads_dy: workspace %zu < %zu", ws_bytes, need);
+    const int rpb = heads_rows_per_block(N);
+    const int nblk = ceil_div(N, rpb);
+    const int slots = 256 / (C >> 2);
+    const size_t shm = ((size_t)slots * 2 * C + 512) * sizeof(float);
+    hipStream_t st = as_stream(stream);
+    hipLaunchKernelGGL(k_heads_dy, dim3(nblk), dim3(256), shm, st, h, ld_h, C, N, is_edge, scores, d_logits, d_scores,
+                       dy_out, (long)r0, (long)(want ? r1 : r0), want, rpb, reinterpret_cast<float*>(ws));
+    int rc = check_launch("heads_dy");
+    if (rc) return rc;
+    const size_t nred = 2 * (size_t)C + 2;
+    float* part = reinterpret_cast<float*>(ws);
+    float* red = part + (size_t)nblk * nred;
+    if ((rc = launch_reduce_slabs(part, nred, nblk, red, nred, 0, st, red + nred))) return rc;
+    hipLaunchKernelGGL(k_heads_dy_final, dim3(ceil_div(2 * C + 2, 256)), dim3(256), 0, st, red, C, dw_node, db_node,
+                       dw_edge, db_edge);
+    return check_launch("heads_dy_final");
+}
+
+}
diff --git a/trackmpnn_amd/csrc/gru_bwd.hip b/trackmpnn_amd/csrc/gru_bwd.hip
--- a/trackmpnn_amd/csrc/gru_bwd.hip
+++ b/trackmpnn_amd/csrc/gru_bwd.hip
@@ -1466,6 +1466,14 @@
 }
 
 #define TWO_MARK(i) do { } while (0)
+__device__ __forceinline__ float head_fold4(const float (&v)[4]) {
+    const auto a = __builtin_amdgcn_permlane32_swap(__float_as_uint(v[0]), __float_as_uint(v[2]), false, false);
+    const auto b = __builtin_amdgcn_permlane32_swap(__float_as_uint(v[1]), __float_as_uint(v[3]), false, false);
+    const float k0 = __uint_as_float(a[0]) + __uint_as_float(a[1]);
+    const float k1 = __uint_as_float(b[0]) + __uint_as_float(b[1]);
+    const auto c = __builtin_amdgcn_permlane16_swap(__float_as_uint(k0), __float_as_uint(k1), false, false);
+    return __uint_as_float(c[0]) + __uint_as_float(c[1]);
+}
 struct TwoRaw { float4 dh, r, z, n, hn, hp, xa, xb, ea, eb; float dy; };
 #define TWO_LD4(p) (*reinterpret_cast<const float4*>(p))
 
@@ -1475,8 +1483,8 @@
 #ifndef TWO_EXP
 #define TWO_EXP 0
 #endif
-template <int XMODE, int UP, bool FUSE, bool HHS = true>
-__global__ __launch_bounds__(512) void k_gru_bwd_two(GruBwdFusedArgs a, int ntiles) {
+template <int XMODE, int UP, bool FUSE, bool HHS = true, bool HG = false>
+__global__ __launch_bounds__(512) void k_gru_bwd_two(GruBwdFusedArgs a, int ntiles, float* __restrict__ slab_h) {
     constexpr int exp_ = TWO_EXP;
     constexpr int H = 64;
     constexpr int SUB = 32 * 128;
@@ -1533,6 +1541,7 @@
 #pragma unroll
         for (int i = 0; i < 16; ++i) acc[j][i] = 0.f;
     float bsum[3] = {0.f, 0.f, 0.f};
+    float hacc = 0.f;
 
     const int G = gridDim.x;
     const int nmine = (ntiles - (int)blockIdx.x + G - 1) / G;
@@ -1561,6 +1570,12 @@
             }                                                                                                \
             half_put((img), st0, PA, o_);                                                                    \
             half_put((img), SUB + (st0 ^ 64), PA, q_);                                                       \
+            if (HG) {                                                                                        \
+                const float hp_[4] = {raw.hp.x, raw.hp.y, raw.hp.z, raw.hp.w};                               \
+                const float dyh_ = (vld) ? raw.dy : 0.f;                                                     \
+                _Pragma("unroll") for (int i = 0; i < 4; ++i) q_[i] = dyh_ * ((1.0f - z_[i]) * n_[i] + z_[i] * hp_[i]); \
+                hacc += head_fold4(q_);                                                                      \
+            }                                                                                                \
         } else if ((SL) == 1) {                                                                              \
             const float z_[4] = {raw.z.x, raw.z.y, raw.z.z, raw.z.w}, n_[4] = {raw.n.x, raw.n.y, raw.n.z, raw.n.w}; \
             const float hp_[4] = {raw.hp.x, raw.hp.y, raw.hp.z, raw.hp.w};                                   \
@@ -1787,7 +1802,14 @@
             const float tot = bsum[j] + __shfl_xor(bsum[j], 32);
             if (half == 0) red[wave * 96 + j * 32 + c32] = tot;
         }
+        if (HG) lds[8 * 96 + wave * 64 + 4 * j16 + kq] = hacc;
         __syncthreads();
+        if (HG && wave == 0) {
+            float s = 0.f;
+#pragma unroll
+            for (int w = 0; w < 8; ++w) s += lds[8 * 96 + w * 64 + lane];
+            slab_h[(size_t)blockIdx.x * 64 + lane] = s;
+        }
         if (HHS && tt == 0 && half == 0) {
             float* sb = a.slab_b + (size_t)blockIdx.x * 6 * H;
 #pragma unroll
@@ -2100,6 +2122,21 @@
     }
 }
 
+__global__ __launch_bounds__(1024) void k_head_slab_sum(const float* __restrict__ slab_h, int n, float* __restrict__ dW_head) {
+    __shared__ float part[16][64];
+    const int c = threadIdx.x & 63, g = threadIdx.x >> 6;
+    float s = 0.f;
+#pragma unroll 4
+    for (int k = g; k < n; k += 16) s += slab_h[(size_t)k * 64 + c];
+    part[g][c] = s;
+    __syncthreads();
+    if (g == 0) {
+        float t = 0.f;
+#pragma unroll
+        for (int i = 0; i < 16; ++i) t += part[i][c];
+        dW_head[c] += t;
+    }
+}
 
 static int weights_variant_default() {
     static const int v = [] {
@@ -2275,7 +2312,7 @@
 #define LC(U, F, S)                                                                                          \
     do {                                                                                                     \
         TM_SHM_ONCE((k_gru_bwd_two<2, U, F, S>), shm);                                                       \
-        hipLaunchKernelGGL((k_gru_bwd_two<2, U, F, S>), dim3(n_rs), dim3(512), shm, st, a, ntiles);          \
+        hipLaunchKernelGGL((k_gru_bwd_two<2, U, F, S>), dim3(n_rs), dim3(512), shm, st, a, ntiles, nullptr);          \
     } while (0)
 #define LCU(F, S) do { if (up == 1) LC(1, F, S); else if (up == 2) LC(2, F, S); else LC(3, F, S); } while (0)
         if (half == 0) { if (fuse) LCU(true, true); else LCU(false, true); }
@@ -2303,12 +2340,15 @@
     return TMPNN_OK;
 }
 
-int tmpnn_gru_bwd_fused(const int32_t* rows, int R, int xmode, const int32_t* src, const int32_t* dst, const float* msg,
-                        int ld_msg, int msg_compact, int IN, const float* h, int ld_h, int H, const float* w_ih,
-                        const float* w_hh, const float* gates, size_t gate_plane, const float* d_hout, int ld_dhout,
-                        const float* dy, const float* w_head, float* d_msg, int ld_dmsg, float* d_h, int ld_dh,
-                        const int32_t* add_src, const int32_t* add_dst, const float* add_msg, int ld_add, float* dW_ih,
-                        float* dW_hh, float* db_ih, float* db_hh, void* ws, size_t ws_bytes, tmpnn_stream stream) {
+static constexpr size_t kHeadSlabBytes = (size_t)256 * 64 * sizeof(float);
+
+static int gru_bwd_fused_impl(const int32_t* rows, int R, int xmode, const int32_t* src, const int32_t* dst, const float* msg,
+                              int ld_msg, int msg_compact, int IN, const float* h, int ld_h, int H, const float* w_ih,
+                              const float* w_hh, const float* gates, size_t gate_plane, const float* d_hout, int ld_dhout,
+                              const float* dy, const float* w_head, float* d_msg, int ld_dmsg, float* d_h, int ld_dh,
+                              const int32_t* add_src, const int32_t* add_dst, const float* add_msg, int ld_add, float* dW_ih,
+                              float* dW_hh, float* db_ih, float* db_hh, float* dW_head, void* ws, size_t ws_bytes,
+                              tmpnn_stream stream) {
     TM_REQUIRE(tmpnn_gru_bwd_fused_available(H, IN, xmode), "gru_bwd_fused: H=%d IN=%d xmode=%d not supported", H, IN, xmode);
     if (R == 0) return TMPNN_OK;
     TM_REQUIRE(R > 0 && rows && h && w_ih && w_hh && gates && d_msg && d_h && dW_ih && dW_hh && db_ih && db_hh,
@@ -2324,10 +2364,13 @@
                "gru_bwd_fused: rows must be 16-byte aligned");
     TM_REQUIRE(xmode == 0 || add_msg == nullptr || (add_src == src && add_dst == dst),
                "gru_bwd_fused: with xmode != 0 the fused adjoint gathers through src / dst (pass the same arrays)");
-    const size_t need = tmpnn_gru_bwd_fused_ws(R, IN, H);
+    const bool hg = dW_head != nullptr;
+    TM_REQUIRE(!hg || (xmode != 2 && dy != nullptr), "gru_bwd_fused_heads: needs xmode 0 / 1 and dy");
+    const size_t need = tmpnn_gru_bwd_fused_ws(R, IN, H) + (hg ? kHeadSlabBytes : 0);
     if (ws == nullptr || ws_bytes < need)
         return set_error(TMPNN_EWORKSPACE, "gru_bwd_fused: workspace %zu < %zu bytes", ws_bytes, need);
     const int n_rs = fused_blocks(R);
+    float* slab_h = hg ? reinterpret_cast<float*>(reinterpret_cast<char*>(ws) + tmpnn_gru_bwd_fused_ws(R, IN, H)) : nullptr;
     const size_t nW = (size_t)3 * H * (IN + H), nB = (size_t)6 * H;
     float* slab_w = reinterpret_cast<float*>(ws);
     float* slab_b = slab_w + (size_t)n_rs * nW;
@@ -2352,7 +2395,7 @@
     do {                                                                                                     \
         if (fused_two_waves() && !((X) == 0 && (F))) {      \
             TM_SHM_ONCE((k_gru_bwd_two<X, U, F>), shm);                                                      \
-            hipLaunchKernelGGL((k_gru_bwd_two<X, U, F>), dim3(n_rs), dim3(512), shm, st, a, ntiles);         \
+            hipLaunchKernelGGL((k_gru_bwd_two<X, U, F>), dim3(n_rs), dim3(512), shm, st, a, ntiles, nullptr);         \
         } else {                                                                                             \
             TM_SHM_ONCE((k_gru_bwd_one<X, U, F>), shm);                                                      \
             hipLaunchKernelGGL((k_gru_bwd_one<X, U, F>), dim3(n_rs), dim3(256), shm, st, a, ntiles);         \
@@ -2364,14 +2407,27 @@
     do {                                                                                                     \
         if (!((X) == 0 && (F))) {                                                                            \
             TM_SHM_ONCE((k_gru_bwd_two<X, U, F>), shm);                                                      \
-            hipLaunchKernelGGL((k_gru_bwd_two<X, U, F>), dim3(n_rs), dim3(512), shm, st, a, ntiles);         \
+            hipLaunchKernelGGL((k_gru_bwd_two<X, U, F>), dim3(n_rs), dim3(512), shm, st, a, ntiles, nullptr);         \
         }                                                                                                    \
     } while (0)
 #endif
+#define LH(X, U, F)                                                                                          \
+    do {                                                                                                     \
+        TM_SHM_ONCE((k_gru_bwd_two<X, U, F, true, true>), shm);                                              \
+        hipLaunchKernelGGL((k_gru_bwd_two<X, U, F, true, true>), dim3(n_rs), dim3(512), shm, st, a, ntiles, slab_h); \
+    } while (0)
 #define LU(X, F) do { if (up == 1) LF(X, 1, F); else if (up == 2) LF(X, 2, F); else LF(X, 3, F); } while (0)
-    if (xmode == 0) { if (fuse) LU(0, true); else LU(0, false); }
-    else            { if (fuse) LU(1, true); else LU(1, false); }
+#define LUH(X, F) do { if (up == 2) LH(X, 2, F); else LH(X, 3, F); } while (0)
+    if (hg) {
+        TM_REQUIRE(!(xmode == 0 && fuse), "gru_bwd_fused_heads: xmode 0 takes no fused adjoint");
+        if (xmode == 0) LUH(0, false);
+        else if (fuse) LUH(1, true);
+        else LUH(1, false);
+    } else if (xmode == 0) { if (fuse) LU(0, true); else LU(0, false); }
+    else                   { if (fuse) LU(1, true); else LU(1, false); }
+#undef LUH
 #undef LU
+#undef LH
 #undef LF
     int rc = check_launch("gru_bwd_fused");
     if (rc) return rc;
@@ -2389,7 +2445,36 @@
     }
     hipLaunchKernelGGL(k_gru_reduce_w, dim3(ceil_div((long)(nW + nB), 256)), dim3(256), 0, st, rw, rb, nred, IN, H,
                        dW_ih, dW_hh, db_ih, db_hh);
-    return check_launch("gru_reduce_w");
+    if ((rc = check_launch("gru_reduce_w"))) return rc;
+    if (hg) {
+        hipLaunchKernelGGL(k_head_slab_sum, dim3(1), dim3(1024), 0, st, slab_h, n_rs, dW_head);
+        return check_launch("head_slab_sum");
+    }
+    return TMPNN_OK;
+}
+
+int tmpnn_gru_bwd_fused(const int32_t* rows, int R, int xmode, const int32_t* src, const int32_t* dst, const float* msg,
+                        int ld_msg, int msg_compact, int IN, const float* h, int ld_h, int H, const float* w_ih,
+                        const float* w_hh, const float* gates, size_t gate_plane, const float* d_hout, int ld_dhout,
+                        const float* dy, const float* w_head, float* d_msg, int ld_dmsg, float* d_h, int ld_dh,
+                        const int32_t* add_src, const int32_t* add_dst, const float* add_msg, int ld_add, float* dW_ih,
+                        float* dW_hh, float* db_ih, float* db_hh, void* ws, size_t ws_bytes, tmpnn_stream stream) {
+    return gru_bwd_fused_impl(rows, R, xmode, src, dst, msg, ld_msg, msg_compact, IN, h, ld_h, H, w_ih, w_hh, gates,
+                              gate_plane, d_hout, ld_dhout, dy, w_head, d_msg, ld_dmsg, d_h, ld_dh, add_src, add_dst, add_msg,
+                              ld_add, dW_ih, dW_hh, db_ih, db_hh, nullptr, ws, ws_bytes, stream);
+}
+
+int tmpnn_gru_bwd_fused_heads(const int32_t* rows, int R, int xmode, const int32_t* src, const int32_t* dst, const float* msg,
+                              int ld_msg, int msg_compact, int IN, const float* h, int ld_h, int H, const float* w_ih,
+                              const float* w_hh, const float* gates, size_t gate_plane, const float* d_hout, int ld_dhout,
+                              const float* dy, const float* w_head, float* d_msg, int ld_dmsg, float* d_h, int ld_dh,
+                              const int32_t* add_src, const int32_t* add_dst, const float* add_msg, int ld_add, float* dW_ih,
+                              float* dW_hh, float* db_ih, float* db_hh, float* dW_head, void* ws, size_t ws_bytes,
+                              tmpnn_stream stream) {
+    TM_REQUIRE(dW_head != nullptr, "gru_bwd_fused_heads: null dW_head");
+    return gru_bwd_fused_impl(rows, R, xmode, src, dst, msg, ld_msg, msg_compact, IN, h, ld_h, H, w_ih, w_hh, gates,
+                              gate_plane, d_hout, ld_dhout, dy, w_head, d_msg, ld_dmsg, d_h, ld_dh, add_src, add_dst, add_msg,
+                              ld_add, dW_ih, dW_hh, db_ih, db_hh, dW_head, ws, ws_bytes, stream);
 }
 
 int tmpnn_gru_bwd_fused_zero_state_available(int H, int IN, int xmode) {
diff --git a/trackmpnn_amd/functional.py b/trackmpnn_amd/functional.py
--- a/trackmpnn_amd/functional.py
+++ b/trackmpnn_amd/functional.py
@@ -16,6 +16,7 @@
 FUSED_BWD = os.environ.get('TMPNN_FUSED_BWD', '1') == '1'
 ZERO_STATE_BWD = os.environ.get('TMPNN_BWD_ZERO_STATE', '1') != '0'
 ZERO_STATE_FWD = os.environ.get('TMPNN_FWD_ZERO_STATE', '1') != '0'
+HEADS_FOLD = os.environ.get('TMPNN_HEADS_FOLD', '1') != '0'
 WIDE_OVERLAP = os.environ.get('TMPNN_WIDE_OVERLAP', '0') == '1' and os.environ.get('TMPNN_KEEP_VARIANTS', '0') == '1'
 ATT_KMAX = 8
 _SPLIT = os.environ.get('TMPNN_SPLIT', '1')[:1] != '0'
@@ -489,8 +490,35 @@
 
     lib = _lib.load()
     dh_up = _f32c(d_hout) if d_hout is not None else None
+    IN_e = spec.IN_e
+    xmode = 2 if spec.msg_type == 'concat' else 1
+    use_fused_bwd = (FUSED_BWD and lib.tmpnn_gru_bwd_fused_available(H, H, 0)
+                     and lib.tmpnn_gru_bwd_fused_available(H, IN_e, xmode))
+    E_old = E - (n - int(plan.new_det_row.numel())) if n > 0 else E
+
+    def zs_of(gi):
+        if 'zs_bwd' in saved:
+            return saved['zs_bwd']
+        b_hn = P[f'factor_grus.{gi}.edge_gru.bias_hh'].data_ptr() + 4 * 2 * H
+        return bool(ZERO_STATE_BWD and n > 0 and K == 0 and xmode == 1 and 0 <= E_old < E and b_hn % 16 == 0
+                    and not (saved.get('proj') and gi in saved['proj'])
+                    and lib.tmpnn_gru_bwd_fused_zero_state_available(H, IN_e, xmode))
+    zs_g = [zs_of(gi) for gi in range(G)] if use_fused_bwd else []
+    fold = (HEADS_FOLD and use_fused_bwd and xmode == 1 and GH <= 1024 and not saved.get('proj')
+            and (d_scores is not None or d_logits is not None) and len(set(zs_g)) == 1)
     dy = None
-    if d_scores is not None or d_logits is not None:
+    if fold:
+        dy = torch.empty((N,), **opts)
+        dl = _f32c(d_logits) if d_logits is not None else None
+        ds = _f32c(d_scores) if d_scores is not None else None
+        ws_b = lib.tmpnn_heads_bwd_ws(N, GH)
+        ws = torch.empty((max(ws_b // 4, 1),), **opts)
+        r0, r1 = (N_old, N) if zs_g[0] else (0, 0)
+        _lib.call('tmpnn_heads_dy', h_out.data_ptr(), GH, GH, N, g.is_edge.data_ptr(), saved['scores'].data_ptr(),
+                  _lib.ptr(dl), _lib.ptr(ds), dy.data_ptr(), r0, r1, None, grads['output_transform_node.bias'].data_ptr(),
+                  grads['output_transform_edge.weight'].data_ptr() if zs_g[0] else None,
+                  grads['output_transform_edge.bias'].data_ptr(), ws.data_ptr(), ws_b, st)
+    elif d_scores is not None or d_logits is not None:
         dy = torch.empty((N,), **opts)
         dl = _f32c(d_logits) if d_logits is not None else None
         ds = _f32c(d_scores) if d_scores is not None else None
@@ -510,15 +538,13 @@
         dh_up = torch.zeros((N, GH), **opts)
 
     d_hcat = torch.empty((N, GH), **opts)
-    IN_e = spec.IN_e
     dmsg = torch.empty((N, IN_e), **opts)
-    xmode = 2 if spec.msg_type == 'concat' else 1
     plane = N * H
     ws_e = lib.tmpnn_gru_bwd_weights_ws(E, IN_e, H)
     ws_n = lib.tmpnn_gru_bwd_weights_ws(Dn, H, H)
-    use_fused_bwd = (FUSED_BWD and lib.tmpnn_gru_bwd_fused_available(H, H, 0)
-                     and lib.tmpnn_gru_bwd_fused_available(H, IN_e, xmode))
     ws_f = max(lib.tmpnn_gru_bwd_fused_ws(E, IN_e, H), lib.tmpnn_gru_bwd_fused_ws(Dn, H, H)) if use_fused_bwd else 0
+    if fold:
+        ws_f += 65536
     ws_w = torch.empty((max(ws_e, ws_n, ws_f) // 4 + 1,), **opts)
     w_node, w_edge = P['output_transform_node.weight'], P['output_transform_edge.weight']
     for gi in range(G):
@@ -533,11 +559,14 @@
         we = (w_edge.data_ptr() + 4 * gi * H) if dy is not None else None
         fuse = K == 0
         if use_fused_bwd:
-            _lib.call('tmpnn_gru_bwd_fused', g.det_row.data_ptr(), Dn, 0, None, None, es.data_ptr(), H, 1, H,
+            hd_n = ((grads['output_transform_node.weight'].data_ptr() + 4 * gi * H,) if fold else ())
+            hd_e = ((grads['output_transform_edge.weight'].data_ptr() + 4 * gi * H,) if fold else ())
+            fused = 'tmpnn_gru_bwd_fused_heads' if fold else 'tmpnn_gru_bwd_fused'
+            _lib.call(fused, g.det_row.data_ptr(), Dn, 0, None, None, es.data_ptr(), H, 1, H,
                       hg, GH, H, P[f + 'node_gru.weight_ih'].data_ptr(), P[f + 'node_gru.weight_hh'].data_ptr(),
                       gp, plane, dog, GH, dyp, wn, dmsg.data_ptr(), IN_e, dhg, GH, None, None, None, 0,
                       grads[f + 'node_gru.weight_ih'].data_ptr(), grads[f + 'node_gru.weight_hh'].data_ptr(),
-                      grads[f + 'node_gru.bias_ih'].data_ptr(), grads[f + 'node_gru.bias_hh'].data_ptr(),
+                      grads[f + 'node_gru.bias_ih'].data_ptr(), grads[f + 'node_gru.bias_hh'].data_ptr(), *hd_n,
                       ws_w.data_ptr(), ws_w.numel() * 4, st)
             if saved.get('proj') and gi in saved['proj']:
                 proj_s, whh_t_s = saved['proj'][gi]
@@ -546,23 +575,17 @@
                           whh_t_s.data_ptr(), P[f + 'edge_gru.bias_ih'].data_ptr(), P[f + 'edge_gru.bias_hh'].data_ptr(),
                           h_scr.data_ptr() + 4 * gi * H, GH, gp, plane, None, None, 0, st)
             b_hn = P[f + 'edge_gru.bias_hh'].data_ptr() + 4 * 2 * H
-            E_old = E - (n - int(plan.new_det_row.numel())) if n > 0 else E
-            if 'zs_bwd' in saved:
-                zs = saved['zs_bwd']
-            else:
-                zs = (ZERO_STATE_BWD and n > 0 and K == 0 and xmode == 1 and 0 <= E_old < E and b_hn % 16 == 0
-                      and not (saved.get('proj') and gi in saved['proj'])
-                      and lib.tmpnn_gru_bwd_fused_zero_state_available(H, IN_e, xmode))
+            zs = zs_g[gi]
             E_full = E_old if zs else E
             if E_full > 0:
-                _lib.call('tmpnn_gru_bwd_fused', g.edge_row.data_ptr(), E_full, xmode, g.src.data_ptr(), g.dst.data_ptr(),
+                _lib.call(fused, g.edge_row.data_ptr(), E_full, xmode, g.src.data_ptr(), g.dst.data_ptr(),
                           None, 0, 0, IN_e, hg, GH, H,
                           P[f + 'edge_gru.weight_ih'].data_ptr(), P[f + 'edge_gru.weight_hh'].data_ptr(),
                           gp, plane, dog, GH, dyp, we, dmsg.data_ptr(), IN_e, dhg, GH,
                           g.src.data_ptr() if fuse else None, g.dst.data_ptr() if fuse else None,
                           dmsg.data_ptr() if fuse else None, IN_e,
                           grads[f + 'edge_gru.weight_ih'].data_ptr(), grads[f + 'edge_gru.weight_hh'].data_ptr(),
-                          grads[f + 'edge_gru.bias_ih'].data_ptr(), grads[f + 'edge_gru.bias_hh'].data_ptr(),
+                          grads[f + 'edge_gru.bias_ih'].data_ptr(), grads[f + 'edge_gru.bias_hh'].data_ptr(), *hd_e,
                           ws_w.data_ptr(), ws_w.numel() * 4, st)
             if zs:
                 _lib.call('tmpnn_gru_bwd_fused_zero_state', g.edge_row.data_ptr() + 4 * E_old, E - E_old,
```

Result: no change. 734.2 million graph-edges/s, median of 6 (+1.0%).
